# zju-vipa/ProtoPFormer

Hardware: AMD Instinct MI355X
Metric: images/sec train step, deit_small+2000 protos, bs256, 1/2/4/8 MI355X (higher is better)
Workload: dtype bf16; 1 GPU; deit_small_patch16_224, synthetic 224x224, 2000x384 prototypes, 200 classes, k=81, batch 256/GPU (BASELINE.json configs[2]), train step = fwd+CE+PPC+bwd+allreduce+AdamW+EMA, DropPath 0.1; blocks after the token reservation run compacted on the 1+k reserved rows (equal to the masked full-length blocks to bf16 rounding); bf16 backbone: the reserved tokens differ from the fp32 reference's in ~2-3 % o; global_batch=256, parallelism=dp1

## Files before the change

include/ppf_hip.h:

```cpp
#ifndef PPF_HIP_H
#define PPF_HIP_H

#include <stddef.h>
#include <stdint.h>

#ifdef __cplusplus
extern "C" {
#endif

typedef struct ihipStream_t* ppf_stream_t;

#define PPF_ERR_SHAPE (-1)
#define PPF_ERR_ALIGN (-2)
#define PPF_ERR_ARG (-3)

#define PPF_ABI_VERSION 10

const char* ppf_last_error(void);
int ppf_abi_version(void);
int ppf_device_info(int* cu_count, int* clock_mhz, char* name, int name_len);
int ppf_stream_arm(ppf_stream_t stream, int on);
int ppf_stream_wait_stream(ppf_stream_t dst, ppf_stream_t src);
int64_t ppf_stream_mark(ppf_stream_t stream);
int ppf_stream_wait_mark(ppf_stream_t stream, int64_t ticket);

int ppf_gemm_bf16(const void* A, const void* B, void* C, int M, int N, int K, int lda, int ldb, int ldc, int trans_a,
                  int trans_b, int epi, const float* bias, const float* res, int ldres, const float* rowscale,
                  int rows_per_group, const float* colscale, const void* aux_in, void* aux_out, int ldaux, float* colsum,
                  float alpha, void* workspace, size_t workspace_bytes, ppf_stream_t stream);
size_t ppf_gemm_workspace_bytes(int M, int N, int K);

int ppf_gemm_test_force_g224(int force);

int ppf_gemm_probe(int enable);
int ppf_gemm_probe_read(double* ms_total, int64_t* launches, double* flops, double* bytes);

int ppf_path_probe(int enable);
int ppf_path_probe_read(int tag, double* ms_total, int64_t* launches, double* flops, double* bytes);

int ppf_gemm_bf16_batched(const void* A, const void* B, void* C, int M, int N, int K, int lda, int ldb, int ldc, int trans_a,
                          int trans_b, int out_f32, float alpha, int batch_outer, int batch_inner, int64_t sa_o, int64_t sa_i,
                          int64_t sb_o, int64_t sb_i, int64_t sc_o, int64_t sc_i, int kpad, ppf_stream_t stream);

int ppf_layernorm_bwd_f32(const float* dy, const float* x, const int* row_map, const float* w, const float* dres_in, float* dx_out, float* dw, float* db,
                          int rows, int D, float eps, ppf_stream_t stream);
int ppf_ew_bwd_f32(int kind, const float* a, const float* b, float* out, const float* rowscale, int rows_per_group, int M, int N, ppf_stream_t stream);
int ppf_colsum_f32(const float* in, float* out, int M, int N, ppf_stream_t stream);
int ppf_attn_bwd_f32(const float* qkv, const float* dout, const float* policy, float* dqkv, float* scratch, int B, int H, int N, int D, int self_keep,
                     int eps_n, ppf_stream_t stream);
int ppf_th_attn_bwd_f32(const float* qkv, const float* dout, const float* wl, const float* bl, const float* ww, const float* bw, float* dqkv,
                        float* dwl, float* dbl, float* dww, float* dbw, int B, int H, int N, int D, ppf_stream_t stream);
int ppf_class_attn_bwd_f32(const float* q, const float* k, const float* v, const float* policy, const float* dout, float* dq, float* dk, float* dv,
                           int B, int H, int N1, int D, ppf_stream_t stream);

int ppf_rowgemm_supported(int D, int K, int rows_per_tile);
int ppf_rowgemm_bf16(const void* A, const void* B, int M, int D, int K, int lda, int ldb, int rows_per_tile, const float* bias, void* out,
                     ppf_stream_t stream);
int ppf_rowgemm_resid_ln(const void* A, const void* B, int M, int D, int K, int lda, int ldb, int rows_per_tile, const float* bias,
                         const float* res, float* xout, const float* rowscale, int rows_per_group, const float* colscale, void* aux_out,
                         const float* ln_w, const float* ln_b, void* ln_out, float* ln_mean, float* ln_rstd, float eps, ppf_stream_t stream);
int ppf_rowgemm_lnbwd(const void* A, const void* B, int M, int D, int K, int lda, int ldb, int rows_per_tile, const float* x, const float* mean,
                      const float* rstd, const float* w, const float* dres_in, float* dx_out, void* cast_out, const float* rowscale,
                      int rows_per_group, const float* colscale, const void* branch, float* partial, size_t partial_bytes, ppf_stream_t stream);
int ppf_rowgemm_colsum(const float* partial, int tiles, int D, int nparts, float* dw, float* db, float* dg, ppf_stream_t stream);
int ppf_transpose_bf16_batched(const void* src, void* dst, const void* desc_i64, int n, int total_tiles, ppf_stream_t stream);

int ppf_layernorm_fwd(const float* x, const int* row_map, const float* w, const float* b, void* y, float* mean, float* rstd,
                      int rows, int D, float eps, ppf_stream_t stream);
int ppf_layernorm_bwd(const void* dy, const float* x, const int* row_map, const float* w, const float* mean, const float* rstd,
                      const float* dres_in, float* dx_out, float* dw, float* db, void* cast_out, const float* rowscale,
                      int rows_per_group, const float* colscale, float* dbias_next, const void* branch, float* dcolscale,
                      int rows, int D, float* partial, size_t partial_bytes, ppf_stream_t stream);
int ppf_layernorm_bwd_blocks(int rows);
int ppf_layernorm_bwd_reduce(const float* partial, int rows, int D, float* dw, float* db, float* dbias_next, float* dcolscale,
                             ppf_stream_t stream);

int ppf_attn_fwd(const void* qkv, void* out, const float* policy, float* rowmax, float* zinv, int B, int H, int N, int D,
                 int self_keep, int eps_n, ppf_stream_t stream);
int ppf_attn_fwd_hm_supported(int H, int N, int D);
int ppf_attn_fwd_hm(const void* qkv, void* out, const float* policy, float* rowmax, float* zinv, float* headmean, int NP, int B, int H, int N,
                    int D, int self_keep, int eps_n, ppf_stream_t stream);
int ppf_attn_headmean(const void* qkv, const float* policy, const float* rowmax, const float* zinv, float* headmean, int NP,
                      int B, int H, int N, int D, int self_keep, int eps_n, ppf_stream_t stream);
int ppf_attn_bwd(const void* qkv, const void* out, const void* dout, void* dqkv, const float* policy, const float* rowmax,
                 const float* zinv, float* delta, int B, int H, int N, int D, int self_keep, int eps_n, ppf_stream_t stream);

int ppf_th_scores(const void* qkv, const float* wl, const float* bl, float* sp, int B, int H, int N, int D, int NP, ppf_stream_t stream);
int ppf_th_dwl(const void* qkv, const float* ds_prime, float* dwl, int B, int H, int N, int D, int NP, ppf_stream_t stream);
int ppf_th_softmax_mix(float* sp, void* a16, float* hm, const float* ww, const float* bw, int B, int H, int N, int NP, int NPK,
                       ppf_stream_t stream);
int ppf_th_softmax_bwd(const float* prob, float* da, void* ds16, const float* ww, const float* wl, float* dww, float* dbw, float* dbl,
                       int B, int H, int N, int NP, int NPK, ppf_stream_t stream);
int ppf_th_fused_supported(int H, int N, int D);
int ppf_th_fwd(const void* qkv, const float* wl, const float* bl, const float* ww, const float* bw, void* a16, float* hm, float* rowmax,
               float* zinv, void* out, int B, int H, int N, int D, int NP, int NPK, ppf_stream_t stream);
size_t ppf_th_bwd_partial_floats(int B, int H, int N);
int ppf_th_bwd(const void* qkv, const void* dout, const float* wl, const float* bl, const float* ww, const float* rowmax, const float* zinv,
               void* ds16, float* partial, int B, int H, int N, int D, int NPK, ppf_stream_t stream);
int ppf_th_param_reduce(const float* partial, int B, int H, int N, float* dww, float* dbw, float* dbl, float* dwl, ppf_stream_t stream);
int ppf_th_grads_supported(int H, int N, int D);
int ppf_th_grads(const void* qkv, const void* dout, const void* ds16, const void* a16, void* dqkv, int B, int H, int N, int D, int NPK,
                 ppf_stream_t stream);
int ppf_class_attn_fwd(const void* q, const void* k, const void* v, const float* policy, float* attn, float* zinv, float* rowmean,
                       void* out, int B, int H, int N1, int D, ppf_stream_t stream);
int ppf_class_attn_bwd(const void* q, const void* k, const void* v, const float* attn, const float* zinv, const void* dout, void* dq,
                       void* dk, void* dv, int B, int H, int N1, int D, ppf_stream_t stream);
int ppf_merge3_cast(const float* a, const float* b, const float* cq, void* out, int rows, int D, int N1, ppf_stream_t stream);

int ppf_rollout_threshold(const float* hm_layer, int B, int N, int NP, int kdrop, void* thr_out_u32, ppf_stream_t stream);
int ppf_rollout(const float* hm, int64_t layer_stride, int L, int B, int N, int NP, const float* init_rows, int n_init, int lead,
                int kdrop, int kdrop_init, float identity, int k, const void* thr_u32, float* cls_attn, int* idx, float* policy,
                ppf_stream_t stream);
int ppf_topk_sorted(const float* scores, int B, int n, int k, int* idx, ppf_stream_t stream);

int ppf_proto_fwd(const float* tok, int64_t stride_b, int t0, int T, const float* protos, int B, int P, int Dp, int act_kind,
                  float eps, float* act_max, int* argmax, float* dist_full, float* act_full, void* workspace, size_t workspace_bytes,
                  ppf_stream_t stream);
size_t ppf_proto_fwd_workspace(int P, int Dp);
int ppf_proto_bwd(const float* tok, int64_t stride_b, int t0, int T, const float* protos, int B, int P, int Dp, int act_kind,
                  float eps, const float* dist_full, int map_is_act, const float* g_full, const float* g_max, const int* argmax, float* dtok,
                  int64_t dstride_b, float* dprotos, void* zeroed_workspace, size_t workspace_bytes, ppf_stream_t stream);
size_t ppf_proto_bwd_workspace(int B, int T, int P, int Dp, int want_dtok, int want_dprotos);
int ppf_proto_bwd_rows(const float* tok, int64_t stride_b, int t0, int T, const float* protos, int B, int P, int Dp, int act_kind,
                       float eps, const float* dist_full, int map_is_act, const float* g_rows, const void* label_i64, int ppc, const float* g_max,
                       const int* argmax, float* dtok, int64_t dstride_b, float* dprotos, void* workspace, size_t workspace_bytes,
                       ppf_stream_t stream);
size_t ppf_proto_bwd_single_workspace(int B, int P, int Dp);
int ppf_proto_bwd_single(const float* tok, int64_t stride_b, int t0, const float* protos, int B, int P, int Dp, int act_kind, float eps,
                         const float* dist, const float* g, float* dtok, int64_t dstride_b, float* dprotos, void* workspace,
                         size_t workspace_bytes, ppf_stream_t stream);

int ppf_ppc_loss(const float* act, const int* idx, const void* label_i64, int B, int P, int T, int ppc, int side,
                 float cov_thresh, float mean_thresh, float* partial, float* gcov, float* gmean, float* loss, ppf_stream_t stream);
int ppf_ppc_loss_bwd(const float* gcov, const float* gmean, const float* up_cov, const float* up_mean, const void* label_i64,
                     float* g_full, int B, int P, int T, int ppc, ppf_stream_t stream);
int ppf_cross_entropy(const float* logits, const void* label_i64, float* per_sample, float* dlogits, float* loss, int B, int C,
                      ppf_stream_t stream);
int ppf_soft_cross_entropy(const float* logits, const float* target, const void* label_i64, float smoothing, float* per_sample,
                           float* dlogits, float* loss, int B, int C, ppf_stream_t stream);
int ppf_eval_metrics(const float* logits, const float* logits_global, const float* logits_local, const void* label_i64, double* acc,
                     int B, int C, ppf_stream_t stream);
int ppf_proto_topk_init(float* val, int* img, int* pos, int P, int K, ppf_stream_t stream);
int ppf_proto_topk_merge(const float* act_max, const int* argmax, const int* idx, int k, const float* tok, int64_t stride_b, int t0, int Dp,
                         const void* label_i64, const int* image_id, int ppc, int B, int P, int K, float* val, int* img, int* pos,
                         float* best_feat, ppf_stream_t stream);
int ppf_explain_topk(const float* act_max, const int* argmax, const int* idx, int T, const float* act_full, const float* weight, float scale,
                     int ppc, const float* logits, const int* cls_in, int sign, int B, int P, int C, int M, int K, int G, int* cls_out,
                     float* cls_logit, int* proto, float* contrib, float* act, int* cell, float* evidence, float* maps, ppf_stream_t stream);
int ppf_sgemm(const float* A, const float* Bm, float* C, int M, int N, int K, int64_t sam, int64_t sak, int64_t sbn, int64_t sbk,
              int ldc, float alpha, float beta, float* workspace, int64_t workspace_floats, ppf_stream_t stream);
int64_t ppf_sgemm_pair_workspace(int M, int N0, int K0, int N1, int K1);
int ppf_sgemm_pair(const float* A0, const float* B0, float* out0, int N0, int K0, int64_t sam0, int64_t sak0, int64_t sbn0, int64_t sbk0,
                   int ldo0, float alpha0, const float* A1, const float* B1, float* out1, int N1, int K1, int64_t sam1, int64_t sak1,
                   int64_t sbn1, int64_t sbk1, int ldo1, float alpha1, float* sum, int ldsum, float c0, float c1, int M, float* workspace,
                   int64_t workspace_floats, ppf_stream_t stream);
int ppf_axpby(const float* x, const float* y, float* out, float a, float b, int64_t n, ppf_stream_t stream);
int ppf_axpbypcz(const float* x, const float* y, const float* z, float* out, float a, float b, float c, int64_t n, ppf_stream_t stream);

int ppf_act_upsample(const float* grids, float* out, int M, int g, int S, ppf_stream_t stream);
int ppf_act_peak(const float* grids, int M, int g, int S, float* peak_val, int* peak_yx, const int* parts, int maps_per_img, int n_parts,
                 int half_size, void* table_u8, ppf_stream_t stream);
int ppf_act_part_table(const int* peak_yx, int M, int S, const int* parts, int maps_per_img, int n_parts, int half_size, void* table_u8,
                       ppf_stream_t stream);
int ppf_act_order_stats(const float* grids, int M, int g, int S, int k_lo, int k_hi, float* stats, ppf_stream_t stream);
int ppf_act_box(const float* grids, const double* thr, int M, int g, int S, int* box, ppf_stream_t stream);
int ppf_add_gauss_noise(const float* x, float* out, int B, int64_t n_per_img, const void* image_id_i64, float sigma, uint64_t seed,
                        ppf_stream_t stream);
int ppf_part_meter_update(const void* table_u8, const void* table_noisy_u8, const int* parts, const void* label_i64, int B, int ppc, int n_parts,
                          int C, int* hits, int* visible, int* stable, int* images, int* bad, ppf_stream_t stream);

int ppf_cast_f32_bf16(const float* in, void* out, int64_t n, ppf_stream_t stream);
int ppf_cast_bf16_f32(const void* in, float* out, int64_t n, ppf_stream_t stream);
int ppf_im2col_patch(const float* img, void* cols, int B, int C, int H, int W, int patch, ppf_stream_t stream);
int ppf_assemble_tokens(const float* tok, const float* cls, const float* pos, float* x, int B, int Np, int D, int lead,
                        ppf_stream_t stream);
int ppf_assemble_tokens_bwd(const float* dx, void* dtok, float* dpos, float* dcls, int B, int Np, int D, int lead,
                            ppf_stream_t stream);
int ppf_sigmoid_bwd_blocks(int rows);
int ppf_sigmoid_bwd(const float* df, const float* f, void* dz, float* dbias, int rows, int cols, float* partial, size_t partial_bytes,
                    ppf_stream_t stream);
int ppf_adamw_step(float* p, const float* g, float* m, float* v, float* ema, void* p16, int64_t n, int nseg,
                   const int64_t* seg_bounds, const float* seg_lr, const float* seg_wd, float beta1, float beta2, float eps,
                   int step, float ema_decay, float grad_scale, ppf_stream_t stream);
int ppf_adamw_step_dev(float* p, const float* g, float* m, float* v, float* ema, void* p16, int64_t n, int nseg,
                       const int64_t* seg_bounds, const float* hyper, float beta1, float beta2, float eps, float ema_decay,
                       ppf_stream_t stream);
int ppf_adamw_step_guarded(float* p, const float* g, float* m, float* v, float* ema, void* p16, int64_t n, int nseg,
                           const int64_t* seg_bounds, const float* hyper, float beta1, float beta2, float eps, float ema_decay,
                           const float* loss, int* nonfinite_flag, ppf_stream_t stream);
int ppf_hyper_set(float* hyper, const float* host_vals, int n, ppf_stream_t stream);
int ppf_clip_grad_blocks(void);
int ppf_clip_grad_scale(const float* g, int64_t n, float max_norm, float pre_scale, float* partial, float* hyper, float* norm_out,
                        ppf_stream_t stream);
int ppf_droppath_scales(float* out, const float* keep, int nslot, int B, uint64_t seed, void* state_u64, ppf_stream_t stream);
int ppf_reserved_rows_map(const int* idx, int* rows, int B, int k, int N, ppf_stream_t stream);
int ppf_gather_rows(const void* src, const int* rows, void* dst, int nrows, int row_bytes, ppf_stream_t stream);
int ppf_scatter_rows(const void* src, const int* rows, void* dst, int nrows_src, int nrows_dst, int row_bytes, ppf_stream_t stream);
int ppf_memset_zero(void* ptr, size_t bytes, ppf_stream_t stream);
int ppf_copy_2d(void* dst, int64_t dst_pitch, const void* src, int64_t src_pitch, int64_t width, int64_t rows, ppf_stream_t stream);
int ppf_image_finish_u8(const void* in_u8_hwc, float* out_nchw, int B, int H, int W, const float* mean3, const float* std3,
                        const int* rects, uint64_t seed, const void* state_u64, ppf_stream_t stream);
#define PPF_MIX_KIND 0
#define PPF_MIX_YL 1
#define PPF_MIX_YH 2
#define PPF_MIX_XL 3
#define PPF_MIX_XH 4
#define PPF_MIX_WSELF 5
#define PPF_MIX_WOTHER 6
#define PPF_MIX_WORDS 8
int ppf_mixup_apply(float* x, const int* table_host, int* table_dev, int B, int Cc, int H, int W, ppf_stream_t stream);
int ppf_mixup_target(const void* label_i64, const float* lam, int lam_stride, float off_value, float on_value, float* target, int B,
                     int C, ppf_stream_t stream);
int ppf_scale_by_scalar(const float* x, const float* scalar_dev, float* out, int64_t n, ppf_stream_t stream);

int ppf_im2col_patch_f32(const float* img, float* cols, int B, int C, int H, int W, int patch, ppf_stream_t stream);
int ppf_layernorm_fwd_f32(const float* x, const int* row_map, const float* w, const float* b, float* y, int rows, int D, float eps,
                          ppf_stream_t stream);
int ppf_epilogue_f32(float* C, const float* bias, int kind, const float* res, const float* rowscale, int rows_per_group,
                     const float* colscale, int M, int N, ppf_stream_t stream);
int ppf_attn_fwd_f32(const float* qkv, float* out, const float* policy, float* headmean, int NP, int B, int H, int N, int D,
                     int self_keep, int eps_n, ppf_stream_t stream);
int ppf_th_attn_fwd_f32(const float* qkv, const float* wl, const float* bl, const float* ww, const float* bw, float* out,
                        float* headmean, int NP, int B, int H, int N, int D, ppf_stream_t stream);
int ppf_class_attn_fwd_f32(const float* q, const float* k, const float* v, const float* policy, float* attn_mean, float* out, int B,
                           int H, int N1, int D, ppf_stream_t stream);

#ifdef __cplusplus
}
#endif
#endif
```

protopformer_amd/backbone.py:

```python
import functools
import os

import torch
import torch.nn as nn

from . import _lib, ops
from .ops import EPI_ATOMIC, EPI_BF16, EPI_DGELU, EPI_F32, EPI_GELU, EPI_RESID, EPI_SIGMOID_F32

LN_EPS = 1e-6
_KEEP_CACHE = {}
_ROW_BWD_MAX_ELEMS = 12_000_000


def _row_bwd(M, D):
    return M * D <= _ROW_BWD_MAX_ELEMS


def droppath_scales(rates, B, device, training):
    slots = [r if training else 0.0 for r in rates]
    active = [i for i, r in enumerate(slots) if r > 0.0]
    if not active:
        return None, [-1] * len(slots)
    key = (tuple(slots), str(device))
    st = _KEEP_CACHE.get(key)
# ... 164 lines not shown
    for j in reversed(range(1, len(convs))):
        c, x_in = convs[j], acts[j - 1]
        ops.linear_wgrad_f32(d, x_in, gv(c.weight), gv(c.bias))
        d = ops.ew_bwd_f32(5, ops.linear_dgrad_f32(d, c.weight), x_in)
    ops.colsum_f32(d, gv(convs[0].bias))
    return ops.cast_bf16(d)


class WgradLane:

    def __init__(self, device):
        self.enabled = os.environ.get("PPF_WGRAD_STREAM", "1") != "0"
        self.streams = [torch.cuda.Stream(device=device)] if self.enabled else []
        self.raws = [st.cuda_stream for st in self.streams]
        self.last_read = {}
        self.tracked = set()
        self.held = []
        self.pending = []

    def track(self, t):
        self.tracked.add(t.data_ptr())
        return t

    def submit(self, fn, reads, tag=None, defer=False):
        if not self.enabled:
            fn()
            return
        self.pending.append((fn, reads, tag))
        self.held.extend(reads)
        if not defer:
            self.flush()

    def flush(self, tag=None):
        if not self.pending:
            return
        raw = self.raws[0]
        try:
            _lib.call("ppf_stream_wait_stream", raw, _lib.stream_ptr())
            for fn, reads, tg in self.pending:
                _lib.push_stream(raw)
                try:
                    fn()
                    ptrs = [t.data_ptr() for t in reads if t.data_ptr() in self.tracked]
                    if ptrs:
                        ticket = _lib.stream_mark(raw)
                        for q in ptrs:
                            self.last_read[q] = ticket
                finally:
                    _lib.pop_stream()
        finally:
            self.pending.clear()

    def before_overwrite(self, t):
        if t.data_ptr() not in self.tracked:
            raise RuntimeError("WgradLane.before_overwrite: buffer was not registered with track()")
        q = t.data_ptr()
        if any(r.data_ptr() == q for _, reads, _t in self.pending for r in reads):
            self.flush()
        ticket = self.last_read.pop(q, None)
        if ticket is not None:
            _lib.call("ppf_stream_wait_mark", _lib.stream_ptr(), ticket)

    def join(self):
        if self.enabled:
            self.flush()
            for raw in self.raws:
                _lib.call("ppf_stream_wait_stream", _lib.stream_ptr(), raw)
        self.last_read.clear()
        self.tracked.clear()
        self.held.clear()


def wgrad_lane(store):
    lane = getattr(store, "_wgrad_lane", None)
    if lane is None:
        lane = store._wgrad_lane = WgradLane(store.device)
    return lane


_ROLL_TAIL = 1
_ROLL_BATCH = 3


def _wgrad(store, dy16, x16, weight, bias=None, defer=False):
    gw = store.grad_view(weight)
    gb = store.grad_view(bias) if bias is not None else None
    wgrad_lane(store).submit(lambda: ops.gemm(dy16, x16, trans_a=True, trans_b=True, epi=EPI_ATOMIC, out=gw.reshape(weight.shape[0], -1),
                                              colsum=gb), (dy16, x16), defer=defer and min(weight.shape[0], weight.shape[1]) <= 256)


_DGRAD_ROW = 3


def _dgrad(store, dy16, weight, rows, which):
    wt = store.w16t(weight)
    if wt is not None and (_DGRAD_ROW & which) and ops.rowgemm_ok(wt.shape[0], wt.shape[1], rows):
        return ops.rowgemm_bf16(dy16, wt, rows)
    if wt is not None:
        return ops.gemm(dy16, wt, epi=EPI_BF16)
    return ops.gemm(dy16, store.w16(weight), trans_b=True, epi=EPI_BF16)


def head_bwd(ppnet, store, saved, df):
    head = saved["head"]
    conv = addon_convs(ppnet)[0]
    dz = addon_bwd(ppnet, store, head, saved["f"].reshape(-1, saved["f"].shape[-1]), df)
    _wgrad(store, dz, head["nf"], conv.weight)
    return ops.gemm(dz, store.w16(conv.weight).reshape(conv.out_channels, -1), trans_b=True, epi=EPI_BF16)


def chunk_ready(gs, lane, chunk):
    lane.flush()
    _lib.run_live(lambda: gs.chunk_ready(chunk, also=lane.streams))


def dyb_ring(lane, D):
    nring = 4 if D > 256 else 64
    ring = {}

    def next_dyb(cur):
        if nring >= 64:
            return torch.empty_like(cur)
        bufs = ring.setdefault(tuple(cur.shape), [cur])
        if not any(b.data_ptr() == cur.data_ptr() for b in bufs):
            bufs.append(cur)
        if len(bufs) < nring:
            nxt = lane.track(torch.empty_like(cur))
            bufs.append(nxt)
        else:
            i = next(j for j, b in enumerate(bufs) if b.data_ptr() == cur.data_ptr())
            nxt = bufs[(i + 1) % len(bufs)]
        lane.before_overwrite(nxt)
        return nxt

    return next_dyb


def branch_out(store, dyb, rowscale, rows_per_group, gamma=None, raw=None):
    kw = dict(cast_out=dyb, rowscale=rowscale, rows_per_group=rows_per_group)
    if gamma is not None:
        kw.update(colscale=gamma, branch=raw, dcolscale=store.grad_view(gamma))
    return kw


def mlp_bwd(store, blk, L, dyb, bias_done):
    fc1, fc2 = blk.mlp.fc1, blk.mlp.fc2
    _wgrad(store, dyb, L["g"], fc2.weight, None if bias_done else fc2.bias, defer=True)
    w2t = store.w16t(fc2.weight)
    if w2t is not None:
        dh = ops.gemm(dyb, w2t, epi=EPI_DGELU, aux_in=L["h"])
    else:
        dh = ops.gemm(dyb, store.w16(fc2.weight), trans_b=True, epi=EPI_DGELU, aux_in=L["h"])
    _wgrad(store, dh, L["n2"], fc1.weight, fc1.bias)
    return dh


def row_tile_bwd(store, blk, D, rpt):
    covered = (all(store.w16t(w) is not None for w in (blk.mlp.fc1.weight, blk.attn.qkv.weight, blk.attn.proj.weight))
               and ops.rowgemm_ok(D, blk.mlp.fc1.out_features, rpt) and ops.rowgemm_ok(D, 3 * D, rpt) and ops.rowgemm_ok(D, D, rpt))
    return rpt if covered else None


def block_bwd(blk, store, L, dx, dyb, bias_done, below, *, next_dyb, attn_bwd, lnb, dgrad, row_tile):
    lane = wgrad_lane(store)
    gv = store.grad_view
    Nl = L["N"]
    fc1, qkv, proj = blk.mlp.fc1, blk.attn.qkv, blk.attn.proj
    fused = row_tile is not None

    def norm_bwd(dy, weight, dn, x, mean, rstd, norm, out, bias_next=None):
        nw = norm.weight
        if fused:
            ops.rowgemm_lnbwd(dy, store.w16t(weight), x, mean, rstd, nw, gv(nw), gv(norm.bias), row_tile, dres_in=dx, dx_out=dx,
                              lane=lane, defer_reduce=True, **out)
        else:
            lnb(dn, x, nw, mean, rstd, gv(nw), gv(norm.bias), dres_in=dx, dx_out=dx, dbias_next=gv(bias_next) if out else None, **out)

    dh = mlp_bwd(store, blk, L, dyb, bias_done)
    dyb = next_dyb(dyb)
    dn2 = None if fused else dgrad(dh, fc1.weight, Nl, 1)
    norm_bwd(dh, fc1.weight, dn2, L["x1"], L["mean2"], L["rstd2"], blk.norm2, branch_out(store, dyb, L["s1"], Nl, getattr(blk, "gamma_1", None), L["raw1"]),
             proj.bias)
    bias_done = not fused
    _wgrad(store, dyb, L["ao"], proj.weight, None if bias_done else proj.bias, defer=True)
    dao = ops.rowgemm_bf16(dyb, store.w16t(proj.weight), row_tile) if fused else dgrad(dyb, proj.weight, Nl, 4)
    dqkv = attn_bwd(blk, L, dao)
    _wgrad(store, dqkv, L["n1"], qkv.weight, qkv.bias)
    dn1 = None if fused else dgrad(dqkv, qkv.weight, Nl, 2)
    if below is None:
        norm_bwd(dqkv, qkv.weight, dn1, L["x"], L["mean1"], L["rstd1"], blk.norm1, {})
        return None, bias_done
    prev, Lp = below
    dyb = next_dyb(dyb)
    norm_bwd(dqkv, qkv.weight, dn1, L["x"], L["mean1"], L["rstd1"], blk.norm1,
             branch_out(store, dyb, Lp["s2"], Nl, getattr(prev, "gamma_2", None), Lp["raw2"]), prev.mlp.fc2.bias)
    return dyb, not fused


def embed_bwd(ppnet, store, saved, dx, lead):
    feats = ppnet.features
    pe = feats.patch_embed
    Np, D = pe.num_patches, dx.shape[1]
    gv = store.grad_view
    dtok = ops.assemble_tokens_bwd(dx, gv(feats.pos_embed).reshape(Np + lead, D), gv(feats.cls_token).reshape(D) if lead else None,
                                   dx.shape[0] // (Np + lead), Np, D, lead)
    _wgrad(store, dtok, saved["cols"], pe.proj.weight, pe.proj.bias)
    lane = wgrad_lane(store)
    gs = getattr(ppnet, "_grad_sync", None)
    if gs is not None:
        chunk_ready(gs, lane, gs.head_chunk)
    lane.join()


def deit_backward(ppnet, store, saved, df):
    feats = ppnet.features
    layers, head = saved["layers"], saved["head"]
    x_last = saved["x_last"]
    B, N, D = x_last.shape
    M = B * N
    dev = x_last.device
    lane = wgrad_lane(store)
    lnb = functools.partial(ops.layernorm_bwd, lane=lane, defer_reduce=True)
    dnf = head_bwd(ppnet, store, saved, df)
    alloc = ops.zeros if head["row_map"] is not None else (lambda shape, dtype, device: torch.empty(shape, dtype=dtype, device=device))
    dx = alloc((M, D), torch.float32, dev)
    dyb = lane.track(alloc((M, D), torch.bfloat16, dev))
    last = feats.blocks[-1]
    lnb(dnf, x_last.reshape(M, D), feats.norm.weight, head["meanf"], head["rstdf"], store.grad_view(feats.norm.weight),
        store.grad_view(feats.norm.bias), dx_out=dx, row_map=head["row_map"], cast_out=dyb, rowscale=layers[-1]["s2"],
        rows_per_group=N, dbias_next=store.grad_view(last.mlp.fc2.bias))
    gs = getattr(ppnet, "_grad_sync", None)
    if gs is not None:
        chunk_ready(gs, lane, gs.tail_chunk)
    bwd = functools.partial(block_bwd, next_dyb=dyb_ring(lane, D), lnb=lnb, dgrad=functools.partial(_dgrad, store),
                            attn_bwd=lambda blk, L, dao: ops.attn_bwd(L["qkv"], L["ao"], dao, L["rowmax"], L["zinv"], B, feats.num_heads, L["N"], D,
                                                                      policy=L["policy"], self_keep=True, eps_n=L["eps_n"]))
    bias_done = True
    for i in range(len(layers) - 1, -1, -1):
        L = layers[i]
        Nl = L["N"]
        row_tile = row_tile_bwd(store, feats.blocks[i], D, ops.rowgemm_tile_rows(B * Nl, Nl, backward=True)) if _row_bwd(B * Nl, D) else None
        dyb, bias_done = bwd(feats.blocks[i], store, L, dx, dyb, bias_done, (feats.blocks[i - 1], layers[i - 1]) if i > 0 else None,
                             row_tile=row_tile)
        if i > 0 and L["rows"] is not None:
            Mf = B * layers[i - 1]["N"]
            dx = ops.scatter_rows(dx, L["rows"], Mf)
            dyb = lane.track(ops.scatter_rows(dyb, L["rows"], Mf))
        if gs is not None and i in gs.block_chunk:
            chunk_ready(gs, lane, gs.block_chunk[i])
    if layers and layers[0]["rows"] is not None:
        dx = ops.scatter_rows(dx, layers[0]["rows"], B * (feats.patch_embed.num_patches + 1))
    embed_bwd(ppnet, store, saved, dx, 1)


class TokensFn(torch.autograd.Function):

    @staticmethod
    def forward(ctx, img, ppnet, dp, *params):
        store = ppnet.flat_store()
        store.refresh_bf16()
        feats = ppnet.features
        need_bwd = any(ctx.needs_input_grad)
        if need_bwd and "t16_params" in ppnet._arch_fns:
            if store._t16 is None:
                store.register_transposed(ppnet._arch_fns["t16_params"](feats))
            if store._t16 is not None and not store._t16["fresh"] and feats.embed_dim <= 256:
                wgrad_lane(store).submit(store.refresh_t16, (store.bf16, store._t16["buf"]), defer=True)
            else:
                store.refresh_t16()
        saved = {} if need_bwd else None
        (layer, k), = ppnet.reserve_layer_nums
        fwd = ppnet._arch_fns
        x = fwd["embed"](feats, store, img, saved)
        x_out, cls_attn, idx, layers = fwd["blocks"](feats, store, x, layer, k, dp, save=need_bwd)
        f, head = head_tokens_fwd(ppnet, store, x_out, idx)
        if need_bwd:
            saved.update(layers=layers, head=head, x_last=x_out, f=f)
            ctx.saved = saved
            ctx.ppnet = ppnet
        ctx.mark_non_differentiable(cls_attn, idx)
        return f, cls_attn, idx

    @staticmethod
    def backward(ctx, df, _dcls, _didx):
        ppnet, saved = ctx.ppnet, ctx.saved
        store = ppnet.flat_store()
        store.attach_all_grads()
        ppnet._arch_fns["backward"](ppnet, store, saved, df.contiguous().reshape(-1, df.shape[-1]))
        ctx.saved = None
        return (None, None, None) + (None,) * (len(ctx.needs_input_grad) - 3)


def t16_params(feats):
    return [w for blk in feats.blocks for w in (blk.mlp.fc1.weight, blk.attn.qkv.weight, blk.attn.proj.weight, blk.mlp.fc2.weight)]


DEIT_FNS = dict(embed=functools.partial(embed_tokens, lead=1), blocks=deit_blocks_fwd, backward=deit_backward, t16_params=t16_params)
```

protopformer_amd/csrc/elementwise.hip:

```cpp
#include "ppf_common.h"
#include "ppf_hip.h"

namespace {

__global__ __launch_bounds__(256) void cast_kernel(const float* __restrict__ in, bf16_t* __restrict__ out, int64_t n8) {
    for (int64_t i = (int64_t)blockIdx.x * 256 + threadIdx.x; i < n8; i += (int64_t)gridDim.x * 256) {
        const float4 a = reinterpret_cast<const float4*>(in)[2 * i], b = reinterpret_cast<const float4*>(in)[2 * i + 1];
        reinterpret_cast<uint4*>(out)[i] = make_uint4(pack_bf16x2(a.x, a.y), pack_bf16x2(a.z, a.w), pack_bf16x2(b.x, b.y), pack_bf16x2(b.z, b.w));
    }
}

__global__ __launch_bounds__(256) void widen_kernel(const bf16_t* __restrict__ in, float* __restrict__ out, int64_t n8) {
    for (int64_t i = (int64_t)blockIdx.x * 256 + threadIdx.x; i < n8; i += (int64_t)gridDim.x * 256) {
        const uint4 u = reinterpret_cast<const uint4*>(in)[i];
        const float2 a = unpack_bf16x2(u.x), b = unpack_bf16x2(u.y), c = unpack_bf16x2(u.z), d = unpack_bf16x2(u.w);
        reinterpret_cast<float4*>(out)[2 * i] = make_float4(a.x, a.y, b.x, b.y);
        reinterpret_cast<float4*>(out)[2 * i + 1] = make_float4(c.x, c.y, d.x, d.y);
    }
}

__global__ __launch_bounds__(256) void im2col_kernel(const float* __restrict__ img, bf16_t* __restrict__ cols, int B, int C,
                                                     int H, int W, int p, int64_t total8) {
    const int gh = H / p, gw = W / p, pp8 = p / 8, kdim = C * p * p;
    for (int64_t i = (int64_t)blockIdx.x * 256 + threadIdx.x; i < total8; i += (int64_t)gridDim.x * 256) {
// ... 123 lines not shown
            dz[o] = h;
            acc += bf16_to_f32(h);
        }
        if (partial) partial[(size_t)blockIdx.x * cols + c] = acc;
        else if (dbias) unsafeAtomicAdd(dbias + c, acc);
    }
}
__global__ __launch_bounds__(1024) void sigmoid_bias_reduce_kernel(const float* __restrict__ partial, float* __restrict__ dbias, int nblk, int cols) {
    __shared__ float red[16][64];
    const int cl = threadIdx.x & 63, g = threadIdx.x >> 6, c = blockIdx.x * 64 + cl;
    float acc = 0.f;
    if (c < cols) {
#pragma unroll 8
        for (int b = g; b < nblk; b += 16) acc += partial[(size_t)b * cols + c];
    }
    red[g][cl] = acc;
    __syncthreads();
    if (g == 0 && c < cols) {
        float t = 0.f;
#pragma unroll
        for (int i = 0; i < 16; ++i) t += red[i][cl];
        dbias[c] += t;
    }
}

__global__ __launch_bounds__(256) void sumsq_partial_kernel(const float* __restrict__ g, int64_t n4, float* __restrict__ partial) {
    float acc = 0.f;
    for (int64_t i = (int64_t)blockIdx.x * 256 + threadIdx.x; i < n4; i += (int64_t)gridDim.x * 256) {
        const float4 v = reinterpret_cast<const float4*>(g)[i];
        acc += v.x * v.x + v.y * v.y + v.z * v.z + v.w * v.w;
    }
    __shared__ float red[4];
    acc = wave_sum(acc);
    if ((threadIdx.x & 63) == 0) red[threadIdx.x >> 6] = acc;
    __syncthreads();
    if (threadIdx.x == 0) partial[blockIdx.x] = (red[0] + red[1]) + (red[2] + red[3]);
}
__global__ __launch_bounds__(256) void clip_finish_kernel(const float* __restrict__ partial, int nblk, float max_norm, float pre_scale,
                                                          float* __restrict__ hyper, float* __restrict__ norm_out) {
    __shared__ float red[256];
    float acc = 0.f;
    for (int i = threadIdx.x; i < nblk; i += 256) acc += partial[i];
    red[threadIdx.x] = acc;
    __syncthreads();
    for (int s = 128; s > 0; s >>= 1) {
        if (threadIdx.x < s) red[threadIdx.x] += red[threadIdx.x + s];
        __syncthreads();
    }
    if (threadIdx.x == 0) {
        const float nrm = pre_scale * sqrtf(red[0]);
        hyper[19] = fminf(1.0f, max_norm / (nrm + 1e-6f));
        if (norm_out) *norm_out = nrm;
    }
}

__global__ __launch_bounds__(256) void droppath_kernel(float* __restrict__ out, const float* __restrict__ keep, int nslot, int B,
                                                       uint64_t seed, unsigned long long* __restrict__ state) {
    const unsigned long long step = state[0];
    const int total = nslot * B;
    for (int i4 = threadIdx.x; i4 * 4 < total; i4 += 256) {
        const uint4 r = philox4x32_10(make_uint4((uint32_t)i4, 0u, (uint32_t)step, (uint32_t)(step >> 32)),
                                      make_uint2((uint32_t)seed, (uint32_t)(seed >> 32)));
        const uint32_t rv[4] = {r.x, r.y, r.z, r.w};
#pragma unroll
        for (int j = 0; j < 4; ++j) {
            const int i = i4 * 4 + j;
            if (i < total) {
                const float kp = keep[i / B];
                const float u = (float)(rv[j] >> 8) * (1.0f / 16777216.0f);
                out[i] = floorf(kp + u) / kp;
            }
        }
    }
    __syncthreads();
    if (threadIdx.x == 0) state[0] = step + 1;
}

__global__ __launch_bounds__(256) void rows_map_kernel(const int* __restrict__ idx, int* __restrict__ rows, int B, int k, int N) {
    const int i = blockIdx.x * 256 + threadIdx.x;
    if (i >= B * (k + 1)) return;
    const int b = i / (k + 1), j = i % (k + 1);
    rows[i] = b * N + (j == 0 ? 0 : 1 + idx[b * k + j - 1]);
}
__global__ __launch_bounds__(256) void move_rows_kernel(const uint4* __restrict__ src, const int* __restrict__ rows, uint4* __restrict__ dst,
                                                        int nrows, int vec, int scatter) {
    const int64_t total = (int64_t)nrows * vec;
    for (int64_t i = (int64_t)blockIdx.x * 256 + threadIdx.x; i < total; i += (int64_t)gridDim.x * 256) {
        const int r = (int)(i / vec), c = (int)(i % vec);
        const int64_t o = (int64_t)rows[r] * vec + c;
        if (scatter) dst[o] = src[i]; else dst[i] = src[o];
    }
}
__global__ __launch_bounds__(256) void scale_by_kernel(const float* __restrict__ x, const float* __restrict__ scalar, float* __restrict__ out, int64_t n) {
    const float s = *scalar;
    for (int64_t i = (int64_t)blockIdx.x * 256 + threadIdx.x; i < n; i += (int64_t)gridDim.x * 256) out[i] = x[i] * s;
}

struct FinishParams { const unsigned char* in; float* out; const int* rects; int B, H, W; float mean[3], inv_std[3]; uint64_t seed; const unsigned long long* state; };
__global__ __launch_bounds__(256) void image_finish_kernel(const FinishParams p) {
    const int64_t hw = (int64_t)p.H * p.W, total4 = (int64_t)p.B * hw / 4;
    const unsigned long long step = p.state ? p.state[0] : 0ull;
    for (int64_t i = (int64_t)blockIdx.x * 256 + threadIdx.x; i < total4; i += (int64_t)gridDim.x * 256) {
        const int b = (int)((i * 4) / hw);
        const int64_t pix = i * 4 - (int64_t)b * hw;
        const int y = (int)(pix / p.W), x = (int)(pix % p.W);
        const unsigned char* src = p.in + ((int64_t)b * hw + pix) * 3;
        const uint32_t w0 = reinterpret_cast<const uint32_t*>(src)[0], w1 = reinterpret_cast<const uint32_t*>(src)[1], w2 = reinterpret_cast<const uint32_t*>(src)[2];
        const unsigned char px[12] = {(unsigned char)w0, (unsigned char)(w0 >> 8), (unsigned char)(w0 >> 16), (unsigned char)(w0 >> 24),
                                      (unsigned char)w1, (unsigned char)(w1 >> 8), (unsigned char)(w1 >> 16), (unsigned char)(w1 >> 24),
                                      (unsigned char)w2, (unsigned char)(w2 >> 8), (unsigned char)(w2 >> 16), (unsigned char)(w2 >> 24)};
        int ry = 0, rx = 0, rh = 0, rw = 0;
        if (p.rects) { ry = p.rects[4 * b]; rx = p.rects[4 * b + 1]; rh = p.rects[4 * b + 2]; rw = p.rects[4 * b + 3]; }
        const bool row_in = rh > 0 && y >= ry && y < ry + rh;
#pragma unroll
        for (int c = 0; c < 3; ++c) {
            float v[4];
#pragma unroll
            for (int j = 0; j < 4; ++j) v[j] = ((float)px[3 * j + c] * (1.0f / 255.0f) - p.mean[c]) * p.inv_std[c];
            if (row_in && x + 3 >= rx && x < rx + rw) {
                const uint4 r = philox4x32_10(make_uint4((uint32_t)(i & 0xffffffff), (uint32_t)(i >> 32) * 3u + c, (uint32_t)step, (uint32_t)(step >> 32)),
                                              make_uint2((uint32_t)p.seed, (uint32_t)(p.seed >> 32)));
                const float u0 = ((float)(r.x >> 8) + 0.5f) * (1.0f / 16777216.0f), u1 = (float)(r.y >> 8) * (1.0f / 16777216.0f);
                const float u2 = ((float)(r.z >> 8) + 0.5f) * (1.0f / 16777216.0f), u3 = (float)(r.w >> 8) * (1.0f / 16777216.0f);
                const float m0 = sqrtf(-2.0f * __logf(u0)), m1 = sqrtf(-2.0f * __logf(u2));
                const float n[4] = {m0 * __cosf(6.283185307f * u1), m0 * __sinf(6.283185307f * u1), m1 * __cosf(6.283185307f * u3), m1 * __sinf(6.283185307f * u3)};
#pragma unroll
                for (int j = 0; j < 4; ++j)
                    if (x + j >= rx && x + j < rx + rw) v[j] = n[j];
            }
            *reinterpret_cast<float4*>(p.out + ((int64_t)b * 3 + c) * hw + pix) = make_float4(v[0], v[1], v[2], v[3]);
        }
    }
}

struct HyperVals { float v[20]; int n; };
__global__ void hyper_set_kernel(float* __restrict__ hyper, const HyperVals h) {
    if ((int)threadIdx.x < h.n) hyper[threadIdx.x] = h.v[threadIdx.x];
}

__global__ __launch_bounds__(256) void copy_2d_kernel(const uint4* __restrict__ src, uint4* __restrict__ dst, int rows, int w16, long long sp16, long long dp16) {
    const long long total = (long long)rows * w16;
    for (long long i = (long long)blockIdx.x * 256 + threadIdx.x; i < total; i += (long long)gridDim.x * 256) {
        const long long r = i / w16, c = i - r * w16;
        dst[r * dp16 + c] = src[r * sp16 + c];
    }
}

inline int grid_for(int64_t work, int per_block = 256) {
    int64_t g = (work + per_block - 1) / per_block;
    return (int)(g < 1 ? 1 : (g > 2048 ? 2048 : g));
}

__global__ __launch_bounds__(256) void transpose_bf16_kernel(const bf16_t* __restrict__ src, bf16_t* __restrict__ dst, const long long* __restrict__ desc, int n) {
    __shared__ bf16_t tile[64][66];
    int b = blockIdx.x, i = 0;
    for (; i < n; ++i) {
        const int tiles = (int)((desc[4 * i + 2] + 63) / 64) * (int)((desc[4 * i + 3] + 63) / 64);
        if (b < tiles) break;
        b -= tiles;
    }
    if (i == n) return;
    const bf16_t* s = src + desc[4 * i];
    bf16_t* d = dst + desc[4 * i + 1];
    const int rows = (int)desc[4 * i + 2], cols = (int)desc[4 * i + 3];
    const int tc = (cols + 63) / 64, r0 = (b / tc) * 64, c0 = (b % tc) * 64;
    const int tx = threadIdx.x & 63, ty = threadIdx.x >> 6;
// ... 68 lines not shown
}

int ppf_adamw_step(float* p, const float* g, float* m, float* v, float* ema, void* p16, int64_t n, int nseg, const int64_t* seg_bounds,
                   const float* seg_lr, const float* seg_wd, float beta1, float beta2, float eps, int step, float ema_decay,
                   float grad_scale, hipStream_t stream) {
    PPF_CHECK_ARG(n > 0 && (n % 4) == 0 && nseg >= 1 && nseg <= MAX_SEGS && step >= 1, PPF_ERR_ARG, "ppf_adamw_step: bad arguments");
    AdamParams a;
    a.p = p; a.g = g; a.m = m; a.v = v; a.ema = ema; a.p16 = (bf16_t*)p16; a.n = n; a.nseg = nseg;
    for (int s = 0; s < nseg; ++s) {
        PPF_CHECK_ARG(seg_bounds[s] % 4 == 0 && seg_bounds[s + 1] >= seg_bounds[s], PPF_ERR_ALIGN, "ppf_adamw_step: segment bounds must be multiples of 4");
        a.seg[s].begin = seg_bounds[s]; a.seg[s].end = seg_bounds[s + 1]; a.seg[s].lr = seg_lr[s]; a.seg[s].wd = seg_wd[s];
    }
    a.beta1 = beta1; a.beta2 = beta2; a.eps = eps;
    a.bc1 = 1.0f - powf(beta1, (float)step);
    a.bc2_sqrt = sqrtf(1.0f - powf(beta2, (float)step));
    a.ema_decay = ema_decay; a.grad_scale = grad_scale; a.hyper = nullptr;
    a.guard = nullptr; a.nonfinite = nullptr;
    hipLaunchKernelGGL(adamw_kernel, dim3(grid_for(n / 4)), dim3(256), 0, stream, a);
    PPF_LAUNCH_CHECK();
    return 0;
}

int ppf_adamw_step_guarded(float* p, const float* g, float* m, float* v, float* ema, void* p16, int64_t n, int nseg,
                           const int64_t* seg_bounds, const float* hyper, float beta1, float beta2, float eps, float ema_decay,
                           const float* loss, int* nonfinite_flag, hipStream_t stream) {
    PPF_CHECK_ARG(n > 0 && (n % 4) == 0 && nseg >= 1 && nseg <= MAX_SEGS && hyper, PPF_ERR_ARG, "ppf_adamw_step_dev: bad arguments");
    PPF_CHECK_ARG((loss == nullptr) == (nonfinite_flag == nullptr), PPF_ERR_ARG, "ppf_adamw_step_guarded: loss and flag go together");
    AdamParams a;
    a.p = p; a.g = g; a.m = m; a.v = v; a.ema = ema; a.p16 = (bf16_t*)p16; a.n = n; a.nseg = nseg;
    for (int s = 0; s < MAX_SEGS; ++s) { a.seg[s].begin = a.seg[s].end = 0; a.seg[s].lr = a.seg[s].wd = 0.f; }
    for (int s = 0; s < nseg; ++s) {
        PPF_CHECK_ARG(seg_bounds[s] % 4 == 0 && seg_bounds[s + 1] >= seg_bounds[s], PPF_ERR_ALIGN, "ppf_adamw_step_dev: segment bounds must be multiples of 4");
        a.seg[s].begin = seg_bounds[s]; a.seg[s].end = seg_bounds[s + 1];
    }
    a.beta1 = beta1; a.beta2 = beta2; a.eps = eps; a.bc1 = a.bc2_sqrt = 1.f; a.ema_decay = ema_decay; a.grad_scale = 1.f; a.hyper = hyper;
    a.guard = loss; a.nonfinite = nonfinite_flag;
    hipLaunchKernelGGL(adamw_kernel, dim3(grid_for(n / 4)), dim3(256), 0, stream, a);
    PPF_LAUNCH_CHECK();
    return 0;
}

int ppf_adamw_step_dev(float* p, const float* g, float* m, float* v, float* ema, void* p16, int64_t n, int nseg,
                       const int64_t* seg_bounds, const float* hyper, float beta1, float beta2, float eps, float ema_decay,
                       hipStream_t stream) {
    return ppf_adamw_step_guarded(p, g, m, v, ema, p16, n, nseg, seg_bounds, hyper, beta1, beta2, eps, ema_decay, nullptr, nullptr, stream);
}

int ppf_hyper_set(float* hyper, const float* host_vals, int n, hipStream_t stream) {
    PPF_CHECK_ARG(hyper && host_vals && n >= 1 && n <= 20, PPF_ERR_ARG, "ppf_hyper_set: bad arguments");
    HyperVals h;
    for (int i = 0; i < 20; ++i) h.v[i] = i < n ? host_vals[i] : 0.f;
    h.n = n;
    hipLaunchKernelGGL(hyper_set_kernel, dim3(1), dim3(64), 0, stream, hyper, h);
    PPF_LAUNCH_CHECK();
    return 0;
}

int ppf_clip_grad_blocks(void) { return 512; }

int ppf_clip_grad_scale(const float* g, int64_t n, float max_norm, float pre_scale, float* partial, float* hyper, float* norm_out,
                        hipStream_t stream) {
    PPF_CHECK_ARG(n > 0 && (n % 4) == 0 && max_norm > 0.f && partial && hyper, PPF_ERR_ARG, "ppf_clip_grad_scale: bad arguments");
    const int nblk = ppf_clip_grad_blocks();
    hipLaunchKernelGGL(sumsq_partial_kernel, dim3(nblk), dim3(256), 0, stream, g, n / 4, partial);
    hipLaunchKernelGGL(clip_finish_kernel, dim3(1), dim3(256), 0, stream, partial, nblk, max_norm, pre_scale, hyper, norm_out);
    PPF_LAUNCH_CHECK();
    return 0;
}

int ppf_droppath_scales(float* out, const float* keep, int nslot, int B, uint64_t seed, void* state_u64, hipStream_t stream) {
    PPF_CHECK_ARG(nslot > 0 && B > 0 && out && keep && state_u64, PPF_ERR_ARG, "ppf_droppath_scales: bad arguments");
    hipLaunchKernelGGL(droppath_kernel, dim3(1), dim3(256), 0, stream, out, keep, nslot, B, seed, (unsigned long long*)state_u64);
    PPF_LAUNCH_CHECK();
    return 0;
}

int ppf_reserved_rows_map(const int* idx, int* rows, int B, int k, int N, hipStream_t stream) {
    PPF_CHECK_ARG(B > 0 && k > 0 && N > k, PPF_ERR_SHAPE, "ppf_reserved_rows_map: bad shape B=%d k=%d N=%d", B, k, N);
    hipLaunchKernelGGL(rows_map_kernel, dim3((B * (k + 1) + 255) / 256), dim3(256), 0, stream, idx, rows, B, k, N);
    PPF_LAUNCH_CHECK();
    return 0;
}

int ppf_gather_rows(const void* src, const int* rows, void* dst, int nrows, int row_bytes, hipStream_t stream) {
    PPF_CHECK_ARG(nrows > 0 && row_bytes > 0 && row_bytes % 16 == 0, PPF_ERR_ALIGN, "ppf_gather_rows: row_bytes=%d must be a positive multiple of 16", row_bytes);
    hipLaunchKernelGGL(move_rows_kernel, dim3(grid_for((int64_t)nrows * (row_bytes / 16))), dim3(256), 0, stream, (const uint4*)src, rows, (uint4*)dst,
                       nrows, row_bytes / 16, 0);
    PPF_LAUNCH_CHECK();
    return 0;
}

int ppf_scatter_rows(const void* src, const int* rows, void* dst, int nrows_src, int nrows_dst, int row_bytes, hipStream_t stream) {
    PPF_CHECK_ARG(nrows_src > 0 && nrows_dst >= nrows_src && row_bytes > 0 && row_bytes % 16 == 0, PPF_ERR_ALIGN, "ppf_scatter_rows: bad arguments");
    hipError_t e = ppf_memset_async(dst, 0, (size_t)nrows_dst * row_bytes, stream);
    if (e != hipSuccess) { ppf_set_error("ppf_scatter_rows: memset failed: %s", hipGetErrorString(e)); return (int)e; }
    hipLaunchKernelGGL(move_rows_kernel, dim3(grid_for((int64_t)nrows_src * (row_bytes / 16))), dim3(256), 0, stream, (const uint4*)src, rows, (uint4*)dst,
                       nrows_src, row_bytes / 16, 1);
    PPF_LAUNCH_CHECK();
    return 0;
}

int ppf_image_finish_u8(const void* in_u8_hwc, float* out_nchw, int B, int H, int W, const float* mean3, const float* std3, const int* rects,
                        uint64_t seed, const void* state_u64, hipStream_t stream) {
    PPF_CHECK_ARG(B > 0 && H > 0 && W > 0 && W % 4 == 0 && in_u8_hwc && out_nchw && mean3 && std3, PPF_ERR_ARG, "ppf_image_finish_u8: bad arguments (W %% 4 == 0)");
    PPF_CHECK_ARG((((uintptr_t)in_u8_hwc) & 3) == 0 && (((uintptr_t)out_nchw) & 15) == 0, PPF_ERR_ALIGN, "ppf_image_finish_u8: alignment");
    FinishParams p;
    p.in = (const unsigned char*)in_u8_hwc; p.out = out_nchw; p.rects = rects; p.B = B; p.H = H; p.W = W; p.seed = seed;
    p.state = (const unsigned long long*)state_u64;
    for (int c = 0; c < 3; ++c) { p.mean[c] = mean3[c]; p.inv_std[c] = 1.0f / std3[c]; }
    hipLaunchKernelGGL(image_finish_kernel, dim3(grid_for((int64_t)B * H * W / 4)), dim3(256), 0, stream, p);
    PPF_LAUNCH_CHECK();
    return 0;
}

int ppf_memset_zero(void* ptr, size_t bytes, hipStream_t stream) {
    if (bytes == 0) return 0;
    hipError_t e = ppf_memset_async(ptr, 0, bytes, stream);
    if (e != hipSuccess) { ppf_set_error("ppf_memset_zero: %s", hipGetErrorString(e)); return (int)e; }
    return 0;
}

int ppf_scale_by_scalar(const float* x, const float* scalar_dev, float* out, int64_t n, hipStream_t stream) {
    PPF_CHECK_ARG(n > 0 && x && scalar_dev && out, PPF_ERR_ARG, "ppf_scale_by_scalar: bad arguments");
    hipLaunchKernelGGL(scale_by_kernel, dim3(grid_for(n)), dim3(256), 0, stream, x, scalar_dev, out, n);
    PPF_LAUNCH_CHECK();
    return 0;
}

int ppf_transpose_bf16_batched(const void* src, void* dst, const void* desc_i64, int n, int total_tiles, hipStream_t stream) {
    PPF_CHECK_ARG(src && dst && desc_i64 && n > 0 && total_tiles > 0, PPF_ERR_ARG, "ppf_transpose_bf16_batched: bad arguments");
    hipLaunchKernelGGL(transpose_bf16_kernel, dim3(total_tiles), dim3(256), 0, stream, (const bf16_t*)src, (bf16_t*)dst, (const long long*)desc_i64, n);
    PPF_LAUNCH_CHECK();
    return 0;
}

int ppf_copy_2d(void* dst, int64_t dst_pitch, const void* src, int64_t src_pitch, int64_t width, int64_t rows, hipStream_t stream) {
    PPF_CHECK_ARG(dst && src && width > 0 && rows > 0 && dst_pitch >= width && src_pitch >= width, PPF_ERR_ARG, "ppf_copy_2d: bad arguments");
    if ((((uintptr_t)dst | (uintptr_t)src | (uint64_t)dst_pitch | (uint64_t)src_pitch | (uint64_t)width) & 15) == 0 && rows * (width / 16) < (int64_t)1 << 31) {
        const int w16 = (int)(width / 16);
        hipLaunchKernelGGL(copy_2d_kernel, dim3(grid_for(rows * w16)), dim3(256), 0, stream, (const uint4*)src, (uint4*)dst, (int)rows, w16,
                           (long long)(src_pitch / 16), (long long)(dst_pitch / 16));
        PPF_LAUNCH_CHECK();
        return 0;
    }
    hipError_t e = ppf_memcpy2d_async(dst, (size_t)dst_pitch, src, (size_t)src_pitch, (size_t)width, (size_t)rows, hipMemcpyDeviceToDevice, stream);
    if (e != hipSuccess) { ppf_set_error("ppf_copy_2d: %s", hipGetErrorString(e)); return (int)e; }
    return 0;
}

}
```

protopformer_amd/csrc/gemm_bf16.hip:

```cpp
#include "ppf_common.h"
#include "ppf_hip.h"
#include "gemm_common.h"
#include <cstdlib>
#include <type_traits>

namespace {
using namespace ppfg;

constexpr int BM = 128, BN = 128, BK = 64, NTHREADS = 256;
constexpr int TILE_BYTES = BM * BK * 2;
constexpr int STAGE_LD = 68;
constexpr int STAGE_BYTES = 4 * 32 * STAGE_LD * 4;


__device__ __forceinline__ int lds_off_mode0(int r, int c16) { return lds_row_off(r, c16); }
template <int ROWS>
__device__ __forceinline__ int lds_off_mode1(int kc, int col) {
    return kc * (ROWS * 2) + ((((col >> 5) ^ (kc & 3))) << 6) + ((col & 31) << 1);
}

typedef uint32_t u32x4 __attribute__((ext_vector_type(4)));

template <bool T, int ROWS, int NTHR = NTHREADS>
struct TileIO {
    static constexpr int NLD = ROWS * 8 / NTHR;
    static constexpr int RPP = NTHR / 8;
    static constexpr int CPR = ROWS / 8;
    static constexpr int KPP = NTHR / CPR;
    static __device__ __forceinline__ unsigned gload(u32x4 (&reg)[NLD], const bf16_t* __restrict__ X, int ld, int R, int row0,
                                                     int k0, int kend, int tid, int kpad) {
        unsigned mask = 0;
        if constexpr (!T) {
            const int c16 = tid & 7, rb = tid >> 3;
            const bool kok = kpad ? (k0 + c16 * 8) < kend : (k0 + c16 * 8 + 8) <= kend;
            const int kk = kok ? k0 + c16 * 8 : 0;
#pragma unroll
            for (int i = 0; i < NLD; ++i) {
                const int r = row0 + rb + RPP * i;
                const bf16_t* src = X + (size_t)min(r, R - 1) * ld + kk;
                reg[i] = *reinterpret_cast<const u32x4*>(src);
                mask |= (kok && r < R) ? (1u << i) : 0u;
            }
        } else {
            const int c16 = tid % CPR, kb = tid / CPR;
            const int col = row0 + c16 * 8;
            const bool cok = kpad ? col < R : (col + 8) <= R;
            const int cc = cok ? col : 0;
#pragma unroll
            for (int i = 0; i < NLD; ++i) {
                const int kc = k0 + kb + KPP * i;
                const bf16_t* src = X + (size_t)min(kc, kend - 1) * ld + cc;
                reg[i] = *reinterpret_cast<const u32x4*>(src);
                mask |= (cok && kc < kend) ? (1u << i) : 0u;
            }
        }
        return mask;
    }
    static __device__ __forceinline__ void sstore(const u32x4 (&reg)[NLD], unsigned mask, unsigned char* tile, int tid) {
        const u32x4 zero = {0u, 0u, 0u, 0u};
        if constexpr (!T) {
            const int c16 = tid & 7, rb = tid >> 3;
#pragma unroll
            for (int i = 0; i < NLD; ++i)
                *reinterpret_cast<u32x4*>(tile + lds_off_mode0(rb + RPP * i, c16)) = ((mask >> i) & 1u) ? reg[i] : zero;
        } else {
            const int c16 = tid % CPR, kb = tid / CPR;
#pragma unroll
            for (int i = 0; i < NLD; ++i)
                *reinterpret_cast<u32x4*>(tile + lds_off_mode1<ROWS>(kb + KPP * i, c16 * 8)) = ((mask >> i) & 1u) ? reg[i] : zero;
        }
    }
    static __device__ __forceinline__ bf16x8 frag(const unsigned char* tile, int rbase, int ks, int lane) {
        if constexpr (!T) {
            return *reinterpret_cast<const bf16x8*>(tile + lds_off_mode0(rbase + (lane & 31), ks * 2 + (lane >> 5)));
        } else {
            typedef __attribute__((address_space(3))) bf16x4 lds_bf16x4;
            const int s = lane & 15, g16 = (lane >> 4) & 1, h = lane >> 5;
            const int col = rbase + 16 * g16 + 4 * (s & 3);
            const int kc = ks * 16 + 8 * h + (s >> 2);
            bf16x4 lo = __builtin_amdgcn_ds_read_tr16_b64_v4bf16((lds_bf16x4*)(tile + lds_off_mode1<ROWS>(kc, col)));
            bf16x4 hi = __builtin_amdgcn_ds_read_tr16_b64_v4bf16((lds_bf16x4*)(tile + lds_off_mode1<ROWS>(kc + 4, col)));
            return __builtin_shufflevector(lo, hi, 0, 1, 2, 3, 4, 5, 6, 7);
        }
    }
};


template <int EPI>
__device__ __forceinline__ void epilogue_rows(const GemmParams& p, const float* stage, int mbase, int nbase, int lane) {
    if (EpiWide<EPI>::value && ((p.ldc | p.ldaux) & 7) == 0) {
        const int col = (lane & 7) * 8;
        const int n = nbase + col;
        if (n + 8 <= p.N) {
            const EpiCols8 cc = epi_load_cols8<EPI>(p, n, true);
            EpiRow8 rr[4];
#pragma unroll
            for (int pass = 0; pass < 4; ++pass) {
                const int m = mbase + pass * 8 + (lane >> 3);
                rr[pass] = epi_load_row8<EPI>(p, m, n, m < p.M);
            }
#pragma unroll
            for (int pass = 0; pass < 4; ++pass) {
                const int r = pass * 8 + (lane >> 3);
                const int m = mbase + r;
                const float4 a = *reinterpret_cast<const float4*>(stage + r * STAGE_LD + col);
                const float4 b = *reinterpret_cast<const float4*>(stage + r * STAGE_LD + col + 4);
                if (m < p.M) epi_store8<EPI>(p, m, n, a, b, cc, rr[pass]);
            }
        } else if (n < p.N) {
            const EpiCols cc = epi_load_cols<EPI>(p, n, true);
#pragma unroll
            for (int pass = 0; pass < 4; ++pass) {
                const int r = pass * 8 + (lane >> 3);
                const int m = mbase + r;
                if (m < p.M) {
                    const EpiRow rr = epi_load_row<EPI>(p, m, n, true);
                    const float4 v = *reinterpret_cast<const float4*>(stage + r * STAGE_LD + col);
                    epi_store<EPI>(p, m, n, v.x, v.y, v.z, v.w, cc, rr);
                }
            }
        }
    } else {
        const int col = (lane & 15) * 4;
        const int n = nbase + col;
        const EpiCols cc = epi_load_cols<EPI>(p, n, n < p.N);
        EpiRow rr[8];
#pragma unroll
        for (int pass = 0; pass < 8; ++pass) {
            const int m = mbase + pass * 4 + (lane >> 4);
            rr[pass] = epi_load_row<EPI>(p, m, n, m < p.M && n < p.N);
        }
#pragma unroll
        for (int pass = 0; pass < 8; ++pass) {
            const int r = pass * 4 + (lane >> 4);
            const int m = mbase + r;
            const float4 v = *reinterpret_cast<const float4*>(stage + r * STAGE_LD + col);
            if (m < p.M && n < p.N) epi_store<EPI>(p, m, n, v.x, v.y, v.z, v.w, cc, rr[pass]);
        }
    }
}

struct KSlice { int kbeg, kend; };
__device__ __forceinline__ KSlice k_slice(int K, int nsplit, int zslice) {
    const int kchunk = (((K + nsplit - 1) / nsplit) + BK - 1) / BK * BK;
    const int kbeg = zslice * kchunk;
    return {kbeg, min(K, kbeg + kchunk)};
}

template <int EPI, int MT>
__device__ __forceinline__ void strip_epilogue(const GemmParams& p, const f32x16 (&acc)[2][MT], int mi, unsigned char* smem, int wave, int lane,
                                               int mbase, int nbase) {
    const int h = lane >> 5;
    float* stage = reinterpret_cast<float*>(smem) + wave * (32 * STAGE_LD);
#pragma unroll
    for (int ni = 0; ni < 2; ++ni)
#pragma unroll
        for (int g = 0; g < 4; ++g)
            *reinterpret_cast<float4*>(stage + (lane & 31) * STAGE_LD + 32 * ni + 8 * g + 4 * h) =
                make_float4(acc[ni][mi][4 * g], acc[ni][mi][4 * g + 1], acc[ni][mi][4 * g + 2], acc[ni][mi][4 * g + 3]);
    __builtin_amdgcn_wave_barrier();
    epilogue_rows<EPI>(p, stage, mbase, nbase, lane);
    __builtin_amdgcn_wave_barrier();
}

__device__ __forceinline__ void store_partial_colsum(const GemmParams& p, int m, float v) {
    p.ws[p.zslice * ((size_t)p.M * p.N + (size_t)p.cs_parts * p.M) + (size_t)p.M * p.N + m] = v;
}

template <bool TA, bool TB, int EPI, bool COLSUM>
__global__ __launch_bounds__(NTHREADS, 3) void gemm_kernel(const GemmParams p_) {
    constexpr int PD = 1, MT = 2;
    extern __shared__ __attribute__((aligned(16))) unsigned char smem[];
    constexpr int TBM = 64 * MT;
    constexpr int A_BYTES = TBM * BK * 2;
    using IOA = TileIO<TA, TBM>;
    using IOB = TileIO<TB, BN>;
    const int tid = threadIdx.x, lane = tid & 63, wave = tid >> 6;
    const int wm = (wave & 1) * (32 * MT), wn = (wave >> 1) * 64;

    const int tiles_n = (p_.N + BN - 1) / BN;
    const int tiles = tiles_n * ((p_.M + TBM - 1) / TBM);
    const int vid_all = xcd_remap(blockIdx.x, gridDim.x);
    const int zslice = vid_all / tiles, vid = vid_all - zslice * tiles;
    const int m0 = (vid / tiles_n) * TBM, n0 = (vid % tiles_n) * BN;
    GemmParams p = p_;
    p.zslice = zslice;
    if (gridDim.y > 1) {
        const int bo = blockIdx.y / p.batch_inner, bi = blockIdx.y % p.batch_inner;
        p.A += bo * p.sa_o + bi * p.sa_i;
        p.B += bo * p.sb_o + bi * p.sb_i;
        const long long co = bo * p.sc_o + bi * p.sc_i;
        p.C = (EPI == EPI_BF16) ? (void*)(reinterpret_cast<bf16_t*>(p.C) + co) : (void*)(reinterpret_cast<float*>(p.C) + co);
    }

    const auto [kbeg, kend] = k_slice(p.K, p.nsplit, zslice);
    if (kbeg >= kend) return;
    const int nk = (kend - kbeg + BK - 1) / BK;

    u32x4 ra[PD][IOA::NLD], rb[PD][IOB::NLD];
    unsigned ma[PD], mb[PD];
    f32x16 acc[2][MT];
#pragma unroll
    for (int i = 0; i < 2; ++i)
#pragma unroll
        for (int j = 0; j < MT; ++j)
#pragma unroll
            for (int r = 0; r < 16; ++r) acc[i][j][r] = 0.f;
    f32x16 accs[MT];
    if constexpr (COLSUM) {
#pragma unroll
        for (int j = 0; j < MT; ++j)
#pragma unroll
            for (int r = 0; r < 16; ++r) accs[j][r] = 0.f;
    }
    const bool do_colsum = COLSUM && p.colsum != nullptr && n0 == 0 && wn == 0;
    unsigned char* tA = smem;
    unsigned char* tB = smem + A_BYTES;

#pragma unroll
    for (int st = 0; st < PD; ++st) {
        const int k0 = min(kbeg + st * BK, kbeg + (nk - 1) * BK);
        ma[st] = IOA::gload(ra[st], p.A, p.lda, p.M, m0, k0, kend, tid, p.kpad);
        mb[st] = IOB::gload(rb[st], p.B, p.ldb, p.N, n0, k0, kend, tid, p.kpad);
    }
    IOA::sstore(ra[0], ma[0], tA, tid);
    IOB::sstore(rb[0], mb[0], tB, tid);
    __syncthreads();

    for (int kt0 = 0; kt0 < nk; kt0 += PD) {
#pragma unroll
        for (int u = 0; u < PD; ++u) {
            const int kt = kt0 + u;
            if (kt >= nk) break;
            {
                const int k0 = kbeg + min(kt + PD, nk - 1) * BK;
                ma[u] = IOA::gload(ra[u], p.A, p.lda, p.M, m0, k0, kend, tid, p.kpad);
                mb[u] = IOB::gload(rb[u], p.B, p.ldb, p.N, n0, k0, kend, tid, p.kpad);
            }
#pragma unroll
            for (int ks = 0; ks < BK / 16; ++ks) {
                bf16x8 fa[MT], fb[2];
#pragma unroll
                for (int i = 0; i < MT; ++i) fa[i] = IOA::frag(tA, wm + 32 * i, ks, lane);
#pragma unroll
                for (int i = 0; i < 2; ++i) fb[i] = IOB::frag(tB, wn + 32 * i, ks, lane);
#pragma unroll
                for (int ni = 0; ni < 2; ++ni)
#pragma unroll
                    for (int mi = 0; mi < MT; ++mi)
                        acc[ni][mi] = __builtin_amdgcn_mfma_f32_32x32x16_bf16(fb[ni], fa[mi], acc[ni][mi], 0, 0, 0);
                if constexpr (COLSUM) {
                    if (do_colsum) {
                        bf16x8 ones;
#pragma unroll
                        for (int e = 0; e < 8; ++e) ones[e] = (__bf16)1.0f;
#pragma unroll
                        for (int mi = 0; mi < MT; ++mi)
                            accs[mi] = __builtin_amdgcn_mfma_f32_32x32x16_bf16(ones, fa[mi], accs[mi], 0, 0, 0);
                    }
                }
            }
            __syncthreads();
            if (kt + 1 < nk) {
                IOA::sstore(ra[(u + 1) % PD], ma[(u + 1) % PD], tA, tid);
                IOB::sstore(rb[(u + 1) % PD], mb[(u + 1) % PD], tB, tid);
            }
            __syncthreads();
        }
    }

#pragma unroll
    for (int mi = 0; mi < MT; ++mi) {
        strip_epilogue<EPI>(p, acc, mi, smem, wave, lane, m0 + wm + 32 * mi, n0 + wn);
        if constexpr (COLSUM) {
            const int m = m0 + wm + 32 * mi + (lane & 31);
            if (do_colsum && (lane >> 5) == 0 && m < p.M) {
                if constexpr (EPI == EPI_PARTIAL) store_partial_colsum(p, m, accs[mi][0]);
                else unsafeAtomicAdd(p.colsum + m, accs[mi][0]);
            }
        }
    }
}

template <int WMW, int WNW, bool COLSUM>
__global__ __launch_bounds__(64 * WMW * WNW, 1) void wgrad8_kernel(const GemmParams p_) {
    extern __shared__ __attribute__((aligned(16))) unsigned char smem[];
    constexpr int NTHR = 64 * WMW * WNW, TBM = 64 * WMW, TBN = 64 * WNW;
    using IOA = TileIO<true, TBM, NTHR>;
    using IOB = TileIO<true, TBN, NTHR>;
    const int tid = threadIdx.x, lane = tid & 63;
    const int wave = __builtin_amdgcn_readfirstlane(tid >> 6);
    const int wm = (wave % WMW) * 64, wn = (wave / WMW) * 64;
    const int tiles_n = (p_.N + TBN - 1) / TBN;
    const int tiles = tiles_n * ((p_.M + TBM - 1) / TBM);
    const int vid_all = xcd_remap(blockIdx.x, gridDim.x);
    const int zslice = vid_all / tiles, vid = vid_all - zslice * tiles;
    const int m0 = (vid / tiles_n) * TBM, n0 = (vid % tiles_n) * TBN;
    GemmParams p = p_;
    p.zslice = zslice;
    const auto [kbeg, kend] = k_slice(p.K, p.nsplit, zslice);
    if (kbeg >= kend) return;
    const int nk = (kend - kbeg + BK - 1) / BK;

    u32x4 ra[IOA::NLD], rb[IOB::NLD];
    unsigned ma, mb;
    f32x16 acc[2][2];
#pragma unroll
    for (int i = 0; i < 2; ++i)
#pragma unroll
        for (int j = 0; j < 2; ++j)
#pragma unroll
            for (int r = 0; r < 16; ++r) acc[i][j][r] = 0.f;
    f32x16 accs[2];
    if constexpr (COLSUM) {
#pragma unroll
        for (int j = 0; j < 2; ++j)
#pragma unroll
            for (int r = 0; r < 16; ++r) accs[j][r] = 0.f;
    }
    const bool do_colsum = COLSUM && p.colsum != nullptr && n0 == 0 && wn == 0;
    unsigned char* tA = smem;
    unsigned char* tB = smem + TBM * BK * 2;
    ma = IOA::gload(ra, p.A, p.lda, p.M, m0, kbeg, kend, tid, 0);
    mb = IOB::gload(rb, p.B, p.ldb, p.N, n0, kbeg, kend, tid, 0);
    IOA::sstore(ra, ma, tA, tid);
    IOB::sstore(rb, mb, tB, tid);
    __syncthreads();
    for (int kt = 0; kt < nk; ++kt) {
        {
            const int k0 = kbeg + min(kt + 1, nk - 1) * BK;
            ma = IOA::gload(ra, p.A, p.lda, p.M, m0, k0, kend, tid, 0);
            mb = IOB::gload(rb, p.B, p.ldb, p.N, n0, k0, kend, tid, 0);
        }
#pragma unroll
        for (int ks = 0; ks < BK / 16; ++ks) {
            bf16x8 fa[2], fb[2];
#pragma unroll
            for (int i = 0; i < 2; ++i) fa[i] = IOA::frag(tA, wm + 32 * i, ks, lane);
#pragma unroll
            for (int i = 0; i < 2; ++i) fb[i] = IOB::frag(tB, wn + 32 * i, ks, lane);
#pragma unroll
            for (int ni = 0; ni < 2; ++ni)
#pragma unroll
                for (int mi = 0; mi < 2; ++mi) acc[ni][mi] = __builtin_amdgcn_mfma_f32_32x32x16_bf16(fb[ni], fa[mi], acc[ni][mi], 0, 0, 0);
            if constexpr (COLSUM) {
                if (do_colsum) {
                    bf16x8 ones;
#pragma unroll
                    for (int e = 0; e < 8; ++e) ones[e] = (__bf16)1.0f;
#pragma unroll
                    for (int mi = 0; mi < 2; ++mi) accs[mi] = __builtin_amdgcn_mfma_f32_32x32x16_bf16(ones, fa[mi], accs[mi], 0, 0, 0);
                }
            }
        }
        __syncthreads();
        if (kt + 1 < nk) {
            IOA::sstore(ra, ma, tA, tid);
            IOB::sstore(rb, mb, tB, tid);
        }
        __syncthreads();
    }
#pragma unroll
    for (int mi = 0; mi < 2; ++mi) {
        strip_epilogue<EPI_PARTIAL>(p, acc, mi, smem, wave, lane, m0 + wm + 32 * mi, n0 + wn);
        if constexpr (COLSUM) {
            const int m = m0 + wm + 32 * mi + (lane & 31);
            if (do_colsum && (lane >> 5) == 0 && m < p.M) store_partial_colsum(p, m, accs[mi][0]);
        }
    }
}

template <int WMW, int WNW>
int launch_wgrad8(const GemmParams& p, int splitk, hipStream_t stream) {
    constexpr int NTHR = 64 * WMW * WNW, TBM = 64 * WMW, TBN = 64 * WNW;
    constexpr int opnd = (TBM + TBN) * BK * 2, strips = (NTHR / 64) * 32 * STAGE_LD * 4;
    constexpr int lds = opnd > strips ? opnd : strips;
    const int tiles = ((p.M + TBM - 1) / TBM) * ((p.N + TBN - 1) / TBN);
    return ppf_launch<wgrad8_kernel<WMW, WNW, true>>(dim3(tiles * splitk), dim3(NTHR), lds, stream, "wgrad8", p);
}

typedef __attribute__((address_space(3))) void g4_lds_t;
typedef const __attribute__((address_space(1))) void g4_gbl_t;

template <int NLA>
struct DirectLds {
    unsigned offA[NLA], offB[4];
    const unsigned char *gA, *gB;
    __device__ __forceinline__ DirectLds(const GemmParams& p, int m0, int n0, int tid)
        : gA(reinterpret_cast<const unsigned char*>(p.A)), gB(reinterpret_cast<const unsigned char*>(p.B)) {
        const int rb = tid >> 3, ch = (tid & 7) ^ lds_swz(rb);
#pragma unroll
        for (int i = 0; i < NLA; ++i) offA[i] = ((unsigned)min(m0 + rb + 32 * i, p.M - 1) * (unsigned)p.lda + ch * 8) * 2u;
#pragma unroll
        for (int i = 0; i < 4; ++i) offB[i] = ((unsigned)min(n0 + rb + 32 * i, p.N - 1) * (unsigned)p.ldb + ch * 8) * 2u;
    }
    __device__ __forceinline__ void load(int kt, unsigned char* tA, unsigned char* tB, int wave) const {
        const unsigned char* ka = gA + (size_t)kt * (BK * 2);
        const unsigned char* kb = gB + (size_t)kt * (BK * 2);
#pragma unroll
        for (int i = 0; i < NLA; ++i)
            __builtin_amdgcn_global_load_lds((g4_gbl_t*)(ka + offA[i]), (g4_lds_t*)(tA + i * 4096 + wave * 1024), 16, 0, 0);
#pragma unroll
        for (int i = 0; i < 4; ++i)
            __builtin_amdgcn_global_load_lds((g4_gbl_t*)(kb + offB[i]), (g4_lds_t*)(tB + i * 4096 + wave * 1024), 16, 0, 0);
        asm volatile("s_waitcnt vmcnt(0)" ::: "memory");
        __syncthreads();
    }
};

template <int EPI>
__global__ __launch_bounds__(NTHREADS, 4) void gemm128g_kernel(const GemmParams p) {
    extern __shared__ __attribute__((aligned(16))) unsigned char smem[];
    using IO = TileIO<false, 128>;
    const int tid = threadIdx.x, lane = tid & 63;
    const int wave = __builtin_amdgcn_readfirstlane(tid >> 6);
    const int wm = (wave & 1) * 64, wn = (wave >> 1) * 64;
    const int tiles_n = (p.N + BN - 1) / BN;
    const int vid = xcd_remap(blockIdx.x, gridDim.x);
    const int m0 = (vid / tiles_n) * BM, n0 = (vid % tiles_n) * BN;
    unsigned char* tA = smem;
    unsigned char* tB = smem + TILE_BYTES;
    const DirectLds<BM / 32> dl(p, m0, n0, tid);
    f32x16 acc[2][2];
#pragma unroll
    for (int i = 0; i < 2; ++i)
#pragma unroll
        for (int j = 0; j < 2; ++j)
#pragma unroll
            for (int r = 0; r < 16; ++r) acc[i][j][r] = 0.f;

    const int nk = p.K / BK;
    for (int kt = 0; kt < nk; ++kt) {
        if (kt > 0) __syncthreads();
        dl.load(kt, tA, tB, wave);
#pragma unroll
        for (int ks = 0; ks < BK / 16; ++ks) {
            bf16x8 fa[2], fb[2];
#pragma unroll
            for (int i = 0; i < 2; ++i) fa[i] = IO::frag(tA, wm + 32 * i, ks, lane);
#pragma unroll
            for (int i = 0; i < 2; ++i) fb[i] = IO::frag(tB, wn + 32 * i, ks, lane);
#pragma unroll
            for (int ni = 0; ni < 2; ++ni)
#pragma unroll
                for (int mi = 0; mi < 2; ++mi)
                    acc[ni][mi] = __builtin_amdgcn_mfma_f32_32x32x16_bf16(fb[ni], fa[mi], acc[ni][mi], 0, 0, 0);
        }
    }
    __syncthreads();
#pragma unroll
    for (int mi = 0; mi < 2; ++mi) strip_epilogue<EPI>(p, acc, mi, smem, wave, lane, m0 + wm + 32 * mi, n0 + wn);
}

template <int EPI>
int launch_g4(const GemmParams& p, hipStream_t stream) {
    constexpr int lds = 2 * TILE_BYTES > STAGE_BYTES ? 2 * TILE_BYTES : STAGE_BYTES;
    const int tiles = ((p.M + BM - 1) / BM) * ((p.N + BN - 1) / BN);
    return ppf_launch<gemm128g_kernel<EPI>>(dim3(tiles), dim3(NTHREADS), lds, stream, "gemm128g", p);
}

constexpr int G224_ROWS = 224, G224_MT = 7, G224_LD = 36;
// ... 3 lines not shown
    const int tid = threadIdx.x, lane = tid & 63;
    const int wave = __builtin_amdgcn_readfirstlane(tid >> 6);
    const int wn = wave * 32;
    const int tiles_n = (p.N + BN - 1) / BN;
    const int vid = xcd_remap(blockIdx.x, gridDim.x);
    const int m0 = (vid / tiles_n) * G224_ROWS, n0 = (vid % tiles_n) * BN;
    unsigned char* tA = smem;
    unsigned char* tB = smem + G224_ROWS * BK * 2;
    const DirectLds<G224_MT> dl(p, m0, n0, tid);
    f32x16 acc[G224_MT];
#pragma unroll
    for (int j = 0; j < G224_MT; ++j)
#pragma unroll
        for (int r = 0; r < 16; ++r) acc[j][r] = 0.f;
    const int nk = p.K / BK;
    for (int kt = 0; kt < nk; ++kt) {
        if (kt > 0) __syncthreads();
        dl.load(kt, tA, tB, wave);
#pragma unroll
        for (int ks = 0; ks < BK / 16; ++ks) {
            const bf16x8 fb = IO::frag(tB, wn, ks, lane);
#pragma unroll
            for (int mi = 0; mi < G224_MT; ++mi)
                acc[mi] = __builtin_amdgcn_mfma_f32_32x32x16_bf16(fb, IO::frag(tA, 32 * mi, ks, lane), acc[mi], 0, 0, 0);
        }
    }
    __syncthreads();
    const int h = lane >> 5;
    float* stage = reinterpret_cast<float*>(smem) + wave * (32 * G224_LD);
    bf16_t* C = reinterpret_cast<bf16_t*>(p.C);
#pragma unroll
    for (int mi = 0; mi < G224_MT; ++mi) {
#pragma unroll
        for (int g = 0; g < 4; ++g)
            *reinterpret_cast<float4*>(stage + (lane & 31) * G224_LD + 8 * g + 4 * h) =
                make_float4(acc[mi][4 * g], acc[mi][4 * g + 1], acc[mi][4 * g + 2], acc[mi][4 * g + 3]);
        __builtin_amdgcn_fence(__ATOMIC_RELEASE, "wavefront");
        __builtin_amdgcn_wave_barrier();
#pragma unroll
        for (int pass = 0; pass < 2; ++pass) {
            const int r = pass * 16 + (lane >> 2), col = (lane & 3) * 8;
            const int m = m0 + 32 * mi + r, n = n0 + wn + col;
            const float4 a = *reinterpret_cast<const float4*>(stage + r * G224_LD + col);
            const float4 b = *reinterpret_cast<const float4*>(stage + r * G224_LD + col + 4);
            if (m < p.M && n < p.N)
                *reinterpret_cast<uint4*>(C + (size_t)m * p.ldc + n) = make_uint4(pack_bf16x2(a.x * p.alpha, a.y * p.alpha), pack_bf16x2(a.z * p.alpha, a.w * p.alpha),
                                                                                 pack_bf16x2(b.x * p.alpha, b.y * p.alpha), pack_bf16x2(b.z * p.alpha, b.w * p.alpha));
        }
        __builtin_amdgcn_fence(__ATOMIC_RELEASE, "wavefront");
        __builtin_amdgcn_wave_barrier();
    }
}

bool g4_eligible(const GemmParams& p);
int g_force_g224 = 0;
bool g224_eligible(const GemmParams& p, int epi) {
    if (epi != EPI_BF16 || p.bias != nullptr || p.kpad || p.K % BK != 0 || p.N % 8 != 0 || (p.ldc & 7) != 0) return false;
    if ((long long)p.M * p.lda >= (1ll << 30) || (long long)p.N * p.ldb >= (1ll << 30)) return false;
    if (g_force_g224) return true;
    if (p.K < 768) return false;
    const int cus = ppf_cu_count();
    const long long tn = (p.N + BN - 1) / BN;
    const long long t128 = (long long)((p.M + BM - 1) / BM) * tn, t224 = (long long)((p.M + G224_ROWS - 1) / G224_ROWS) * tn;
    const int per128 = g4_eligible(p) ? 4 : 3;
    auto cost = [](long long tiles, long long slots, int rows, int per) {
        const long long full = tiles / slots, rest = tiles - full * slots;
        double c = (double)full * rows * per;
        if (rest) c += rows * per * (4 * rest >= slots ? 1.0 : 0.5);
        return c;
    };
    return t128 >= (long long)per128 * cus && cost(t224, 3ll * cus, G224_ROWS, 3) < 0.97 * cost(t128, (long long)per128 * cus, BM, per128);
}
int launch_g224(const GemmParams& p, hipStream_t stream) {
    constexpr int lds = G224_ROWS * BK * 2 + TILE_BYTES;
    const int tiles = ((p.M + G224_ROWS - 1) / G224_ROWS) * ((p.N + BN - 1) / BN);
    return ppf_launch<gemm224g_kernel>(dim3(tiles), dim3(NTHREADS), lds, stream, "gemm224g", p);
}

bool g4_eligible(const GemmParams& p) {
    return p.K % BK == 0 && p.K <= 512 && p.N >= 512 && !p.kpad && (long long)p.M * p.lda < (1ll << 30) &&
           (long long)p.N * p.ldb < (1ll << 30) && (long long)((p.M + BM - 1) / BM) * ((p.N + BN - 1) / BN) >= 512;
}

template <bool TA, bool TB, int EPI, bool COLSUM>
int launch(const GemmParams& p, int splitk, hipStream_t stream, int nbatch = 1) {
    const int tiles = ((p.M + BM - 1) / BM) * ((p.N + BN - 1) / BN);
    constexpr int lds = 2 * TILE_BYTES > STAGE_BYTES ? 2 * TILE_BYTES : STAGE_BYTES;
    GemmParams q = p;
    q.nsplit = splitk;
    return ppf_launch<gemm_kernel<TA, TB, EPI, COLSUM>>(dim3(tiles * splitk, nbatch, 1), dim3(NTHREADS), lds, stream, "gemm", q);
}

__global__ __launch_bounds__(256) void splitk_reduce_kernel(const float* __restrict__ ws, float* __restrict__ C, float* __restrict__ colsum,
                                                            int M, int N, int ldc, int nsplit, int cs_parts) {
    const size_t mn = (size_t)M * N, slice = mn + (colsum ? (size_t)cs_parts * M : 0);
    const size_t total4 = mn / 4;
    const size_t i = (size_t)blockIdx.x * 256 + threadIdx.x;
    if (i < total4) {
        const float* p = ws + i * 4;
        float4 acc = make_float4(0.f, 0.f, 0.f, 0.f);
        for (int z0 = 0; z0 < nsplit; z0 += 16) {
            float4 v[16];
#pragma unroll
            for (int u = 0; u < 16; ++u) {
                const int z = min(z0 + u, nsplit - 1);
                v[u] = *reinterpret_cast<const float4*>(p + (size_t)z * slice);
            }
#pragma unroll
            for (int u = 0; u < 16; ++u)
                if (z0 + u < nsplit) { acc.x += v[u].x; acc.y += v[u].y; acc.z += v[u].z; acc.w += v[u].w; }
        }
        const size_t e = i * 4, m = e / N, n = e - m * N;
        float4* dst = reinterpret_cast<float4*>(C + m * ldc + n);
        const float4 c = *dst;
        *dst = make_float4(c.x + acc.x, c.y + acc.y, c.z + acc.z, c.w + acc.w);
    } else if (colsum && i < total4 + (size_t)M) {
        const size_t m = i - total4;
        float a = 0.f;
        for (int z = 0; z < nsplit; ++z)
            for (int q = 0; q < cs_parts; ++q) a += ws[(size_t)z * slice + mn + (size_t)q * M + m];
        colsum[m] += a;
    }
}

PpfEventPool g_probe;
bool g_probe_on = false;

constexpr size_t PPF_GEMM_COUNTER_BYTES = 16384;

int pick_splitk(int M, int N, int K) {
    const int tiles = ((M + BM - 1) / BM) * ((N + BN - 1) / BN);
    const int target = min(M, N) <= 256 ? 216 : 432;
    int s = target / tiles;
    const int maxs = (K + 4 * BK - 1) / (4 * BK);
    if (s > maxs) s = maxs;
    if (s < 1) s = 1;
    const int kchunk = (((K + s - 1) / s) + BK - 1) / BK * BK;
    return (K + kchunk - 1) / kchunk;
}

template <int... EPIS, class F>
bool dispatch_epi(int epi, int& rc, F&& f) {
    return ((epi == EPIS && (rc = f(std::integral_constant<int, EPIS>()), true)) || ...);
}

}

extern "C" {

int ppf_gemm_test_force_g224(int force) { g_force_g224 = force != 0; return 0; }

size_t ppf_gemm_workspace_bytes(int M, int N, int K) {
    return PPF_GEMM_COUNTER_BYTES + (size_t)pick_splitk(M, N, K) * ((size_t)M * N + M) * sizeof(float);
}

int ppf_gemm_bf16(const void* A, const void* B, void* C, int M, int N, int K, int lda, int ldb, int ldc, int trans_a,
                  int trans_b, int epi, const float* bias, const float* res, int ldres, const float* rowscale,
                  int rows_per_group, const float* colscale, const void* aux_in, void* aux_out, int ldaux, float* colsum,
                  float alpha, void* workspace, size_t workspace_bytes, hipStream_t stream) {
    PPF_CHECK_ARG(M > 0 && N > 0 && K > 0, PPF_ERR_SHAPE, "ppf_gemm_bf16: bad shape M=%d N=%d K=%d", M, N, K);
    PPF_CHECK_ARG((lda % 8) == 0 && (ldb % 8) == 0 && (ldc % 4) == 0 && (N % 4) == 0, PPF_ERR_ALIGN,
                  "ppf_gemm_bf16: lda/ldb must be multiples of 8, ldc and N of 4 (lda=%d ldb=%d ldc=%d N=%d)", lda, ldb, ldc, N);
    PPF_CHECK_ARG(trans_a ? (M % 8 == 0) : (K % 8 == 0), PPF_ERR_ALIGN, "ppf_gemm_bf16: A inner extent must be a multiple of 8");
    PPF_CHECK_ARG(trans_b ? (N % 8 == 0) : (K % 8 == 0), PPF_ERR_ALIGN, "ppf_gemm_bf16: B inner extent must be a multiple of 8");
    PPF_CHECK_ARG((((uintptr_t)A | (uintptr_t)B | (uintptr_t)C) & 15) == 0, PPF_ERR_ALIGN, "ppf_gemm_bf16: pointers must be 16-byte aligned");
    PPF_CHECK_ARG(!(trans_a && !trans_b), PPF_ERR_ARG, "ppf_gemm_bf16: (trans_a=1, trans_b=0) is not instantiated");
    PPF_CHECK_ARG((((uintptr_t)aux_in | (uintptr_t)aux_out | (uintptr_t)res) & 15) == 0 && (ldaux % 4) == 0 && (ldres % 4) == 0, PPF_ERR_ALIGN,
                  "ppf_gemm_bf16: aux / residual pointers must be 16-byte aligned, ldaux and ldres multiples of 4 (the epilogues use 8/16-byte accesses)");
    GemmParams p;
    p.A = (const bf16_t*)A; p.B = (const bf16_t*)B; p.C = C; p.M = M; p.N = N; p.K = K; p.lda = lda; p.ldb = ldb; p.ldc = ldc;
    p.bias = bias; p.res = res; p.ldres = ldres; p.rowscale = rowscale; p.rows_per_group = rows_per_group > 0 ? rows_per_group : 1;
    p.colscale = colscale; p.aux_in = (const bf16_t*)aux_in; p.aux_out = (bf16_t*)aux_out; p.ldaux = ldaux; p.colsum = colsum; p.alpha = alpha; p.ws = nullptr;
    p.batch_inner = 1; p.sa_o = p.sa_i = p.sb_o = p.sb_i = p.sc_o = p.sc_i = 0; p.kpad = 0; p.cs_parts = 1; p.nsplit = 1;
    if (epi == EPI_RESID) PPF_CHECK_ARG(res != nullptr, PPF_ERR_ARG, "ppf_gemm_bf16: epi=4 needs a residual");
    if (epi == EPI_GELU) PPF_CHECK_ARG(aux_out != nullptr, PPF_ERR_ARG, "ppf_gemm_bf16: epi=2 needs aux_out");
    if (epi == EPI_DGELU) PPF_CHECK_ARG(aux_in != nullptr, PPF_ERR_ARG, "ppf_gemm_bf16: epi=5 needs aux_in");
    int rc;
    if (!trans_a && !trans_b) {
        if (g224_eligible(p, epi)) return launch_g224(p, stream);
        const auto g4 = [&](auto e) { return launch_g4<decltype(e)::value>(p, stream); };
        const auto nt = [&](auto e) { return launch<false, false, decltype(e)::value, false>(p, 1, stream); };
        if (g4_eligible(p) && dispatch_epi<EPI_BF16, EPI_GELU, EPI_RESID, EPI_DGELU>(epi, rc, g4)) return rc;
        if (dispatch_epi<EPI_BF16, EPI_F32, EPI_GELU, EPI_SIGMOID_F32, EPI_RESID, EPI_DGELU>(epi, rc, nt)) return rc;
    } else if (!trans_a && trans_b) {
        const auto nn = [&](auto e) { return launch<false, true, decltype(e)::value, false>(p, 1, stream); };
        if (dispatch_epi<EPI_BF16, EPI_F32, EPI_DGELU>(epi, rc, nn)) return rc;
    } else if (epi == EPI_ATOMIC) {
        const int ns = pick_splitk(M, N, K);
        const size_t need = PPF_GEMM_COUNTER_BYTES + (size_t)ns * ((size_t)M * N + M) * sizeof(float);
        if (workspace == nullptr || workspace_bytes < need || ns == 1) return launch<true, true, EPI_ATOMIC, true>(p, ns, stream);
        p.ws = (float*)((unsigned char*)workspace + PPF_GEMM_COUNTER_BYTES);
        p.cs_parts = 1;
        p.nsplit = ns;
        hipEvent_t e1 = nullptr;
        if (g_probe_on) {
            const auto ev = g_probe.acquire();
            (void)hipEventRecord(ev.first, stream);
            e1 = ev.second;
        }
        const bool wide = (M < N ? M : N) >= 320;
        if (wide && M >= 512 && M >= N && (M % 256 == 0 || M >= 1024)) rc = launch_wgrad8<4, 2>(p, ns, stream);
        else if (wide && N >= 512 && (N % 256 == 0 || N >= 1024)) rc = launch_wgrad8<2, 4>(p, ns, stream);
        else rc = launch<true, true, EPI_PARTIAL, true>(p, ns, stream);
        if (rc) return rc;
        if (e1) {
            (void)hipEventRecord(e1, stream);
            g_probe.flops += 2.0 * M * N * (double)K;
            g_probe.bytes += 2.0 * ((double)M * K + (double)N * K) + 4.0 * M * N;
        }
        const size_t work = (size_t)M * N / 4 + (colsum ? M : 0);
        const int grid = (int)((work + 255) / 256);
        hipLaunchKernelGGL(splitk_reduce_kernel, dim3(grid), dim3(256), 0, stream, p.ws, (float*)C, colsum, M, N, ldc, ns, p.cs_parts);
        PPF_LAUNCH_CHECK();
        return 0;
    } else if (epi == EPI_F32) {
        return launch<true, true, EPI_F32, false>(p, 1, stream);
    }
    ppf_set_error("ppf_gemm_bf16: combination trans_a=%d trans_b=%d epi=%d not instantiated", trans_a, trans_b, epi);
    return PPF_ERR_ARG;
}

int ppf_gemm_probe(int enable) {
    if (enable == 1) g_probe.reset();
    if (enable == 2) g_probe.destroy();
    g_probe_on = enable == 1;
    return 0;
}
int ppf_gemm_probe_read(double* ms_total, int64_t* launches, double* flops, double* bytes) {
    return g_probe.sum_ms("ppf_gemm_probe_read", ms_total, launches, flops, bytes);
}

int ppf_gemm_bf16_batched(const void* A, const void* B, void* C, int M, int N, int K, int lda, int ldb, int ldc, int trans_a, int trans_b,
                          int out_f32, float alpha, int batch_outer, int batch_inner, int64_t sa_o, int64_t sa_i, int64_t sb_o, int64_t sb_i,
                          int64_t sc_o, int64_t sc_i, int kpad, hipStream_t stream) {
    PPF_CHECK_ARG(M > 0 && N > 0 && K > 0 && batch_outer > 0 && batch_inner > 0, PPF_ERR_SHAPE, "ppf_gemm_bf16_batched: bad shape");
    PPF_CHECK_ARG((lda % 8) == 0 && (ldb % 8) == 0 && (ldc % 4) == 0 && (N % 4) == 0, PPF_ERR_ALIGN, "ppf_gemm_bf16_batched: ld alignment");
    PPF_CHECK_ARG(kpad || (trans_a ? (M % 8 == 0) : (K % 8 == 0)), PPF_ERR_ALIGN, "ppf_gemm_bf16_batched: A inner extent must be a multiple of 8");
    PPF_CHECK_ARG(kpad || (trans_b ? (N % 8 == 0) : (K % 8 == 0)), PPF_ERR_ALIGN, "ppf_gemm_bf16_batched: B inner extent must be a multiple of 8");
    PPF_CHECK_ARG(((sa_o | sa_i | sb_o | sb_i) % 8) == 0 && ((sc_o | sc_i) % 4) == 0, PPF_ERR_ALIGN, "ppf_gemm_bf16_batched: batch strides alignment");
    PPF_CHECK_ARG(out_f32 || (ldc % 8) != 0 || ((sc_o | sc_i) % 8) == 0, PPF_ERR_ALIGN,
                  "ppf_gemm_bf16_batched: bf16 output with ldc %% 8 == 0 needs batch strides of C that are multiples of 8 elements (sc_o=%lld sc_i=%lld)",
                  (long long)sc_o, (long long)sc_i);
    PPF_CHECK_ARG((((uintptr_t)A | (uintptr_t)B | (uintptr_t)C) & 15) == 0, PPF_ERR_ALIGN, "ppf_gemm_bf16_batched: pointers must be 16-byte aligned");
    GemmParams p;
    p.A = (const bf16_t*)A; p.B = (const bf16_t*)B; p.C = C; p.M = M; p.N = N; p.K = K; p.lda = lda; p.ldb = ldb; p.ldc = ldc;
    p.bias = nullptr; p.res = nullptr; p.ldres = 0; p.rowscale = nullptr; p.rows_per_group = 1; p.colscale = nullptr; p.aux_in = nullptr;
    p.aux_out = nullptr; p.ldaux = 0; p.colsum = nullptr; p.ws = nullptr; p.alpha = alpha;
    p.batch_inner = batch_inner; p.sa_o = sa_o; p.sa_i = sa_i; p.sb_o = sb_o; p.sb_i = sb_i; p.sc_o = sc_o; p.sc_i = sc_i; p.kpad = kpad;
    const int nb = batch_outer * batch_inner;
    const auto go = [&](auto ta, auto tb) {
        int rc = PPF_ERR_ARG;
        dispatch_epi<EPI_BF16, EPI_F32>(out_f32 ? EPI_F32 : EPI_BF16, rc, [&](auto e) {
            return launch<decltype(ta)::value, decltype(tb)::value, decltype(e)::value, false>(p, 1, stream, nb);
        });
        return rc;
    };
    if (!trans_a && !trans_b) return go(std::false_type(), std::false_type());
    if (!trans_a && trans_b) return go(std::false_type(), std::true_type());
    if (trans_a && trans_b) return go(std::true_type(), std::true_type());
    ppf_set_error("ppf_gemm_bf16_batched: (trans_a=1, trans_b=0) is not instantiated");
    return PPF_ERR_ARG;
}

}
```

protopformer_amd/csrc/gemm_common.h:

```cpp
#pragma once
#include "ppf_common.h"

namespace ppfg {

enum Epi { EPI_BF16 = 0, EPI_F32 = 1, EPI_GELU = 2, EPI_SIGMOID_F32 = 3, EPI_RESID = 4, EPI_DGELU = 5, EPI_ATOMIC = 6, EPI_PARTIAL = 7 };

struct GemmParams {
    const bf16_t* A; const bf16_t* B; void* C;
    int M, N, K, lda, ldb, ldc;
    const float* bias;
    const float* res;
    int ldres;
    const float* rowscale;
    int rows_per_group;
    const float* colscale;
    const bf16_t* aux_in;
    bf16_t* aux_out;
    int ldaux;
    float* colsum;
    float* ws;
    float alpha;
    int batch_inner;
    long long sa_o, sa_i, sb_o, sb_i, sc_o, sc_i;
    int zslice;
    int nsplit;
    int cs_parts;
    int kpad;
};

constexpr float GELU8_ZERO = 26.0f, GELU8_STEP = 1.0f / 196.0f, GELU8_INV = 196.0f;
__device__ __forceinline__ uint32_t gelu8_pack4(float a, float b, float c, float d) {
    uint32_t r = 0;
    r = __builtin_amdgcn_cvt_pk_u8_f32(a * GELU8_INV + GELU8_ZERO, 0, r);
    r = __builtin_amdgcn_cvt_pk_u8_f32(b * GELU8_INV + GELU8_ZERO, 1, r);
    r = __builtin_amdgcn_cvt_pk_u8_f32(c * GELU8_INV + GELU8_ZERO, 2, r);
    r = __builtin_amdgcn_cvt_pk_u8_f32(d * GELU8_INV + GELU8_ZERO, 3, r);
    return r;
}
__device__ __forceinline__ void gelu8_unpack4(uint32_t q, float (&d)[4]) {
    d[0] = ((float)(q & 0xffu) - GELU8_ZERO) * GELU8_STEP;
    d[1] = ((float)((q >> 8) & 0xffu) - GELU8_ZERO) * GELU8_STEP;
    d[2] = ((float)((q >> 16) & 0xffu) - GELU8_ZERO) * GELU8_STEP;
    d[3] = ((float)((q >> 24) & 0xffu) - GELU8_ZERO) * GELU8_STEP;
}

struct EpiCols { float4 bias, colscale; };
struct EpiRow { float4 res; uint2 aux; float rowscale; };

template <int EPI>
__device__ __forceinline__ EpiCols epi_load_cols(const GemmParams& p, int n0, bool ok) {
    EpiCols c;
    c.bias = make_float4(0.f, 0.f, 0.f, 0.f);
    c.colscale = make_float4(1.f, 1.f, 1.f, 1.f);
    if constexpr (EPI != EPI_ATOMIC && EPI != EPI_PARTIAL) {
        if (ok && p.bias) c.bias = *reinterpret_cast<const float4*>(p.bias + n0);
        if constexpr (EPI == EPI_RESID) { if (ok && p.colscale) c.colscale = *reinterpret_cast<const float4*>(p.colscale + n0); }
    }
    return c;
}

template <int EPI>
__device__ __forceinline__ EpiRow epi_load_row(const GemmParams& p, int m, int n0, bool ok) {
    EpiRow r;
    r.res = make_float4(0.f, 0.f, 0.f, 0.f); r.aux = make_uint2(0, 0); r.rowscale = 1.0f;
    if constexpr (EPI == EPI_RESID) {
        if (ok) {
            r.res = *reinterpret_cast<const float4*>(p.res + (size_t)m * p.ldres + n0);
            if (p.rowscale) r.rowscale = p.rowscale[m / p.rows_per_group];
        }
    } else if constexpr (EPI == EPI_DGELU) {
        if (ok) {
            const uint32_t t = __builtin_nontemporal_load(reinterpret_cast<const uint32_t*>(reinterpret_cast<const unsigned char*>(p.aux_in) + (size_t)m * p.ldaux + n0));
            r.aux = make_uint2(t, 0);
        }
    }
    return r;
}

template <int EPI>
__device__ __forceinline__ void epi_store(const GemmParams& p, int m, int n0, float v0, float v1, float v2, float v3, const EpiCols& cc, const EpiRow& rr) {
    float v[4] = {v0 * p.alpha, v1 * p.alpha, v2 * p.alpha, v3 * p.alpha};
    if constexpr (EPI == EPI_ATOMIC) {
        float* c = reinterpret_cast<float*>(p.C) + (size_t)m * p.ldc + n0;
#pragma unroll
        for (int i = 0; i < 4; ++i) unsafeAtomicAdd(c + i, v[i]);
        return;
    }
    if constexpr (EPI == EPI_PARTIAL) {
        const size_t slice = (size_t)p.M * p.N + (p.colsum ? (size_t)p.cs_parts * p.M : 0);
        float* dst = p.ws + p.zslice * slice + (size_t)m * p.N + n0;
        *reinterpret_cast<float4*>(dst) = make_float4(v[0], v[1], v[2], v[3]);
        return;
    }
    v[0] += cc.bias.x; v[1] += cc.bias.y; v[2] += cc.bias.z; v[3] += cc.bias.w;
    if constexpr (EPI == EPI_BF16) {
        *reinterpret_cast<uint2*>(reinterpret_cast<bf16_t*>(p.C) + (size_t)m * p.ldc + n0) =
            make_uint2(pack_bf16x2(v[0], v[1]), pack_bf16x2(v[2], v[3]));
    } else if constexpr (EPI == EPI_F32) {
        *reinterpret_cast<float4*>(reinterpret_cast<float*>(p.C) + (size_t)m * p.ldc + n0) = make_float4(v[0], v[1], v[2], v[3]);
    } else if constexpr (EPI == EPI_GELU) {
        ppf_float2 g01, d01, g23, d23;
        gelu_erf_both2(ppf_float2{v[0], v[1]}, g01, d01);
        gelu_erf_both2(ppf_float2{v[2], v[3]}, g23, d23);
        const float g[4] = {g01.x, g01.y, g23.x, g23.y}, d[4] = {d01.x, d01.y, d23.x, d23.y};
        __builtin_nontemporal_store(gelu8_pack4(d[0], d[1], d[2], d[3]), reinterpret_cast<uint32_t*>(reinterpret_cast<unsigned char*>(p.aux_out) + (size_t)m * p.ldaux + n0));
        *reinterpret_cast<uint2*>(reinterpret_cast<bf16_t*>(p.C) + (size_t)m * p.ldc + n0) = make_uint2(pack_bf16x2(g[0], g[1]), pack_bf16x2(g[2], g[3]));
    } else if constexpr (EPI == EPI_SIGMOID_F32) {
#pragma unroll
        for (int i = 0; i < 4; ++i) v[i] = 1.0f / (1.0f + __expf(-v[i]));
        *reinterpret_cast<float4*>(reinterpret_cast<float*>(p.C) + (size_t)m * p.ldc + n0) = make_float4(v[0], v[1], v[2], v[3]);
    } else if constexpr (EPI == EPI_RESID) {
        if (p.aux_out)
            *reinterpret_cast<uint2*>(p.aux_out + (size_t)m * p.ldaux + n0) = make_uint2(pack_bf16x2(v[0], v[1]), pack_bf16x2(v[2], v[3]));
        const float s = rr.rowscale;
        *reinterpret_cast<float4*>(reinterpret_cast<float*>(p.C) + (size_t)m * p.ldc + n0) =
            make_float4(rr.res.x + v[0] * cc.colscale.x * s, rr.res.y + v[1] * cc.colscale.y * s, rr.res.z + v[2] * cc.colscale.z * s,
                        rr.res.w + v[3] * cc.colscale.w * s);
    } else if constexpr (EPI == EPI_DGELU) {
        float hd[4];
        gelu8_unpack4(rr.aux.x, hd);
        *reinterpret_cast<uint2*>(reinterpret_cast<bf16_t*>(p.C) + (size_t)m * p.ldc + n0) =
            make_uint2(pack_bf16x2(v[0] * hd[0], v[1] * hd[1]), pack_bf16x2(v[2] * hd[2], v[3] * hd[3]));
    }
}

template <int EPI> struct EpiWide { static constexpr bool value = (EPI == EPI_BF16 || EPI == EPI_GELU || EPI == EPI_DGELU); };
struct EpiCols8 { float4 bias[2]; };
struct EpiRow8 { uint4 aux; };

template <int EPI>
__device__ __forceinline__ EpiCols8 epi_load_cols8(const GemmParams& p, int n0, bool ok) {
    EpiCols8 c;
    c.bias[0] = c.bias[1] = make_float4(0.f, 0.f, 0.f, 0.f);
    if (ok && p.bias) { c.bias[0] = *reinterpret_cast<const float4*>(p.bias + n0); c.bias[1] = *reinterpret_cast<const float4*>(p.bias + n0 + 4); }
    return c;
}
template <int EPI>
__device__ __forceinline__ EpiRow8 epi_load_row8(const GemmParams& p, int m, int n0, bool ok) {
    EpiRow8 r;
    r.aux = make_uint4(0, 0, 0, 0);
    if constexpr (EPI == EPI_DGELU) {
        if (ok) {
            typedef uint32_t u32x2 __attribute__((ext_vector_type(2)));
            const u32x2 t = __builtin_nontemporal_load(reinterpret_cast<const u32x2*>(reinterpret_cast<const unsigned char*>(p.aux_in) + (size_t)m * p.ldaux + n0));
            r.aux = make_uint4(t.x, t.y, 0, 0);
        }
    }
    return r;
}
template <int EPI>
__device__ __forceinline__ void epi_store8(const GemmParams& p, int m, int n0, const float4& a, const float4& b, const EpiCols8& cc, const EpiRow8& rr) {
    typedef uint32_t u32x4 __attribute__((ext_vector_type(4)));
    float v[8] = {a.x * p.alpha + cc.bias[0].x, a.y * p.alpha + cc.bias[0].y, a.z * p.alpha + cc.bias[0].z, a.w * p.alpha + cc.bias[0].w,
                  b.x * p.alpha + cc.bias[1].x, b.y * p.alpha + cc.bias[1].y, b.z * p.alpha + cc.bias[1].z, b.w * p.alpha + cc.bias[1].w};
    bf16_t* dst = reinterpret_cast<bf16_t*>(p.C) + (size_t)m * p.ldc + n0;
    if constexpr (EPI == EPI_BF16) {
        *reinterpret_cast<uint4*>(dst) = make_uint4(pack_bf16x2(v[0], v[1]), pack_bf16x2(v[2], v[3]), pack_bf16x2(v[4], v[5]), pack_bf16x2(v[6], v[7]));
    } else if constexpr (EPI == EPI_GELU) {
        ppf_float2 g[4], d[4];
#pragma unroll
        for (int i = 0; i < 4; ++i) gelu_erf_both2(ppf_float2{v[2 * i], v[2 * i + 1]}, g[i], d[i]);
        typedef uint32_t u32x2 __attribute__((ext_vector_type(2)));
        const u32x2 dv = {gelu8_pack4(d[0].x, d[0].y, d[1].x, d[1].y), gelu8_pack4(d[2].x, d[2].y, d[3].x, d[3].y)};
        __builtin_nontemporal_store(dv, reinterpret_cast<u32x2*>(reinterpret_cast<unsigned char*>(p.aux_out) + (size_t)m * p.ldaux + n0));
        *reinterpret_cast<uint4*>(dst) = make_uint4(pack_bf16x2(g[0].x, g[0].y), pack_bf16x2(g[1].x, g[1].y), pack_bf16x2(g[2].x, g[2].y), pack_bf16x2(g[3].x, g[3].y));
    } else if constexpr (EPI == EPI_DGELU) {
        float ha[4], hb[4];
        gelu8_unpack4(rr.aux.x, ha);
        gelu8_unpack4(rr.aux.y, hb);
        *reinterpret_cast<uint4*>(dst) = make_uint4(pack_bf16x2(v[0] * ha[0], v[1] * ha[1]), pack_bf16x2(v[2] * ha[2], v[3] * ha[3]),
                                                    pack_bf16x2(v[4] * hb[0], v[5] * hb[1]), pack_bf16x2(v[6] * hb[2], v[7] * hb[3]));
    }
}


}
```

protopformer_amd/csrc/layernorm.hip:

```cpp
#include "ppf_common.h"
#include "ppf_hip.h"
#include <cstdlib>
#include <type_traits>

namespace {

constexpr int WAVES = 4;
constexpr int MAXJ = 8;

template <int NJ>
__global__ __launch_bounds__(256) void ln_fwd_kernel(const float* __restrict__ x, const int* __restrict__ row_map,
                                                     const float* __restrict__ w, const float* __restrict__ b,
                                                     bf16_t* __restrict__ y, float* __restrict__ mean_out,
                                                     float* __restrict__ rstd_out, int rows, int D, float eps) {
    const int lane = threadIdx.x & 63, wave = threadIdx.x >> 6;
    float2 wv[NJ], bv[NJ];
#pragma unroll
    for (int j = 0; j < NJ; ++j) {
        const int c = 2 * lane + 128 * j;
        wv[j] = c < D ? *reinterpret_cast<const float2*>(w + c) : make_float2(0.f, 0.f);
        bv[j] = c < D ? *reinterpret_cast<const float2*>(b + c) : make_float2(0.f, 0.f);
    }
    const float invD = 1.0f / (float)D;
    for (int r = blockIdx.x * WAVES + wave; r < rows; r += gridDim.x * WAVES) {
        const size_t src = row_map ? (size_t)row_map[r] : (size_t)r;
        const float* xr = x + src * D;
        float2 v[NJ];
        float s = 0.f;
#pragma unroll
        for (int j = 0; j < NJ; ++j) {
            const int c = 2 * lane + 128 * j;
            v[j] = c < D ? *reinterpret_cast<const float2*>(xr + c) : make_float2(0.f, 0.f);
            s += v[j].x + v[j].y;
        }
        const float mu = wave_sum(s) * invD;
        float q = 0.f;
#pragma unroll
        for (int j = 0; j < NJ; ++j) {
            const int c = 2 * lane + 128 * j;
            if (c < D) { const float a = v[j].x - mu, bb = v[j].y - mu; q += a * a + bb * bb; }
        }
        const float rs = rsqrtf(wave_sum(q) * invD + eps);
        bf16_t* yr = y + (size_t)r * D;
#pragma unroll
        for (int j = 0; j < NJ; ++j) {
            const int c = 2 * lane + 128 * j;
            if (c < D)
                *reinterpret_cast<uint32_t*>(yr + c) =
                    pack_bf16x2((v[j].x - mu) * rs * wv[j].x + bv[j].x, (v[j].y - mu) * rs * wv[j].y + bv[j].y);
        }
        if (lane == 0) { mean_out[r] = mu; rstd_out[r] = rs; }
    }
}

struct LnBwdParams {
    const bf16_t* dy; const float* x; const int* row_map; const float* w; const float* mean; const float* rstd;
    const float* dres_in; float* dx_out; float* dw; float* db;
    bf16_t* cast_out; const float* rowscale; int rows_per_group; const float* colscale; float* dbias_next;
    const bf16_t* branch; float* dcolscale;
    int rows, D;
    float* partial;
};

template <int NJ>
__global__ __launch_bounds__(256) void ln_bwd_kernel(const LnBwdParams p) {
    __shared__ float red[WAVES][NJ * 2 * 64];
    const int lane = threadIdx.x & 63, wave = threadIdx.x >> 6;
    const int D = p.D;
    float2 wv[NJ], cs[NJ];
    float2 adw[NJ], adb[NJ], anb[NJ], acs[NJ];
#pragma unroll
    for (int j = 0; j < NJ; ++j) {
        const int c = 2 * lane + 128 * j;
        wv[j] = (p.dy && c < D) ? *reinterpret_cast<const float2*>(p.w + c) : make_float2(0.f, 0.f);
        cs[j] = (p.colscale && c < D) ? *reinterpret_cast<const float2*>(p.colscale + c) : make_float2(1.f, 1.f);
        adw[j] = adb[j] = anb[j] = acs[j] = make_float2(0.f, 0.f);
    }
    const float invD = 1.0f / (float)D;
    for (int r = blockIdx.x * WAVES + wave; r < p.rows; r += gridDim.x * WAVES) {
        const size_t src = p.row_map ? (size_t)p.row_map[r] : (size_t)r;
        float2 dx[NJ];
#pragma unroll
        for (int j = 0; j < NJ; ++j) {
            const int c = 2 * lane + 128 * j;
            dx[j] = (p.dres_in && c < D) ? *reinterpret_cast<const float2*>(p.dres_in + src * D + c) : make_float2(0.f, 0.f);
        }
        if (p.dy) {
            const float mu = p.mean[r], rs = p.rstd[r];
            float2 xh[NJ], g[NJ];
            float s1 = 0.f, s2 = 0.f;
#pragma unroll
            for (int j = 0; j < NJ; ++j) {
                const int c = 2 * lane + 128 * j;
                if (c < D) {
                    const float2 xv = *reinterpret_cast<const float2*>(p.x + src * D + c);
                    const float2 dyv = unpack_bf16x2(*reinterpret_cast<const uint32_t*>(p.dy + (size_t)r * D + c));
                    xh[j] = make_float2((xv.x - mu) * rs, (xv.y - mu) * rs);
                    g[j] = make_float2(dyv.x * wv[j].x, dyv.y * wv[j].y);
                    s1 += g[j].x + g[j].y;
                    s2 += g[j].x * xh[j].x + g[j].y * xh[j].y;
                    adw[j].x += dyv.x * xh[j].x; adw[j].y += dyv.y * xh[j].y;
                    adb[j].x += dyv.x; adb[j].y += dyv.y;
                } else {
                    xh[j] = g[j] = make_float2(0.f, 0.f);
                }
            }
            const float c1 = wave_sum(s1) * invD, c2 = wave_sum(s2) * invD;
#pragma unroll
            for (int j = 0; j < NJ; ++j) {
                dx[j].x += rs * (g[j].x - c1 - xh[j].x * c2);
                dx[j].y += rs * (g[j].y - c1 - xh[j].y * c2);
            }
        }
        const float rsc = p.rowscale ? p.rowscale[src / p.rows_per_group] : 1.0f;
#pragma unroll
        for (int j = 0; j < NJ; ++j) {
            const int c = 2 * lane + 128 * j;
            if (c < D) {
                if (p.dx_out) *reinterpret_cast<float2*>(p.dx_out + src * D + c) = dx[j];
                if (p.cast_out) {
                    const float sx = dx[j].x * rsc, sy = dx[j].y * rsc;
                    if (p.branch) {
                        const float2 br = unpack_bf16x2(*reinterpret_cast<const uint32_t*>(p.branch + src * D + c));
                        acs[j].x += sx * br.x; acs[j].y += sy * br.y;
                    }
                    const uint32_t pk = pack_bf16x2(sx * cs[j].x, sy * cs[j].y);
                    *reinterpret_cast<uint32_t*>(p.cast_out + src * D + c) = pk;
                    const float2 rt = unpack_bf16x2(pk);
                    anb[j].x += rt.x; anb[j].y += rt.y;
                }
            }
        }
    }
    auto flush = [&](float2 (&a)[NJ], float* dst, int which) {
        if (!dst) return;
        float* part = p.partial ? p.partial + ((size_t)blockIdx.x * 4 + which) * D : nullptr;
        __syncthreads();
#pragma unroll
        for (int j = 0; j < NJ; ++j) { red[wave][(j * 64 + lane) * 2] = a[j].x; red[wave][(j * 64 + lane) * 2 + 1] = a[j].y; }
        __syncthreads();
        for (int i = threadIdx.x; i < NJ * 128; i += 256) {
            const int j = i >> 7, rem = i & 127, l = rem >> 1, e = rem & 1;
            const int c = 2 * l + 128 * j + e;
            if (c < D) {
                float s = 0.f;
#pragma unroll
                for (int wv_ = 0; wv_ < WAVES; ++wv_) s += red[wv_][i];
                if (part) part[c] = s; else unsafeAtomicAdd(dst + c, s);
            }
        }
    };
    if (p.dy) { flush(adw, p.dw, 0); flush(adb, p.db, 1); }
    if (p.cast_out) { flush(anb, p.dbias_next, 2); if (p.branch) flush(acs, p.dcolscale, 3); }
}

template <int V, int NJ, bool LS>
__global__ __launch_bounds__(256) void ln_bwd2_kernel(const LnBwdParams p) {
    __shared__ float red[WAVES][NJ * V * 32];
    const int lane = threadIdx.x & 63, wave = threadIdx.x >> 6, l32 = lane & 31, half = lane >> 5;
    const int D = p.D;
    float wv[NJ][V], cs[NJ][V], adw[NJ][V], adb[NJ][V], anb[NJ][V], acs[NJ][V];
#pragma unroll
    for (int j = 0; j < NJ; ++j)
#pragma unroll
        for (int e = 0; e < V; ++e) {
            const int c = V * l32 + 32 * V * j + e;
            wv[j][e] = p.dy ? p.w[c] : 0.f;
            cs[j][e] = (LS && p.colscale) ? p.colscale[c] : 1.f;
            adw[j][e] = adb[j][e] = anb[j][e] = acs[j][e] = 0.f;
        }
    const float invD = 1.0f / (float)D;
    for (int r0 = (blockIdx.x * WAVES + wave) * 2; r0 < p.rows; r0 += gridDim.x * WAVES * 2) {
        const int r = r0 + half;
        const bool ok = r < p.rows;
        const size_t src = ok ? (p.row_map ? (size_t)p.row_map[r] : (size_t)r) : 0;
        float dx[NJ][V];
#pragma unroll
        for (int j = 0; j < NJ; ++j) {
            const int c = V * l32 + 32 * V * j;
            if (p.dres_in && ok) {
                if constexpr (V == 4) { const float4 t = *reinterpret_cast<const float4*>(p.dres_in + src * D + c); dx[j][0] = t.x; dx[j][1] = t.y; dx[j][2] = t.z; dx[j][3] = t.w; }
                else { const float2 t = *reinterpret_cast<const float2*>(p.dres_in + src * D + c); dx[j][0] = t.x; dx[j][1] = t.y; }
            } else {
#pragma unroll
                for (int e = 0; e < V; ++e) dx[j][e] = 0.f;
            }
        }
        if (p.dy) {
            const float mu = ok ? p.mean[r] : 0.f, rs = ok ? p.rstd[r] : 0.f;
            float xh[NJ][V], g[NJ][V];
            float s1 = 0.f, s2 = 0.f;
#pragma unroll
            for (int j = 0; j < NJ; ++j) {
                const int c = V * l32 + 32 * V * j;
                float xv[V], dyv[V];
                if (ok) {
                    if constexpr (V == 4) {
                        const float4 t = *reinterpret_cast<const float4*>(p.x + src * D + c); xv[0] = t.x; xv[1] = t.y; xv[2] = t.z; xv[3] = t.w;
                        const uint2 u = *reinterpret_cast<const uint2*>(p.dy + (size_t)r * D + c);
                        const float2 a = unpack_bf16x2(u.x), b = unpack_bf16x2(u.y); dyv[0] = a.x; dyv[1] = a.y; dyv[2] = b.x; dyv[3] = b.y;
                    } else {
                        const float2 t = *reinterpret_cast<const float2*>(p.x + src * D + c); xv[0] = t.x; xv[1] = t.y;
                        const float2 a = unpack_bf16x2(*reinterpret_cast<const uint32_t*>(p.dy + (size_t)r * D + c)); dyv[0] = a.x; dyv[1] = a.y;
                    }
                } else {
#pragma unroll
                    for (int e = 0; e < V; ++e) { xv[e] = 0.f; dyv[e] = 0.f; }
                }
#pragma unroll
                for (int e = 0; e < V; ++e) {
                    xh[j][e] = (xv[e] - mu) * rs;
                    g[j][e] = dyv[e] * wv[j][e];
                    s1 += g[j][e];
                    s2 += g[j][e] * xh[j][e];
                    adw[j][e] += dyv[e] * xh[j][e];
                    adb[j][e] += dyv[e];
                }
            }
#pragma unroll
            for (int o = 16; o > 0; o >>= 1) { s1 += __shfl_xor(s1, o, 64); s2 += __shfl_xor(s2, o, 64); }
            const float c1 = s1 * invD, c2 = s2 * invD;
#pragma unroll
            for (int j = 0; j < NJ; ++j)
#pragma unroll
                for (int e = 0; e < V; ++e) dx[j][e] += rs * (g[j][e] - c1 - xh[j][e] * c2);
        }
        if (!ok) continue;
        const float rsc = p.rowscale ? p.rowscale[src / p.rows_per_group] : 1.0f;
#pragma unroll
        for (int j = 0; j < NJ; ++j) {
            const int c = V * l32 + 32 * V * j;
            if (p.dx_out) {
                if constexpr (V == 4) *reinterpret_cast<float4*>(p.dx_out + src * D + c) = make_float4(dx[j][0], dx[j][1], dx[j][2], dx[j][3]);
                else *reinterpret_cast<float2*>(p.dx_out + src * D + c) = make_float2(dx[j][0], dx[j][1]);
            }
            if (p.cast_out) {
                float sx[V];
#pragma unroll
                for (int e = 0; e < V; ++e) sx[e] = dx[j][e] * rsc;
                if (LS && p.branch) {
                    float br[V];
                    if constexpr (V == 4) {
                        const uint2 u = *reinterpret_cast<const uint2*>(p.branch + src * D + c);
                        const float2 a = unpack_bf16x2(u.x), b = unpack_bf16x2(u.y); br[0] = a.x; br[1] = a.y; br[2] = b.x; br[3] = b.y;
                    } else {
                        const float2 a = unpack_bf16x2(*reinterpret_cast<const uint32_t*>(p.branch + src * D + c)); br[0] = a.x; br[1] = a.y;
                    }
#pragma unroll
                    for (int e = 0; e < V; ++e) acs[j][e] += sx[e] * br[e];
                }
                uint32_t pk[V / 2];
#pragma unroll
                for (int e = 0; e < V; e += 2) {
                    pk[e / 2] = LS ? pack_bf16x2(sx[e] * cs[j][e], sx[e + 1] * cs[j][e + 1]) : pack_bf16x2(sx[e], sx[e + 1]);
                    const float2 rt = unpack_bf16x2(pk[e / 2]);
                    anb[j][e] += rt.x; anb[j][e + 1] += rt.y;
                }
                if constexpr (V == 4) *reinterpret_cast<uint2*>(p.cast_out + src * D + c) = make_uint2(pk[0], pk[1]);
                else *reinterpret_cast<uint32_t*>(p.cast_out + src * D + c) = pk[0];
            }
        }
    }
    auto flush = [&](float (&a)[NJ][V], float* dst, int which) {
        if (!dst) return;
        float* part = p.partial ? p.partial + ((size_t)blockIdx.x * 4 + which) * D : nullptr;
        __syncthreads();
#pragma unroll
        for (int j = 0; j < NJ; ++j)
#pragma unroll
            for (int e = 0; e < V; ++e) {
                const float v = a[j][e] + __shfl_xor(a[j][e], 32, 64);
                if (half == 0) red[wave][(j * 32 + l32) * V + e] = v;
            }
        __syncthreads();
        for (int i = threadIdx.x; i < NJ * V * 32; i += 256) {
            float s = 0.f;
#pragma unroll
            for (int w_ = 0; w_ < WAVES; ++w_) s += red[w_][i];
            const int j = i / (32 * V), rem = i % (32 * V);
            if (part) part[32 * V * j + rem] = s;
            else unsafeAtomicAdd(dst + 32 * V * j + rem, s);
        }
    };
    if (p.dy) { flush(adw, p.dw, 0); flush(adb, p.db, 1); }
    if (p.cast_out) { flush(anb, p.dbias_next, 2); if (LS && p.branch) flush(acs, p.dcolscale, 3); }
}

constexpr int LN_RS = 16;
__global__ __launch_bounds__(1024) void ln_colsum_reduce_kernel(const float* __restrict__ partial, int nblocks, int D, float* d0, float* d1,
                                                                  float* d2, float* d3) {
    __shared__ float red[16][64];
    const int which = blockIdx.y;
    float* dst = which == 0 ? d0 : which == 1 ? d1 : which == 2 ? d2 : d3;
    if (!dst) return;
    const int cl = threadIdx.x & 63, g = threadIdx.x >> 6, c = blockIdx.x * 64 + cl;
    float s = 0.f;
    if (c < D) {
#pragma unroll 8
        for (int b = g; b < nblocks; b += 16) s += partial[((size_t)b * 4 + which) * D + c];
    }
    red[g][cl] = s;
    __syncthreads();
    if (g == 0 && c < D) {
        float t = 0.f;
#pragma unroll
        for (int i = 0; i < 16; ++i) t += red[i][cl];
        dst[c] += t;
    }
}

int ln_bwd_grid(int rows) {
    constexpr int cap = 1024;
    const int g = (rows + WAVES * 8 - 1) / (WAVES * 8);
    return g < cap ? g : cap;
}

template <typename F>
int dispatch_nj(int D, F&& f) {
    const int nj = (D + 127) / 128;
    switch (nj) {
        case 1: return f(std::integral_constant<int, 1>());
        case 2: return f(std::integral_constant<int, 2>());
        case 3: return f(std::integral_constant<int, 3>());
        case 4: return f(std::integral_constant<int, 4>());
        case 6: return f(std::integral_constant<int, 6>());
        case 8: return f(std::integral_constant<int, 8>());
        default: break;
    }
    ppf_set_error("layernorm: unsupported width D=%d (need D even, ceil(D/128) in {1,2,3,4,6,8})", D);
    return PPF_ERR_SHAPE;
}

}

extern "C" {

int ppf_layernorm_fwd(const float* x, const int* row_map, const float* w, const float* b, void* y, float* mean, float* rstd,
                      int rows, int D, float eps, hipStream_t stream) {
    PPF_CHECK_ARG(rows > 0 && D > 0 && (D % 2) == 0 && D <= 128 * MAXJ, PPF_ERR_SHAPE, "ppf_layernorm_fwd: bad shape rows=%d D=%d", rows, D);
    const int grid = min((rows + WAVES - 1) / WAVES, 256 * 16);
    return dispatch_nj(D, [&](auto nj) {
        hipLaunchKernelGGL((ln_fwd_kernel<decltype(nj)::value>), dim3(grid), dim3(256), 0, stream, x, row_map, w, b, (bf16_t*)y, mean, rstd, rows, D, eps);
        PPF_LAUNCH_CHECK();
        return 0;
    });
}

int ppf_layernorm_bwd(const void* dy, const float* x, const int* row_map, const float* w, const float* mean, const float* rstd,
                      const float* dres_in, float* dx_out, float* dw, float* db, void* cast_out, const float* rowscale,
                      int rows_per_group, const float* colscale, float* dbias_next, const void* branch, float* dcolscale,
                      int rows, int D, float* partial, size_t partial_bytes, hipStream_t stream) {
    PPF_CHECK_ARG(rows > 0 && D > 0 && (D % 2) == 0 && D <= 128 * MAXJ, PPF_ERR_SHAPE, "ppf_layernorm_bwd: bad shape rows=%d D=%d", rows, D);
    PPF_CHECK_ARG(dy != nullptr || dres_in != nullptr, PPF_ERR_ARG, "ppf_layernorm_bwd: need dy or dres_in");
    LnBwdParams p;
    p.dy = (const bf16_t*)dy; p.x = x; p.row_map = row_map; p.w = w; p.mean = mean; p.rstd = rstd; p.dres_in = dres_in; p.dx_out = dx_out;
    p.dw = dw; p.db = db; p.cast_out = (bf16_t*)cast_out; p.rowscale = rowscale; p.rows_per_group = rows_per_group > 0 ? rows_per_group : 1;
    p.colscale = colscale; p.dbias_next = dbias_next; p.branch = (const bf16_t*)branch; p.dcolscale = dcolscale; p.rows = rows; p.D = D;
    const int grid = ln_bwd_grid(rows);
    PPF_CHECK_ARG(partial == nullptr || partial_bytes >= (size_t)(grid + LN_RS) * 4 * D * sizeof(float), PPF_ERR_ARG,
                  "ppf_layernorm_bwd: partial-sum workspace needs ppf_layernorm_bwd_blocks(rows)*4*D*4 = %zu bytes", (size_t)(grid + LN_RS) * 4 * D * sizeof(float));
    p.partial = partial;
    const bool ls = colscale != nullptr || branch != nullptr || dcolscale != nullptr;
#define PPF_LN2(V, NJ) { if (ls) hipLaunchKernelGGL((ln_bwd2_kernel<V, NJ, true>), dim3(grid), dim3(256), 0, stream, p); \
                         else hipLaunchKernelGGL((ln_bwd2_kernel<V, NJ, false>), dim3(grid), dim3(256), 0, stream, p); \
                         PPF_LAUNCH_CHECK(); return 0; }
    if (D % 128 == 0 && D <= 512) { switch (D / 128) { case 1: PPF_LN2(4, 1) case 2: PPF_LN2(4, 2) case 3: PPF_LN2(4, 3) case 4: PPF_LN2(4, 4) } }
    if (D % 64 == 0 && D <= 512) { switch (D / 64) { case 1: PPF_LN2(2, 1) case 3: PPF_LN2(2, 3) case 5: PPF_LN2(2, 5) case 7: PPF_LN2(2, 7) } }
#undef PPF_LN2
    return dispatch_nj(D, [&](auto nj) {
        hipLaunchKernelGGL((ln_bwd_kernel<decltype(nj)::value>), dim3(grid), dim3(256), 0, stream, p);
        PPF_LAUNCH_CHECK();
        return 0;
    });
}

int ppf_layernorm_bwd_blocks(int rows) { return ln_bwd_grid(rows) + LN_RS; }

int ppf_layernorm_bwd_reduce(const float* partial, int rows, int D, float* dw, float* db, float* dbias_next, float* dcolscale, hipStream_t stream) {
    PPF_CHECK_ARG(partial && rows > 0 && D > 0, PPF_ERR_ARG, "ppf_layernorm_bwd_reduce: bad arguments");
    const int nb = ln_bwd_grid(rows);
    hipLaunchKernelGGL(ln_colsum_reduce_kernel, dim3((D + 63) / 64, 4), dim3(1024), 0, stream, partial, nb, D, dw, db, dbias_next, dcolscale);
    PPF_LAUNCH_CHECK();
    return 0;
}

}
```

protopformer_amd/ops.py:

```python
import os

import torch

from . import _lib

EPI_BF16, EPI_F32, EPI_GELU, EPI_SIGMOID_F32, EPI_RESID, EPI_DGELU, EPI_ATOMIC = range(7)


DOMINANT_NAME = ("weight-gradient bf16 MFMA GEMM, split over the contraction, ordered partial tiles: wgrad8_kernel<4,2> / <2,4> (256x128 / 128x256 tiles) "
                 "and gemm_kernel<TA=1,TB=1,EPI_PARTIAL,COLSUM> (128x128)")


_WORKSPACE = {}
_GEMM_WS = {}
_RETIRED_WS = []


def _workspace(device, nbytes, pool=_WORKSPACE):
    key = (device, _lib.stream_ptr())
    buf = pool.get(key)
    if buf is None or buf.numel() < nbytes:
        if buf is not None:
            _RETIRED_WS.append(buf)
        buf = torch.empty(max(nbytes, 64 << 20), dtype=torch.uint8, device=device)
        pool[key] = buf
    return buf


def _chk(t, dtype=None):
    assert t.is_cuda and t.is_contiguous(), "kernel operands must be contiguous CUDA tensors"
    if dtype is not None:
        assert t.dtype == dtype, f"expected {dtype}, got {t.dtype}"
    return t


def gemm(a, b, *, trans_a=False, trans_b=False, epi=EPI_BF16, out=None, bias=None, res=None, rowscale=None,
         rows_per_group=1, colscale=None, aux_in=None, aux_out=None, colsum=None, alpha=1.0, lda=None, ldb=None, workspace=True):
    _chk(a, torch.bfloat16), _chk(b, torch.bfloat16)
    lda = a.shape[1] if lda is None else lda
    ldb = b.shape[1] if ldb is None else ldb
    M, K = (a.shape[1], a.numel() // lda) if trans_a else (a.numel() // lda, a.shape[1])
    N, Kb = (b.shape[1], b.numel() // ldb) if trans_b else (b.numel() // ldb, b.shape[1])
    assert K == Kb, f"contraction mismatch {K} vs {Kb}"
    if out is None:
        odt = torch.float32 if epi in (EPI_F32, EPI_SIGMOID_F32, EPI_RESID, EPI_ATOMIC) else torch.bfloat16
        out = torch.empty((M, N), dtype=odt, device=a.device)
        if epi == EPI_ATOMIC:
            zero_(out)
    ldaux = 0
    for t in (aux_in, aux_out):
        if t is not None:
            _chk(t, torch.uint8 if epi in (EPI_GELU, EPI_DGELU) else torch.bfloat16)
            ldaux = t.shape[-1]
    ws = None
    if epi == EPI_ATOMIC and workspace:
        ws = _workspace(a.device, _lib.lib().ppf_gemm_workspace_bytes(M, N, K), _GEMM_WS)
    _lib.call("ppf_gemm_bf16", a, b, out, M, N, K, lda, ldb, out.shape[-1], int(trans_a), int(trans_b), epi,
              bias, res, res.shape[-1] if res is not None else 0, rowscale, rows_per_group, colscale, aux_in, aux_out, ldaux,
              colsum, float(alpha), ws, ws.numel() if ws is not None else 0)
    return out


def rowgemm_ok(D, K, rows_per_tile):
    return bool(_lib.lib().ppf_rowgemm_supported(int(D), int(K), int(rows_per_tile)))


_CU_COUNT = {}


def rowgemm_tile_rows(M, rows_per_sample, device=None, backward=False):
    dev = torch.cuda.current_device() if device is None else device
    cus = _CU_COUNT.get(dev)
    if cus is None:
        cus = _CU_COUNT[dev] = torch.cuda.get_device_properties(dev).multi_processor_count
    tiles = (M + rows_per_sample - 1) // rows_per_sample
    if 3 * tiles > 2 * cus or rows_per_sample <= 16:
        return rows_per_sample
    half = (rows_per_sample + 1) // 2
    if backward:
        target = max(1, int(0.62 * cus))
        return max(half, min(rows_per_sample, (M + target - 1) // target))
    return half


def rowgemm_bf16(a, b, rows_per_tile, bias=None):
    _chk(a, torch.bfloat16), _chk(b, torch.bfloat16)
    M, K = a.shape
    D = b.shape[0]
    out = torch.empty((M, D), dtype=torch.bfloat16, device=a.device)
    _lib.call("ppf_rowgemm_bf16", a, b, M, D, K, K, b.shape[1], rows_per_tile, bias, out)
    return out


def rowgemm_resid_ln(a, b, res, rows_per_tile, bias=None, rowscale=None, rows_per_group=1, ln_w=None, ln_b=None, eps=1e-6, colscale=None, aux_out=None):
    _chk(a, torch.bfloat16), _chk(b, torch.bfloat16), _chk(res, torch.float32)
    M, K = a.shape
    D = b.shape[0]
    xout = torch.empty((M, D), dtype=torch.float32, device=a.device)
    n = mean = rstd = None
    if ln_w is not None:
        n = torch.empty((M, D), dtype=torch.bfloat16, device=a.device)
        mean = torch.empty(M, dtype=torch.float32, device=a.device)
        rstd = torch.empty(M, dtype=torch.float32, device=a.device)
    _lib.call("ppf_rowgemm_resid_ln", a, b, M, D, K, K, b.shape[1], rows_per_tile, bias, res, xout, rowscale, rows_per_group, colscale, aux_out,
              ln_w, ln_b, n, mean, rstd, float(eps))
    return xout, n, mean, rstd


def rowgemm_lnbwd(a, b, x, mean, rstd, w, dw, db, rows_per_tile, dres_in=None, dx_out=None, cast_out=None, rowscale=None, rows_per_group=1,
                  lane=None, defer_reduce=False, colscale=None, branch=None, dcolscale=None):
    _chk(a, torch.bfloat16), _chk(b, torch.bfloat16), _chk(x, torch.float32)
    M, K = a.shape
    D = b.shape[0]
    tiles = (M + rows_per_tile - 1) // rows_per_tile
    nparts = 3 if colscale is not None else 2
    part = torch.empty(tiles * nparts * D, dtype=torch.float32, device=a.device)
    if dx_out is None:
        dx_out = torch.empty((M, D), dtype=torch.float32, device=a.device)
    _lib.call("ppf_rowgemm_lnbwd", a, b, M, D, K, K, b.shape[1], rows_per_tile, x, mean, rstd, w, dres_in, dx_out, cast_out, rowscale, rows_per_group,
              colscale, branch, part, part.numel() * 4)
    red = lambda: _lib.call("ppf_rowgemm_colsum", part, tiles, D, nparts, dw, db, dcolscale)
    if lane is not None:
        lane.submit(red, (part,), defer=defer_reduce)
    else:
        red()
    return dx_out


def transpose_bf16_batched(src, dst, desc, n, total_tiles):
    _lib.call("ppf_transpose_bf16_batched", src, dst, desc, n, total_tiles)


def layernorm_fwd(x, w, b, eps=1e-6, row_map=None):
    _chk(x, torch.float32)
    D = x.shape[-1]
    rows = row_map.numel() if row_map is not None else x.numel() // D
    y = torch.empty((rows, D), dtype=torch.bfloat16, device=x.device)
    mean = torch.empty(rows, dtype=torch.float32, device=x.device)
    rstd = torch.empty(rows, dtype=torch.float32, device=x.device)
    _lib.call("ppf_layernorm_fwd", x, row_map, w, b, y, mean, rstd, rows, D, float(eps))
    return y, mean, rstd


def layernorm_bwd(dy, x, w, mean, rstd, dw, db, *, dres_in=None, dx_out=None, row_map=None, cast_out=None, rowscale=None,
                  rows_per_group=1, colscale=None, dbias_next=None, branch=None, dcolscale=None, lane=None, defer_reduce=False):
    D = x.shape[-1] if x is not None else dres_in.shape[-1]
    if dy is not None:
        rows = dy.numel() // D
    else:
        rows = dres_in.numel() // D
    sums = (dw if dy is not None else None, db if dy is not None else None, dbias_next if cast_out is not None else None,
            dcolscale if (cast_out is not None and branch is not None) else None)
    part = None
    if any(t is not None for t in sums):
        dev = (dy if dy is not None else dres_in).device
        part = torch.empty(_lib.lib().ppf_layernorm_bwd_blocks(rows) * 4 * D, dtype=torch.float32, device=dev)
    _lib.call("ppf_layernorm_bwd", dy, x, row_map, w, mean, rstd, dres_in, dx_out, dw, db, cast_out, rowscale, rows_per_group,
              colscale, dbias_next, branch, dcolscale, rows, D, part, part.numel() * 4 if part is not None else 0)
    if part is not None:
        red = lambda: _lib.call("ppf_layernorm_bwd_reduce", part, rows, D, *sums)
        if lane is not None:
            lane.submit(red, (part,), defer=defer_reduce, tag="LNRED")
        else:
            red()


def cast_bf16(src, dst=None):
    _chk(src, torch.float32)
    n = src.numel()
    assert n % 8 == 0
    if dst is None:
        dst = torch.empty(src.shape, dtype=torch.bfloat16, device=src.device)
    _lib.call("ppf_cast_f32_bf16", src, dst, n)
    return dst


def im2col_patch(img, patch):
    _chk(img, torch.float32)
    B, C, H, W = img.shape
    cols = torch.empty((B * (H // patch) * (W // patch), C * patch * patch), dtype=torch.bfloat16, device=img.device)
    _lib.call("ppf_im2col_patch", img, cols, B, C, H, W, patch)
    return cols


def assemble_tokens(tok, cls, pos, B, Np, D, lead):
    x = torch.empty((B, Np + lead, D), dtype=torch.float32, device=tok.device)
    _lib.call("ppf_assemble_tokens", tok, cls, pos, x, B, Np, D, lead)
    return x


def assemble_tokens_bwd(dx, dpos, dcls, B, Np, D, lead):
    dtok = torch.empty((B * Np, D), dtype=torch.bfloat16, device=dx.device)
    _lib.call("ppf_assemble_tokens_bwd", dx, dtok, dpos, dcls, B, Np, D, lead)
    return dtok


def attn_fwd_hm_ok(H, N, D):
    return bool(_lib.lib().ppf_attn_fwd_hm_supported(H, N, D))


def attn_fwd(qkv, B, H, N, D, policy=None, self_keep=True, eps_n=0, headmean=None):
    _chk(qkv, torch.bfloat16)
    out = torch.empty((B * N, D), dtype=torch.bfloat16, device=qkv.device)
    rowmax = torch.empty((B, H, N), dtype=torch.float32, device=qkv.device)
    zinv = torch.empty((B, H, N), dtype=torch.float32, device=qkv.device)
    if headmean is not None:
        NP = (N + 3) // 4 * 4
        _lib.call("ppf_attn_fwd_hm", qkv, out, policy, rowmax, zinv, headmean, NP, B, H, N, D, int(self_keep), int(eps_n))
    else:
        _lib.call("ppf_attn_fwd", qkv, out, policy, rowmax, zinv, B, H, N, D, int(self_keep), int(eps_n))
    return out, rowmax, zinv


def attn_headmean(qkv, rowmax, zinv, B, H, N, D, policy=None, self_keep=True, out=None, eps_n=0):
    NP = (N + 3) // 4 * 4
    if out is None:
        out = torch.empty((B, N, NP), dtype=torch.float32, device=qkv.device)
    _lib.call("ppf_attn_headmean", qkv, policy, rowmax, zinv, out, NP, B, H, N, D, int(self_keep), int(eps_n))
    return out


def attn_bwd(qkv, out, dout, rowmax, zinv, B, H, N, D, policy=None, self_keep=True, eps_n=0):
    dqkv = torch.empty_like(qkv)
    delta = torch.empty((B, H, N), dtype=torch.float32, device=qkv.device)
    _lib.call("ppf_attn_bwd", qkv, out, dout, dqkv, policy, rowmax, zinv, delta, B, H, N, D, int(self_keep), int(eps_n))
    return dqkv


def rollout_threshold(hm_layer, thr_out, N, discard_ratio=0.9):
    B, _, NP = hm_layer.shape
    _lib.call("ppf_rollout_threshold", hm_layer, B, N, NP, int(N * N * discard_ratio), thr_out)


def rollout_outputs(B, N, k, lead, device):
    Nk = N - lead
    return (torch.empty((B, Nk), dtype=torch.float32, device=device), torch.empty((B, k), dtype=torch.int32, device=device),
            torch.empty((B, Nk + 1), dtype=torch.float32, device=device))


def rollout(hm, L, B, N, k, lead=1, init_rows=None, discard_ratio=0.9, identity=0.2, thr=None, out=None):
    _chk(hm, torch.float32)
# ... 336 lines not shown
              a1, b1, out1, N1, K1, sa1[0], sa1[1], sb1[0], sb1[1], out1.shape[-1] if out1 is not None else 0, float(alpha1),
              total, total.shape[-1] if total is not None else 0, float(c0), float(c1), M, ws, ws.numel() // 4)


def axpbypcz(x, y, z, a, b, c):
    out = torch.empty_like(x)
    _lib.call("ppf_axpbypcz", x, y, z, out, float(a), float(b), float(c), x.numel())
    return out


_CONST = {}


def const_scalar(device, value):
    key = (device, float(value))
    t = _CONST.get(key)
    if t is None:
        t = _CONST[key] = torch.full((), float(value), dtype=torch.float32, device=device)
    return t


def is_const_one(t):
    c = _CONST.get((t.device, 1.0))
    return c is not None and t.data_ptr() == c.data_ptr()


def axpby(x, y, a, b, out=None):
    if out is None:
        out = torch.empty_like(x)
    _lib.call("ppf_axpby", x, y, out, float(a), float(b), x.numel())
    return out


def topk_sorted(scores, k):
    _chk(scores, torch.float32)
    B, n = scores.shape
    idx = torch.empty((B, k), dtype=torch.int32, device=scores.device)
    _lib.call("ppf_topk_sorted", scores, B, n, k, idx)
    return idx


def sigmoid_bwd(df, f, dbias):
    rows, cols = f.shape
    dz = torch.empty((rows, cols), dtype=torch.bfloat16, device=f.device)
    part = torch.empty(_lib.lib().ppf_sigmoid_bwd_blocks(rows) * cols, dtype=torch.float32, device=f.device) if dbias is not None else None
    _lib.call("ppf_sigmoid_bwd", df, f, dz, dbias, rows, cols, part, part.numel() * 4 if part is not None else 0)
    return dz


def zeros(shape, dtype, device):
    t = torch.empty(shape, dtype=dtype, device=device)
    _lib.call("ppf_memset_zero", t, t.numel() * t.element_size())
    return t


def zero_(t):
    _lib.call("ppf_memset_zero", t, t.numel() * t.element_size())
    return t


def copy_2d(dst, src):
    assert dst.dim() == 2 and src.dim() == 2 and dst.shape == src.shape and dst.stride(1) == 1 and src.stride(1) == 1 and dst.dtype == src.dtype
    es = dst.element_size()
    _lib.call("ppf_copy_2d", dst, dst.stride(0) * es, src, src.stride(0) * es, dst.shape[1] * es, dst.shape[0])
    return dst


def cat_rows(first, rest):
    B, N, D = rest.shape
    out = torch.empty((B, N + 1, D), dtype=rest.dtype, device=rest.device)
    o2 = out.reshape(B, (N + 1) * D)
    copy_2d(o2[:, :D], first.reshape(B, D))
    copy_2d(o2[:, D:], rest.reshape(B, N * D))
    return out


def reserved_rows_map(idx, N):
    B, k = idx.shape
    rows = torch.empty(B * (k + 1), dtype=torch.int32, device=idx.device)
    _lib.call("ppf_reserved_rows_map", idx, rows, B, k, N)
    return rows


def gather_rows(src, rows):
    _chk(src)
    dst = torch.empty((rows.numel(), src.shape[1]), dtype=src.dtype, device=src.device)
    _lib.call("ppf_gather_rows", src, rows, dst, rows.numel(), src.shape[1] * src.element_size())
    return dst


def scatter_rows(src, rows, nrows_dst):
    _chk(src)
    dst = torch.empty((nrows_dst, src.shape[1]), dtype=src.dtype, device=src.device)
    _lib.call("ppf_scatter_rows", src, rows, dst, src.shape[0], nrows_dst, src.shape[1] * src.element_size())
    return dst


def droppath_draw(out, keep, seed, state):
    nslot, B = out.shape
    _lib.call("ppf_droppath_scales", out, keep, nslot, B, int(seed) & 0xFFFFFFFFFFFFFFFF, state)
    return out


def scale_by_scalar(x, scalar):
    out = torch.empty_like(x)
    _lib.call("ppf_scale_by_scalar", x, scalar, out, x.numel())
    return out


def gemm_batched(a, b, c, M, N, K, lda, ldb, ldc, trans_a, trans_b, out_f32, alpha, bo, bi, sa, sb, sc, kpad=0):
    _lib.call("ppf_gemm_bf16_batched", a, b, c, M, N, K, lda, ldb, ldc, int(trans_a), int(trans_b), int(out_f32), float(alpha), bo, bi,
              sa[0], sa[1], sb[0], sb[1], sc[0], sc[1], int(kpad))


class _Off:

    def __init__(self, t, off):
        self.t, self.off = t, off

    def data_ptr(self):
        return self.t.data_ptr() + self.off * self.t.element_size()


def th_scores(qkv, wl, bl, B, H, N, D):
    NP = (N + 3) // 4 * 4
    sp = torch.empty((B, H, N, NP), dtype=torch.float32, device=qkv.device)
    _lib.call("ppf_th_scores", qkv, wl, bl, sp, B, H, N, D, NP)
    return sp


def th_softmax_mix(sp, ww, bw, hm_out):
    B, H, N, NP = sp.shape
    NPK = (N + 7) // 8 * 8
    a16 = torch.empty((B, H, N, NPK), dtype=torch.bfloat16, device=sp.device)
    _lib.call("ppf_th_softmax_mix", sp, a16, hm_out, ww, bw, B, H, N, NP, NPK)
    return a16


def th_softmax_bwd(prob, da, ww, wl, dww, dbw, dbl):
    B, H, N, NP = prob.shape
    NPK = (N + 7) // 8 * 8
    ds16 = torch.empty((B, H, N, NPK), dtype=torch.bfloat16, device=prob.device)
    _lib.call("ppf_th_softmax_bwd", prob, da, ds16, ww, wl, dww, dbw, dbl, B, H, N, NP, NPK)
    return ds16


def th_dwl(qkv, ds_prime, dwl, B, H, N, D):
    _lib.call("ppf_th_dwl", qkv, ds_prime, dwl, B, H, N, D, ds_prime.shape[-1])


def _th_mode():
    return os.environ.get("PPF_TH_FUSED", "1")


def th_fused_ok(H, N, D):
    return _th_mode() != "0" and bool(_lib.lib().ppf_th_fused_supported(H, N, D))


def th_pv_fused():
    return _th_mode() == "1"


def th_fwd(qkv, wl, bl, ww, bw, hm_out, B, H, N, D, with_out=True):
    NP, NPK = (N + 3) // 4 * 4, (N + 7) // 8 * 8
    a16 = torch.empty((B, H, N, NPK), dtype=torch.bfloat16, device=qkv.device)
    rowmax = torch.empty((B, H, N), dtype=torch.float32, device=qkv.device)
# ... 159 lines not shown
```

Before: 17190 images/sec.

## Skip scattering zero rows at the token-reservation boundary in backward

```diff
diff --git a/include/ppf_hip.h b/include/ppf_hip.h
--- a/include/ppf_hip.h
+++ b/include/ppf_hip.h
@@ -29,6 +29,10 @@
                   int rows_per_group, const float* colscale, const void* aux_in, void* aux_out, int ldaux, float* colsum,
                   float alpha, void* workspace, size_t workspace_bytes, ppf_stream_t stream);
 size_t ppf_gemm_workspace_bytes(int M, int N, int K);
+int ppf_gemm_wgrad_masked(const void* dy, const void* x, const int* inv, void* dW, int M, int N, int K, int lda, int ldb, int ldc, float* colsum,
+                          void* workspace, size_t workspace_bytes, ppf_stream_t stream);
+int ppf_gemm_dgelu_rows(const void* A, const void* B, void* C, int M, int N, int K, int lda, int ldb, int ldc, int trans_b, const void* codes,
+                        const int* rows, int ldaux, ppf_stream_t stream);
 
 int ppf_gemm_test_force_g224(int force);
 
@@ -71,6 +75,10 @@
                       const float* dres_in, float* dx_out, float* dw, float* db, void* cast_out, const float* rowscale,
                       int rows_per_group, const float* colscale, float* dbias_next, const void* branch, float* dcolscale,
                       int rows, int D, float* partial, size_t partial_bytes, ppf_stream_t stream);
+int ppf_layernorm_bwd_masked_supported(int D);
+int ppf_layernorm_bwd_masked(const void* dy, const float* x, const int* inv, const float* w, const float* mean, const float* rstd,
+                             const float* dres_in, float* dx_out, float* dw, float* db, void* cast_out, const float* rowscale,
+                             int rows_per_group, float* dbias_next, int rows, int D, float* partial, size_t partial_bytes, ppf_stream_t stream);
 int ppf_layernorm_bwd_blocks(int rows);
 int ppf_layernorm_bwd_reduce(const float* partial, int rows, int D, float* dw, float* db, float* dbias_next, float* dcolscale,
                              ppf_stream_t stream);
@@ -194,6 +202,7 @@
                         ppf_stream_t stream);
 int ppf_droppath_scales(float* out, const float* keep, int nslot, int B, uint64_t seed, void* state_u64, ppf_stream_t stream);
 int ppf_reserved_rows_map(const int* idx, int* rows, int B, int k, int N, ppf_stream_t stream);
+int ppf_inverse_rows_map(const int* rows, int* inv, int nrows, int nrows_full, ppf_stream_t stream);
 int ppf_gather_rows(const void* src, const int* rows, void* dst, int nrows, int row_bytes, ppf_stream_t stream);
 int ppf_scatter_rows(const void* src, const int* rows, void* dst, int nrows_src, int nrows_dst, int row_bytes, ppf_stream_t stream);
 int ppf_memset_zero(void* ptr, size_t bytes, ppf_stream_t stream);
diff --git a/protopformer_amd/backbone.py b/protopformer_amd/backbone.py
--- a/protopformer_amd/backbone.py
+++ b/protopformer_amd/backbone.py
@@ -270,11 +270,12 @@
 _ROLL_BATCH = 3
 
 
-def _wgrad(store, dy16, x16, weight, bias=None, defer=False):
+def _wgrad(store, dy16, x16, weight, bias=None, defer=False, inv=None):
     gw = store.grad_view(weight)
     gb = store.grad_view(bias) if bias is not None else None
+    reads = (dy16, x16) if inv is None else (dy16, x16, inv)
     wgrad_lane(store).submit(lambda: ops.gemm(dy16, x16, trans_a=True, trans_b=True, epi=EPI_ATOMIC, out=gw.reshape(weight.shape[0], -1),
-                                              colsum=gb), (dy16, x16), defer=defer and min(weight.shape[0], weight.shape[1]) <= 256)
+                                              colsum=gb, inv=inv), reads, defer=defer and min(weight.shape[0], weight.shape[1]) <= 256)
 
 
 _DGRAD_ROW = 3
@@ -331,15 +332,15 @@
     return kw
 
 
-def mlp_bwd(store, blk, L, dyb, bias_done):
+def mlp_bwd(store, blk, L, dyb, bias_done, rows=None, inv=None):
     fc1, fc2 = blk.mlp.fc1, blk.mlp.fc2
-    _wgrad(store, dyb, L["g"], fc2.weight, None if bias_done else fc2.bias, defer=True)
+    _wgrad(store, dyb, L["g"], fc2.weight, None if bias_done else fc2.bias, defer=True, inv=inv)
     w2t = store.w16t(fc2.weight)
     if w2t is not None:
-        dh = ops.gemm(dyb, w2t, epi=EPI_DGELU, aux_in=L["h"])
+        dh = ops.gemm(dyb, w2t, epi=EPI_DGELU, aux_in=L["h"], rows=rows)
     else:
-        dh = ops.gemm(dyb, store.w16(fc2.weight), trans_b=True, epi=EPI_DGELU, aux_in=L["h"])
-    _wgrad(store, dh, L["n2"], fc1.weight, fc1.bias)
+        dh = ops.gemm(dyb, store.w16(fc2.weight), trans_b=True, epi=EPI_DGELU, aux_in=L["h"], rows=rows)
+    _wgrad(store, dh, L["n2"], fc1.weight, fc1.bias, inv=inv)
     return dh
 
 
@@ -349,40 +350,68 @@
     return rpt if covered else None
 
 
-def block_bwd(blk, store, L, dx, dyb, bias_done, below, *, next_dyb, attn_bwd, lnb, dgrad, row_tile):
+def _norm_bwd(store, lane, lnb, row_tile, dx, dy, weight, dn, x, mean, rstd, norm, out, bias_next=None):
+    gv = store.grad_view
+    nw = norm.weight
+    if row_tile is not None:
+        ops.rowgemm_lnbwd(dy, store.w16t(weight), x, mean, rstd, nw, gv(nw), gv(norm.bias), row_tile, dres_in=dx, dx_out=dx,
+                          lane=lane, defer_reduce=True, **out)
+    else:
+        lnb(dn, x, nw, mean, rstd, gv(nw), gv(norm.bias), dres_in=dx, dx_out=dx, dbias_next=gv(bias_next) if out else None, **out)
+
+
+def block_bwd_mlp_proj(blk, store, L, dx, dyb, bias_done, *, next_dyb, lnb, dgrad, row_tile):
     lane = wgrad_lane(store)
-    gv = store.grad_view
     Nl = L["N"]
-    fc1, qkv, proj = blk.mlp.fc1, blk.attn.qkv, blk.attn.proj
+    fc1, proj = blk.mlp.fc1, blk.attn.proj
     fused = row_tile is not None
-
-    def norm_bwd(dy, weight, dn, x, mean, rstd, norm, out, bias_next=None):
-        nw = norm.weight
-        if fused:
-            ops.rowgemm_lnbwd(dy, store.w16t(weight), x, mean, rstd, nw, gv(nw), gv(norm.bias), row_tile, dres_in=dx, dx_out=dx,
-                              lane=lane, defer_reduce=True, **out)
-        else:
-            lnb(dn, x, nw, mean, rstd, gv(nw), gv(norm.bias), dres_in=dx, dx_out=dx, dbias_next=gv(bias_next) if out else None, **out)
-
     dh = mlp_bwd(store, blk, L, dyb, bias_done)
     dyb = next_dyb(dyb)
     dn2 = None if fused else dgrad(dh, fc1.weight, Nl, 1)
-    norm_bwd(dh, fc1.weight, dn2, L["x1"], L["mean2"], L["rstd2"], blk.norm2, branch_out(store, dyb, L["s1"], Nl, getattr(blk, "gamma_1", None), L["raw1"]),
-             proj.bias)
+    _norm_bwd(store, lane, lnb, row_tile, dx, dh, fc1.weight, dn2, L["x1"], L["mean2"], L["rstd2"], blk.norm2,
+              branch_out(store, dyb, L["s1"], Nl, getattr(blk, "gamma_1", None), L["raw1"]), proj.bias)
     bias_done = not fused
     _wgrad(store, dyb, L["ao"], proj.weight, None if bias_done else proj.bias, defer=True)
-    dao = ops.rowgemm_bf16(dyb, store.w16t(proj.weight), row_tile) if fused else dgrad(dyb, proj.weight, Nl, 4)
+    return ops.rowgemm_bf16(dyb, store.w16t(proj.weight), row_tile) if fused else dgrad(dyb, proj.weight, Nl, 4), dyb
+
+
+def block_bwd_mlp_proj_reserved(blk, store, L, dx, dyb, bias_done, rows, rows_per_sample, *, next_dyb, lnb, dgrad):
+    fc1, proj = blk.mlp.fc1, blk.attn.proj
+    Mf = L["x1"].shape[0]
+    inv = ops.inverse_rows_map(rows, Mf)
+    dh = mlp_bwd(store, blk, L, dyb, bias_done, rows, inv)
+    dyb = next_dyb(dyb)
+    dn2 = dgrad(dh, fc1.weight, rows_per_sample, 1)
+    gv = store.grad_view
+    dx_full = torch.empty((Mf, dx.shape[1]), dtype=torch.float32, device=dx.device)
+    lnb(dn2, L["x1"], blk.norm2.weight, L["mean2"], L["rstd2"], gv(blk.norm2.weight), gv(blk.norm2.bias), dres_in=dx, dx_out=dx_full,
+        dbias_next=gv(proj.bias), inv=inv, cast_out=dyb, rowscale=L["s1"], rows_per_group=L["N"])
+    _wgrad(store, dyb, L["ao"], proj.weight, None, defer=True, inv=inv)
+    dao = ops.scatter_rows(dgrad(dyb, proj.weight, rows_per_sample, 4), rows, Mf)
+    return dx_full, dao, dyb
+
+
+def block_bwd_attn(blk, store, L, dx, dao, dyb, below, *, next_dyb, attn_bwd, lnb, dgrad, row_tile):
+    lane = wgrad_lane(store)
+    Nl = L["N"]
+    qkv = blk.attn.qkv
+    fused = row_tile is not None
     dqkv = attn_bwd(blk, L, dao)
     _wgrad(store, dqkv, L["n1"], qkv.weight, qkv.bias)
     dn1 = None if fused else dgrad(dqkv, qkv.weight, Nl, 2)
     if below is None:
-        norm_bwd(dqkv, qkv.weight, dn1, L["x"], L["mean1"], L["rstd1"], blk.norm1, {})
-        return None, bias_done
+        _norm_bwd(store, lane, lnb, row_tile, dx, dqkv, qkv.weight, dn1, L["x"], L["mean1"], L["rstd1"], blk.norm1, {})
+        return None, not fused
     prev, Lp = below
-    dyb = next_dyb(dyb)
-    norm_bwd(dqkv, qkv.weight, dn1, L["x"], L["mean1"], L["rstd1"], blk.norm1,
-             branch_out(store, dyb, Lp["s2"], Nl, getattr(prev, "gamma_2", None), Lp["raw2"]), prev.mlp.fc2.bias)
+    dyb = next_dyb(dyb) if dyb.shape[0] == dx.shape[0] else lane.track(torch.empty(dx.shape, dtype=torch.bfloat16, device=dx.device))
+    _norm_bwd(store, lane, lnb, row_tile, dx, dqkv, qkv.weight, dn1, L["x"], L["mean1"], L["rstd1"], blk.norm1,
+              branch_out(store, dyb, Lp["s2"], Nl, getattr(prev, "gamma_2", None), Lp["raw2"]), prev.mlp.fc2.bias)
     return dyb, not fused
+
+
+def block_bwd(blk, store, L, dx, dyb, bias_done, below, *, next_dyb, attn_bwd, lnb, dgrad, row_tile):
+    dao, dyb = block_bwd_mlp_proj(blk, store, L, dx, dyb, bias_done, next_dyb=next_dyb, lnb=lnb, dgrad=dgrad, row_tile=row_tile)
+    return block_bwd_attn(blk, store, L, dx, dao, dyb, below, next_dyb=next_dyb, attn_bwd=attn_bwd, lnb=lnb, dgrad=dgrad, row_tile=row_tile)
 
 
 def embed_bwd(ppnet, store, saved, dx, lead):
@@ -400,7 +429,7 @@
     lane.join()
 
 
-def deit_backward(ppnet, store, saved, df):
+def deit_backward(ppnet, store, saved, df, dense_reserved_bwd=False):
     feats = ppnet.features
     layers, head = saved["layers"], saved["head"]
     x_last = saved["x_last"]
@@ -420,20 +449,35 @@
     gs = getattr(ppnet, "_grad_sync", None)
     if gs is not None:
         chunk_ready(gs, lane, gs.tail_chunk)
-    bwd = functools.partial(block_bwd, next_dyb=dyb_ring(lane, D), lnb=lnb, dgrad=functools.partial(_dgrad, store),
-                            attn_bwd=lambda blk, L, dao: ops.attn_bwd(L["qkv"], L["ao"], dao, L["rowmax"], L["zinv"], B, feats.num_heads, L["N"], D,
-                                                                      policy=L["policy"], self_keep=True, eps_n=L["eps_n"]))
+    kw = dict(next_dyb=dyb_ring(lane, D), lnb=lnb, dgrad=functools.partial(_dgrad, store))
+    attn_bwd = lambda blk, L, dao: ops.attn_bwd(L["qkv"], L["ao"], dao, L["rowmax"], L["zinv"], B, feats.num_heads, L["N"], D,
+                                                policy=L["policy"], self_keep=True, eps_n=L["eps_n"])
+
+    def tile(blk, Nl):
+        return row_tile_bwd(store, blk, D, ops.rowgemm_tile_rows(B * Nl, Nl, backward=True)) if _row_bwd(B * Nl, D) else None
+
     bias_done = True
+    rows = None
     for i in range(len(layers) - 1, -1, -1):
-        L = layers[i]
+        L, blk = layers[i], feats.blocks[i]
         Nl = L["N"]
-        row_tile = row_tile_bwd(store, feats.blocks[i], D, ops.rowgemm_tile_rows(B * Nl, Nl, backward=True)) if _row_bwd(B * Nl, D) else None
-        dyb, bias_done = bwd(feats.blocks[i], store, L, dx, dyb, bias_done, (feats.blocks[i - 1], layers[i - 1]) if i > 0 else None,
-                             row_tile=row_tile)
+        below = (feats.blocks[i - 1], layers[i - 1]) if i > 0 else None
+        if rows is None:
+            dyb, bias_done = block_bwd(blk, store, L, dx, dyb, bias_done, below, attn_bwd=attn_bwd, row_tile=tile(blk, Nl), **kw)
+        else:
+            dx, dao, dyb = block_bwd_mlp_proj_reserved(blk, store, L, dx, dyb, bias_done, rows, layers[i + 1]["N"], **kw)
+            rows = None
+            dyb, bias_done = block_bwd_attn(blk, store, L, dx, dao, dyb, below, attn_bwd=attn_bwd, row_tile=None, **kw)
         if i > 0 and L["rows"] is not None:
-            Mf = B * layers[i - 1]["N"]
-            dx = ops.scatter_rows(dx, L["rows"], Mf)
-            dyb = lane.track(ops.scatter_rows(dyb, L["rows"], Mf))
+            prev = feats.blocks[i - 1]
+            skip_zero_rows = (not dense_reserved_bwd and getattr(prev, "gamma_1", None) is None and tile(prev, layers[i - 1]["N"]) is None
+                              and ops.layernorm_bwd_masked_ok(D))
+            if not skip_zero_rows:
+                Mf = B * layers[i - 1]["N"]
+                dx = ops.scatter_rows(dx, L["rows"], Mf)
+                dyb = lane.track(ops.scatter_rows(dyb, L["rows"], Mf))
+            else:
+                rows = L["rows"]
         if gs is not None and i in gs.block_chunk:
             chunk_ready(gs, lane, gs.block_chunk[i])
     if layers and layers[0]["rows"] is not None:
diff --git a/protopformer_amd/csrc/elementwise.hip b/protopformer_amd/csrc/elementwise.hip
--- a/protopformer_amd/csrc/elementwise.hip
+++ b/protopformer_amd/csrc/elementwise.hip
@@ -229,6 +229,10 @@
     const int b = i / (k + 1), j = i % (k + 1);
     rows[i] = b * N + (j == 0 ? 0 : 1 + idx[b * k + j - 1]);
 }
+__global__ __launch_bounds__(256) void inverse_rows_kernel(const int* __restrict__ rows, int* __restrict__ inv, int nrows) {
+    const int i = blockIdx.x * 256 + threadIdx.x;
+    if (i < nrows) inv[rows[i]] = i;
+}
 __global__ __launch_bounds__(256) void move_rows_kernel(const uint4* __restrict__ src, const int* __restrict__ rows, uint4* __restrict__ dst,
                                                         int nrows, int vec, int scatter) {
     const int64_t total = (int64_t)nrows * vec;
@@ -463,6 +467,15 @@
     return 0;
 }
 
+int ppf_inverse_rows_map(const int* rows, int* inv, int nrows, int nrows_full, hipStream_t stream) {
+    PPF_CHECK_ARG(rows && inv && nrows > 0 && nrows_full >= nrows, PPF_ERR_ARG, "ppf_inverse_rows_map: bad arguments");
+    hipError_t e = ppf_memset_async(inv, 0xff, (size_t)nrows_full * sizeof(int), stream);
+    if (e != hipSuccess) { ppf_set_error("ppf_inverse_rows_map: memset failed: %s", hipGetErrorString(e)); return (int)e; }
+    hipLaunchKernelGGL(inverse_rows_kernel, dim3((nrows + 255) / 256), dim3(256), 0, stream, rows, inv, nrows);
+    PPF_LAUNCH_CHECK();
+    return 0;
+}
+
 int ppf_gather_rows(const void* src, const int* rows, void* dst, int nrows, int row_bytes, hipStream_t stream) {
     PPF_CHECK_ARG(nrows > 0 && row_bytes > 0 && row_bytes % 16 == 0, PPF_ERR_ALIGN, "ppf_gather_rows: row_bytes=%d must be a positive multiple of 16", row_bytes);
     hipLaunchKernelGGL(move_rows_kernel, dim3(grid_for((int64_t)nrows * (row_bytes / 16))), dim3(256), 0, stream, (const uint4*)src, rows, (uint4*)dst,
diff --git a/protopformer_amd/csrc/gemm_bf16.hip b/protopformer_amd/csrc/gemm_bf16.hip
--- a/protopformer_amd/csrc/gemm_bf16.hip
+++ b/protopformer_amd/csrc/gemm_bf16.hip
@@ -21,14 +21,15 @@
 
 typedef uint32_t u32x4 __attribute__((ext_vector_type(4)));
 
-template <bool T, int ROWS, int NTHR = NTHREADS>
+template <bool T, int ROWS, int NTHR = NTHREADS, int MASK = 0>
 struct TileIO {
+    static_assert(T || MASK == 0, "the row mask applies to the contraction-strided storage mode");
     static constexpr int NLD = ROWS * 8 / NTHR;
     static constexpr int RPP = NTHR / 8;
     static constexpr int CPR = ROWS / 8;
     static constexpr int KPP = NTHR / CPR;
     static __device__ __forceinline__ unsigned gload(u32x4 (&reg)[NLD], const bf16_t* __restrict__ X, int ld, int R, int row0,
-                                                     int k0, int kend, int tid, int kpad) {
+                                                     int k0, int kend, int tid, int kpad, const int* __restrict__ map = nullptr) {
         unsigned mask = 0;
         if constexpr (!T) {
             const int c16 = tid & 7, rb = tid >> 3;
@@ -49,9 +50,16 @@
 #pragma unroll
             for (int i = 0; i < NLD; ++i) {
                 const int kc = k0 + kb + KPP * i;
-                const bf16_t* src = X + (size_t)min(kc, kend - 1) * ld + cc;
+                int kr = min(kc, kend - 1);
+                bool live = true;
+                if constexpr (MASK != 0) {
+                    const int c = map[kr];
+                    live = c >= 0;
+                    kr = live ? (MASK == 1 ? c : kr) : 0;
+                }
+                const bf16_t* src = X + (size_t)kr * ld + cc;
                 reg[i] = *reinterpret_cast<const u32x4*>(src);
-                mask |= (cok && kc < kend) ? (1u << i) : 0u;
+                mask |= (cok && kc < kend && live) ? (1u << i) : 0u;
             }
         }
         return mask;
@@ -167,14 +175,14 @@
     p.ws[p.zslice * ((size_t)p.M * p.N + (size_t)p.cs_parts * p.M) + (size_t)p.M * p.N + m] = v;
 }
 
-template <bool TA, bool TB, int EPI, bool COLSUM>
+template <bool TA, bool TB, int EPI, bool COLSUM, bool MAPB = false>
 __global__ __launch_bounds__(NTHREADS, 3) void gemm_kernel(const GemmParams p_) {
     constexpr int PD = 1, MT = 2;
     extern __shared__ __attribute__((aligned(16))) unsigned char smem[];
     constexpr int TBM = 64 * MT;
     constexpr int A_BYTES = TBM * BK * 2;
-    using IOA = TileIO<TA, TBM>;
-    using IOB = TileIO<TB, BN>;
+    using IOA = TileIO<TA, TBM, NTHREADS, MAPB ? 1 : 0>;
+    using IOB = TileIO<TB, BN, NTHREADS, MAPB ? 2 : 0>;
     const int tid = threadIdx.x, lane = tid & 63, wave = tid >> 6;
     const int wm = (wave & 1) * (32 * MT), wn = (wave >> 1) * 64;
 
@@ -220,8 +228,8 @@
 #pragma unroll
     for (int st = 0; st < PD; ++st) {
         const int k0 = min(kbeg + st * BK, kbeg + (nk - 1) * BK);
-        ma[st] = IOA::gload(ra[st], p.A, p.lda, p.M, m0, k0, kend, tid, p.kpad);
-        mb[st] = IOB::gload(rb[st], p.B, p.ldb, p.N, n0, k0, kend, tid, p.kpad);
+        ma[st] = IOA::gload(ra[st], p.A, p.lda, p.M, m0, k0, kend, tid, p.kpad, p.rowmap);
+        mb[st] = IOB::gload(rb[st], p.B, p.ldb, p.N, n0, k0, kend, tid, p.kpad, p.rowmap);
     }
     IOA::sstore(ra[0], ma[0], tA, tid);
     IOB::sstore(rb[0], mb[0], tB, tid);
@@ -234,8 +242,8 @@
             if (kt >= nk) break;
             {
                 const int k0 = kbeg + min(kt + PD, nk - 1) * BK;
-                ma[u] = IOA::gload(ra[u], p.A, p.lda, p.M, m0, k0, kend, tid, p.kpad);
-                mb[u] = IOB::gload(rb[u], p.B, p.ldb, p.N, n0, k0, kend, tid, p.kpad);
+                ma[u] = IOA::gload(ra[u], p.A, p.lda, p.M, m0, k0, kend, tid, p.kpad, p.rowmap);
+                mb[u] = IOB::gload(rb[u], p.B, p.ldb, p.N, n0, k0, kend, tid, p.kpad, p.rowmap);
             }
 #pragma unroll
             for (int ks = 0; ks < BK / 16; ++ks) {
@@ -282,12 +290,12 @@
     }
 }
 
-template <int WMW, int WNW, bool COLSUM>
+template <int WMW, int WNW, bool COLSUM, bool MAPB = false>
 __global__ __launch_bounds__(64 * WMW * WNW, 1) void wgrad8_kernel(const GemmParams p_) {
     extern __shared__ __attribute__((aligned(16))) unsigned char smem[];
     constexpr int NTHR = 64 * WMW * WNW, TBM = 64 * WMW, TBN = 64 * WNW;
-    using IOA = TileIO<true, TBM, NTHR>;
-    using IOB = TileIO<true, TBN, NTHR>;
+    using IOA = TileIO<true, TBM, NTHR, MAPB ? 1 : 0>;
+    using IOB = TileIO<true, TBN, NTHR, MAPB ? 2 : 0>;
     const int tid = threadIdx.x, lane = tid & 63;
     const int wave = __builtin_amdgcn_readfirstlane(tid >> 6);
     const int wm = (wave % WMW) * 64, wn = (wave / WMW) * 64;
@@ -321,16 +329,16 @@
     const bool do_colsum = COLSUM && p.colsum != nullptr && n0 == 0 && wn == 0;
     unsigned char* tA = smem;
     unsigned char* tB = smem + TBM * BK * 2;
-    ma = IOA::gload(ra, p.A, p.lda, p.M, m0, kbeg, kend, tid, 0);
-    mb = IOB::gload(rb, p.B, p.ldb, p.N, n0, kbeg, kend, tid, 0);
+    ma = IOA::gload(ra, p.A, p.lda, p.M, m0, kbeg, kend, tid, 0, p.rowmap);
+    mb = IOB::gload(rb, p.B, p.ldb, p.N, n0, kbeg, kend, tid, 0, p.rowmap);
     IOA::sstore(ra, ma, tA, tid);
     IOB::sstore(rb, mb, tB, tid);
     __syncthreads();
     for (int kt = 0; kt < nk; ++kt) {
         {
             const int k0 = kbeg + min(kt + 1, nk - 1) * BK;
-            ma = IOA::gload(ra, p.A, p.lda, p.M, m0, k0, kend, tid, 0);
-            mb = IOB::gload(rb, p.B, p.ldb, p.N, n0, k0, kend, tid, 0);
+            ma = IOA::gload(ra, p.A, p.lda, p.M, m0, k0, kend, tid, 0, p.rowmap);
+            mb = IOB::gload(rb, p.B, p.ldb, p.N, n0, k0, kend, tid, 0, p.rowmap);
         }
 #pragma unroll
         for (int ks = 0; ks < BK / 16; ++ks) {
@@ -370,13 +378,13 @@
     }
 }
 
-template <int WMW, int WNW>
+template <int WMW, int WNW, bool MAPB = false>
 int launch_wgrad8(const GemmParams& p, int splitk, hipStream_t stream) {
     constexpr int NTHR = 64 * WMW * WNW, TBM = 64 * WMW, TBN = 64 * WNW;
     constexpr int opnd = (TBM + TBN) * BK * 2, strips = (NTHR / 64) * 32 * STAGE_LD * 4;
     constexpr int lds = opnd > strips ? opnd : strips;
     const int tiles = ((p.M + TBM - 1) / TBM) * ((p.N + TBN - 1) / TBN);
-    return ppf_launch<wgrad8_kernel<WMW, WNW, true>>(dim3(tiles * splitk), dim3(NTHR), lds, stream, "wgrad8", p);
+    return ppf_launch<wgrad8_kernel<WMW, WNW, true, MAPB>>(dim3(tiles * splitk), dim3(NTHR), lds, stream, "wgrad8", p);
 }
 
 typedef __attribute__((address_space(3))) void g4_lds_t;
@@ -546,13 +554,13 @@
            (long long)p.N * p.ldb < (1ll << 30) && (long long)((p.M + BM - 1) / BM) * ((p.N + BN - 1) / BN) >= 512;
 }
 
-template <bool TA, bool TB, int EPI, bool COLSUM>
+template <bool TA, bool TB, int EPI, bool COLSUM, bool MAPB = false>
 int launch(const GemmParams& p, int splitk, hipStream_t stream, int nbatch = 1) {
     const int tiles = ((p.M + BM - 1) / BM) * ((p.N + BN - 1) / BN);
     constexpr int lds = 2 * TILE_BYTES > STAGE_BYTES ? 2 * TILE_BYTES : STAGE_BYTES;
     GemmParams q = p;
     q.nsplit = splitk;
-    return ppf_launch<gemm_kernel<TA, TB, EPI, COLSUM>>(dim3(tiles * splitk, nbatch, 1), dim3(NTHREADS), lds, stream, "gemm", q);
+    return ppf_launch<gemm_kernel<TA, TB, EPI, COLSUM, MAPB>>(dim3(tiles * splitk, nbatch, 1), dim3(NTHREADS), lds, stream, "gemm", q);
 }
 
 __global__ __launch_bounds__(256) void splitk_reduce_kernel(const float* __restrict__ ws, float* __restrict__ C, float* __restrict__ colsum,
@@ -618,10 +626,10 @@
     return PPF_GEMM_COUNTER_BYTES + (size_t)pick_splitk(M, N, K) * ((size_t)M * N + M) * sizeof(float);
 }
 
-int ppf_gemm_bf16(const void* A, const void* B, void* C, int M, int N, int K, int lda, int ldb, int ldc, int trans_a,
-                  int trans_b, int epi, const float* bias, const float* res, int ldres, const float* rowscale,
-                  int rows_per_group, const float* colscale, const void* aux_in, void* aux_out, int ldaux, float* colsum,
-                  float alpha, void* workspace, size_t workspace_bytes, hipStream_t stream) {
+static int gemm_run(const void* A, const void* B, void* C, int M, int N, int K, int lda, int ldb, int ldc, int trans_a,
+                    int trans_b, int epi, const float* bias, const float* res, int ldres, const float* rowscale,
+                    int rows_per_group, const float* colscale, const void* aux_in, void* aux_out, int ldaux, float* colsum,
+                    float alpha, void* workspace, size_t workspace_bytes, const int* rowmap, hipStream_t stream) {
     PPF_CHECK_ARG(M > 0 && N > 0 && K > 0, PPF_ERR_SHAPE, "ppf_gemm_bf16: bad shape M=%d N=%d K=%d", M, N, K);
     PPF_CHECK_ARG((lda % 8) == 0 && (ldb % 8) == 0 && (ldc % 4) == 0 && (N % 4) == 0, PPF_ERR_ALIGN,
                   "ppf_gemm_bf16: lda/ldb must be multiples of 8, ldc and N of 4 (lda=%d ldb=%d ldc=%d N=%d)", lda, ldb, ldc, N);
@@ -636,23 +644,30 @@
     p.bias = bias; p.res = res; p.ldres = ldres; p.rowscale = rowscale; p.rows_per_group = rows_per_group > 0 ? rows_per_group : 1;
     p.colscale = colscale; p.aux_in = (const bf16_t*)aux_in; p.aux_out = (bf16_t*)aux_out; p.ldaux = ldaux; p.colsum = colsum; p.alpha = alpha; p.ws = nullptr;
     p.batch_inner = 1; p.sa_o = p.sa_i = p.sb_o = p.sb_i = p.sc_o = p.sc_i = 0; p.kpad = 0; p.cs_parts = 1; p.nsplit = 1;
+    p.rowmap = rowmap;
+    const bool mapped = rowmap != nullptr;
+    PPF_CHECK_ARG(!mapped || epi == EPI_DGELU || (epi == EPI_ATOMIC && trans_a && trans_b), PPF_ERR_ARG,
+                  "ppf_gemm_bf16: a row map is instantiated for the weight-gradient form and the dGELU epilogue only");
     if (epi == EPI_RESID) PPF_CHECK_ARG(res != nullptr, PPF_ERR_ARG, "ppf_gemm_bf16: epi=4 needs a residual");
     if (epi == EPI_GELU) PPF_CHECK_ARG(aux_out != nullptr, PPF_ERR_ARG, "ppf_gemm_bf16: epi=2 needs aux_out");
     if (epi == EPI_DGELU) PPF_CHECK_ARG(aux_in != nullptr, PPF_ERR_ARG, "ppf_gemm_bf16: epi=5 needs aux_in");
     int rc;
     if (!trans_a && !trans_b) {
+        if (mapped) return g4_eligible(p) ? launch_g4<EPI_DGELU_MAP>(p, stream) : launch<false, false, EPI_DGELU_MAP, false>(p, 1, stream);
         if (g224_eligible(p, epi)) return launch_g224(p, stream);
         const auto g4 = [&](auto e) { return launch_g4<decltype(e)::value>(p, stream); };
         const auto nt = [&](auto e) { return launch<false, false, decltype(e)::value, false>(p, 1, stream); };
         if (g4_eligible(p) && dispatch_epi<EPI_BF16, EPI_GELU, EPI_RESID, EPI_DGELU>(epi, rc, g4)) return rc;
         if (dispatch_epi<EPI_BF16, EPI_F32, EPI_GELU, EPI_SIGMOID_F32, EPI_RESID, EPI_DGELU>(epi, rc, nt)) return rc;
     } else if (!trans_a && trans_b) {
+        if (mapped) return launch<false, true, EPI_DGELU_MAP, false>(p, 1, stream);
         const auto nn = [&](auto e) { return launch<false, true, decltype(e)::value, false>(p, 1, stream); };
         if (dispatch_epi<EPI_BF16, EPI_F32, EPI_DGELU>(epi, rc, nn)) return rc;
     } else if (epi == EPI_ATOMIC) {
         const int ns = pick_splitk(M, N, K);
         const size_t need = PPF_GEMM_COUNTER_BYTES + (size_t)ns * ((size_t)M * N + M) * sizeof(float);
-        if (workspace == nullptr || workspace_bytes < need || ns == 1) return launch<true, true, EPI_ATOMIC, true>(p, ns, stream);
+        if (workspace == nullptr || workspace_bytes < need || ns == 1)
+            return mapped ? launch<true, true, EPI_ATOMIC, true, true>(p, ns, stream) : launch<true, true, EPI_ATOMIC, true>(p, ns, stream);
         p.ws = (float*)((unsigned char*)workspace + PPF_GEMM_COUNTER_BYTES);
         p.cs_parts = 1;
         p.nsplit = ns;
@@ -663,9 +678,9 @@
             e1 = ev.second;
         }
         const bool wide = (M < N ? M : N) >= 320;
-        if (wide && M >= 512 && M >= N && (M % 256 == 0 || M >= 1024)) rc = launch_wgrad8<4, 2>(p, ns, stream);
-        else if (wide && N >= 512 && (N % 256 == 0 || N >= 1024)) rc = launch_wgrad8<2, 4>(p, ns, stream);
-        else rc = launch<true, true, EPI_PARTIAL, true>(p, ns, stream);
+        if (wide && M >= 512 && M >= N && (M % 256 == 0 || M >= 1024)) rc = mapped ? launch_wgrad8<4, 2, true>(p, ns, stream) : launch_wgrad8<4, 2>(p, ns, stream);
+        else if (wide && N >= 512 && (N % 256 == 0 || N >= 1024)) rc = mapped ? launch_wgrad8<2, 4, true>(p, ns, stream) : launch_wgrad8<2, 4>(p, ns, stream);
+        else rc = mapped ? launch<true, true, EPI_PARTIAL, true, true>(p, ns, stream) : launch<true, true, EPI_PARTIAL, true>(p, ns, stream);
         if (rc) return rc;
         if (e1) {
             (void)hipEventRecord(e1, stream);
@@ -682,6 +697,28 @@
     }
     ppf_set_error("ppf_gemm_bf16: combination trans_a=%d trans_b=%d epi=%d not instantiated", trans_a, trans_b, epi);
     return PPF_ERR_ARG;
+}
+
+int ppf_gemm_bf16(const void* A, const void* B, void* C, int M, int N, int K, int lda, int ldb, int ldc, int trans_a,
+                  int trans_b, int epi, const float* bias, const float* res, int ldres, const float* rowscale,
+                  int rows_per_group, const float* colscale, const void* aux_in, void* aux_out, int ldaux, float* colsum,
+                  float alpha, void* workspace, size_t workspace_bytes, hipStream_t stream) {
+    return gemm_run(A, B, C, M, N, K, lda, ldb, ldc, trans_a, trans_b, epi, bias, res, ldres, rowscale, rows_per_group, colscale, aux_in, aux_out,
+                    ldaux, colsum, alpha, workspace, workspace_bytes, nullptr, stream);
+}
+
+int ppf_gemm_wgrad_masked(const void* dy, const void* x, const int* inv, void* dW, int M, int N, int K, int lda, int ldb, int ldc, float* colsum,
+                          void* workspace, size_t workspace_bytes, hipStream_t stream) {
+    PPF_CHECK_ARG(inv != nullptr, PPF_ERR_ARG, "ppf_gemm_wgrad_masked: null row mask");
+    return gemm_run(dy, x, dW, M, N, K, lda, ldb, ldc, 1, 1, EPI_ATOMIC, nullptr, nullptr, 0, nullptr, 1, nullptr, nullptr, nullptr, 0, colsum, 1.0f,
+                    workspace, workspace_bytes, inv, stream);
+}
+
+int ppf_gemm_dgelu_rows(const void* A, const void* B, void* C, int M, int N, int K, int lda, int ldb, int ldc, int trans_b, const void* codes,
+                        const int* rows, int ldaux, hipStream_t stream) {
+    PPF_CHECK_ARG(rows != nullptr, PPF_ERR_ARG, "ppf_gemm_dgelu_rows: null row map");
+    return gemm_run(A, B, C, M, N, K, lda, ldb, ldc, 0, trans_b, EPI_DGELU, nullptr, nullptr, 0, nullptr, 1, nullptr, codes, nullptr, ldaux, nullptr, 1.0f,
+                    nullptr, 0, rows, stream);
 }
 
 int ppf_gemm_probe(int enable) {
@@ -710,6 +747,7 @@
     p.A = (const bf16_t*)A; p.B = (const bf16_t*)B; p.C = C; p.M = M; p.N = N; p.K = K; p.lda = lda; p.ldb = ldb; p.ldc = ldc;
     p.bias = nullptr; p.res = nullptr; p.ldres = 0; p.rowscale = nullptr; p.rows_per_group = 1; p.colscale = nullptr; p.aux_in = nullptr;
     p.aux_out = nullptr; p.ldaux = 0; p.colsum = nullptr; p.ws = nullptr; p.alpha = alpha;
+    p.rowmap = nullptr;
     p.batch_inner = batch_inner; p.sa_o = sa_o; p.sa_i = sa_i; p.sb_o = sb_o; p.sb_i = sb_i; p.sc_o = sc_o; p.sc_i = sc_i; p.kpad = kpad;
     const int nb = batch_outer * batch_inner;
     const auto go = [&](auto ta, auto tb) {
diff --git a/protopformer_amd/csrc/gemm_common.h b/protopformer_amd/csrc/gemm_common.h
--- a/protopformer_amd/csrc/gemm_common.h
+++ b/protopformer_amd/csrc/gemm_common.h
@@ -3,7 +3,8 @@
 
 namespace ppfg {
 
-enum Epi { EPI_BF16 = 0, EPI_F32 = 1, EPI_GELU = 2, EPI_SIGMOID_F32 = 3, EPI_RESID = 4, EPI_DGELU = 5, EPI_ATOMIC = 6, EPI_PARTIAL = 7 };
+enum Epi { EPI_BF16 = 0, EPI_F32 = 1, EPI_GELU = 2, EPI_SIGMOID_F32 = 3, EPI_RESID = 4, EPI_DGELU = 5, EPI_ATOMIC = 6, EPI_PARTIAL = 7,
+           EPI_DGELU_MAP = 8 };
 
 struct GemmParams {
     const bf16_t* A; const bf16_t* B; void* C;
@@ -26,7 +27,10 @@
     int nsplit;
     int cs_parts;
     int kpad;
+    const int* rowmap;
 };
+
+template <int EPI> struct EpiIsDgelu { static constexpr bool value = (EPI == EPI_DGELU || EPI == EPI_DGELU_MAP); };
 
 constexpr float GELU8_ZERO = 26.0f, GELU8_STEP = 1.0f / 196.0f, GELU8_INV = 196.0f;
 __device__ __forceinline__ uint32_t gelu8_pack4(float a, float b, float c, float d) {
@@ -68,9 +72,10 @@
             r.res = *reinterpret_cast<const float4*>(p.res + (size_t)m * p.ldres + n0);
             if (p.rowscale) r.rowscale = p.rowscale[m / p.rows_per_group];
         }
-    } else if constexpr (EPI == EPI_DGELU) {
+    } else if constexpr (EpiIsDgelu<EPI>::value) {
         if (ok) {
-            const uint32_t t = __builtin_nontemporal_load(reinterpret_cast<const uint32_t*>(reinterpret_cast<const unsigned char*>(p.aux_in) + (size_t)m * p.ldaux + n0));
+            const size_t ma = EPI == EPI_DGELU_MAP ? (size_t)p.rowmap[m] : (size_t)m;
+            const uint32_t t = __builtin_nontemporal_load(reinterpret_cast<const uint32_t*>(reinterpret_cast<const unsigned char*>(p.aux_in) + ma * p.ldaux + n0));
             r.aux = make_uint2(t, 0);
         }
     }
@@ -116,7 +121,7 @@
         *reinterpret_cast<float4*>(reinterpret_cast<float*>(p.C) + (size_t)m * p.ldc + n0) =
             make_float4(rr.res.x + v[0] * cc.colscale.x * s, rr.res.y + v[1] * cc.colscale.y * s, rr.res.z + v[2] * cc.colscale.z * s,
                         rr.res.w + v[3] * cc.colscale.w * s);
-    } else if constexpr (EPI == EPI_DGELU) {
+    } else if constexpr (EpiIsDgelu<EPI>::value) {
         float hd[4];
         gelu8_unpack4(rr.aux.x, hd);
         *reinterpret_cast<uint2*>(reinterpret_cast<bf16_t*>(p.C) + (size_t)m * p.ldc + n0) =
@@ -124,7 +129,7 @@
     }
 }
 
-template <int EPI> struct EpiWide { static constexpr bool value = (EPI == EPI_BF16 || EPI == EPI_GELU || EPI == EPI_DGELU); };
+template <int EPI> struct EpiWide { static constexpr bool value = (EPI == EPI_BF16 || EPI == EPI_GELU || EPI == EPI_DGELU || EPI == EPI_DGELU_MAP); };
 struct EpiCols8 { float4 bias[2]; };
 struct EpiRow8 { uint4 aux; };
 
@@ -139,10 +144,11 @@
 __device__ __forceinline__ EpiRow8 epi_load_row8(const GemmParams& p, int m, int n0, bool ok) {
     EpiRow8 r;
     r.aux = make_uint4(0, 0, 0, 0);
-    if constexpr (EPI == EPI_DGELU) {
+    if constexpr (EpiIsDgelu<EPI>::value) {
         if (ok) {
             typedef uint32_t u32x2 __attribute__((ext_vector_type(2)));
-            const u32x2 t = __builtin_nontemporal_load(reinterpret_cast<const u32x2*>(reinterpret_cast<const unsigned char*>(p.aux_in) + (size_t)m * p.ldaux + n0));
+            const size_t ma = EPI == EPI_DGELU_MAP ? (size_t)p.rowmap[m] : (size_t)m;
+            const u32x2 t = __builtin_nontemporal_load(reinterpret_cast<const u32x2*>(reinterpret_cast<const unsigned char*>(p.aux_in) + ma * p.ldaux + n0));
             r.aux = make_uint4(t.x, t.y, 0, 0);
         }
     }
@@ -164,7 +170,7 @@
         const u32x2 dv = {gelu8_pack4(d[0].x, d[0].y, d[1].x, d[1].y), gelu8_pack4(d[2].x, d[2].y, d[3].x, d[3].y)};
         __builtin_nontemporal_store(dv, reinterpret_cast<u32x2*>(reinterpret_cast<unsigned char*>(p.aux_out) + (size_t)m * p.ldaux + n0));
         *reinterpret_cast<uint4*>(dst) = make_uint4(pack_bf16x2(g[0].x, g[0].y), pack_bf16x2(g[1].x, g[1].y), pack_bf16x2(g[2].x, g[2].y), pack_bf16x2(g[3].x, g[3].y));
-    } else if constexpr (EPI == EPI_DGELU) {
+    } else if constexpr (EpiIsDgelu<EPI>::value) {
         float ha[4], hb[4];
         gelu8_unpack4(rr.aux.x, ha);
         gelu8_unpack4(rr.aux.y, hb);
diff --git a/protopformer_amd/csrc/layernorm.hip b/protopformer_amd/csrc/layernorm.hip
--- a/protopformer_amd/csrc/layernorm.hip
+++ b/protopformer_amd/csrc/layernorm.hip
@@ -60,6 +60,7 @@
     const bf16_t* branch; float* dcolscale;
     int rows, D;
     float* partial;
+    const int* inv;
 };
 
 template <int NJ>
@@ -154,7 +155,7 @@
     if (p.cast_out) { flush(anb, p.dbias_next, 2); if (p.branch) flush(acs, p.dcolscale, 3); }
 }
 
-template <int V, int NJ, bool LS>
+template <int V, int NJ, bool LS, bool IM = false>
 __global__ __launch_bounds__(256) void ln_bwd2_kernel(const LnBwdParams p) {
     __shared__ float red[WAVES][NJ * V * 32];
     const int lane = threadIdx.x & 63, wave = threadIdx.x >> 6, l32 = lane & 31, half = lane >> 5;
@@ -174,34 +175,37 @@
         const int r = r0 + half;
         const bool ok = r < p.rows;
         const size_t src = ok ? (p.row_map ? (size_t)p.row_map[r] : (size_t)r) : 0;
+        const int ci = IM ? (ok ? p.inv[r] : -1) : 0;
+        const bool live = IM ? ci >= 0 : ok;
+        const size_t cr = IM ? (size_t)max(ci, 0) : src, cy = IM ? cr : (size_t)r;
         float dx[NJ][V];
 #pragma unroll
         for (int j = 0; j < NJ; ++j) {
             const int c = V * l32 + 32 * V * j;
-            if (p.dres_in && ok) {
-                if constexpr (V == 4) { const float4 t = *reinterpret_cast<const float4*>(p.dres_in + src * D + c); dx[j][0] = t.x; dx[j][1] = t.y; dx[j][2] = t.z; dx[j][3] = t.w; }
-                else { const float2 t = *reinterpret_cast<const float2*>(p.dres_in + src * D + c); dx[j][0] = t.x; dx[j][1] = t.y; }
+            if (p.dres_in && live) {
+                if constexpr (V == 4) { const float4 t = *reinterpret_cast<const float4*>(p.dres_in + cr * D + c); dx[j][0] = t.x; dx[j][1] = t.y; dx[j][2] = t.z; dx[j][3] = t.w; }
+                else { const float2 t = *reinterpret_cast<const float2*>(p.dres_in + cr * D + c); dx[j][0] = t.x; dx[j][1] = t.y; }
             } else {
 #pragma unroll
                 for (int e = 0; e < V; ++e) dx[j][e] = 0.f;
             }
         }
         if (p.dy) {
-            const float mu = ok ? p.mean[r] : 0.f, rs = ok ? p.rstd[r] : 0.f;
+            const float mu = live ? p.mean[r] : 0.f, rs = live ? p.rstd[r] : 0.f;
             float xh[NJ][V], g[NJ][V];
             float s1 = 0.f, s2 = 0.f;
 #pragma unroll
             for (int j = 0; j < NJ; ++j) {
                 const int c = V * l32 + 32 * V * j;
                 float xv[V], dyv[V];
-                if (ok) {
+                if (live) {
                     if constexpr (V == 4) {
                         const float4 t = *reinterpret_cast<const float4*>(p.x + src * D + c); xv[0] = t.x; xv[1] = t.y; xv[2] = t.z; xv[3] = t.w;
-                        const uint2 u = *reinterpret_cast<const uint2*>(p.dy + (size_t)r * D + c);
+                        const uint2 u = *reinterpret_cast<const uint2*>(p.dy + cy * D + c);
                         const float2 a = unpack_bf16x2(u.x), b = unpack_bf16x2(u.y); dyv[0] = a.x; dyv[1] = a.y; dyv[2] = b.x; dyv[3] = b.y;
                     } else {
                         const float2 t = *reinterpret_cast<const float2*>(p.x + src * D + c); xv[0] = t.x; xv[1] = t.y;
-                        const float2 a = unpack_bf16x2(*reinterpret_cast<const uint32_t*>(p.dy + (size_t)r * D + c)); dyv[0] = a.x; dyv[1] = a.y;
+                        const float2 a = unpack_bf16x2(*reinterpret_cast<const uint32_t*>(p.dy + cy * D + c)); dyv[0] = a.x; dyv[1] = a.y;
                     }
                 } else {
 #pragma unroll
@@ -234,7 +238,7 @@
                 if constexpr (V == 4) *reinterpret_cast<float4*>(p.dx_out + src * D + c) = make_float4(dx[j][0], dx[j][1], dx[j][2], dx[j][3]);
                 else *reinterpret_cast<float2*>(p.dx_out + src * D + c) = make_float2(dx[j][0], dx[j][1]);
             }
-            if (p.cast_out) {
+            if (p.cast_out && live) {
                 float sx[V];
 #pragma unroll
                 for (int e = 0; e < V; ++e) sx[e] = dx[j][e] * rsc;
@@ -256,8 +260,8 @@
                     const float2 rt = unpack_bf16x2(pk[e / 2]);
                     anb[j][e] += rt.x; anb[j][e + 1] += rt.y;
                 }
-                if constexpr (V == 4) *reinterpret_cast<uint2*>(p.cast_out + src * D + c) = make_uint2(pk[0], pk[1]);
-                else *reinterpret_cast<uint32_t*>(p.cast_out + src * D + c) = pk[0];
+                if constexpr (V == 4) *reinterpret_cast<uint2*>(p.cast_out + cr * D + c) = make_uint2(pk[0], pk[1]);
+                else *reinterpret_cast<uint32_t*>(p.cast_out + cr * D + c) = pk[0];
             }
         }
     }
@@ -335,6 +339,10 @@
 
 extern "C" {
 
+int ppf_layernorm_bwd_masked_supported(int D) {
+    return D > 0 && D <= 512 && (D % 128 == 0 || (D % 64 == 0 && (D / 64 == 1 || D / 64 == 3 || D / 64 == 5 || D / 64 == 7)));
+}
+
 int ppf_layernorm_fwd(const float* x, const int* row_map, const float* w, const float* b, void* y, float* mean, float* rstd,
                       int rows, int D, float eps, hipStream_t stream) {
     PPF_CHECK_ARG(rows > 0 && D > 0 && (D % 2) == 0 && D <= 128 * MAXJ, PPF_ERR_SHAPE, "ppf_layernorm_fwd: bad shape rows=%d D=%d", rows, D);
@@ -346,7 +354,7 @@
     });
 }
 
-int ppf_layernorm_bwd(const void* dy, const float* x, const int* row_map, const float* w, const float* mean, const float* rstd,
+static int ln_bwd_run(const void* dy, const float* x, const int* row_map, const int* inv, const float* w, const float* mean, const float* rstd,
                       const float* dres_in, float* dx_out, float* dw, float* db, void* cast_out, const float* rowscale,
                       int rows_per_group, const float* colscale, float* dbias_next, const void* branch, float* dcolscale,
                       int rows, int D, float* partial, size_t partial_bytes, hipStream_t stream) {
@@ -356,12 +364,16 @@
     p.dy = (const bf16_t*)dy; p.x = x; p.row_map = row_map; p.w = w; p.mean = mean; p.rstd = rstd; p.dres_in = dres_in; p.dx_out = dx_out;
     p.dw = dw; p.db = db; p.cast_out = (bf16_t*)cast_out; p.rowscale = rowscale; p.rows_per_group = rows_per_group > 0 ? rows_per_group : 1;
     p.colscale = colscale; p.dbias_next = dbias_next; p.branch = (const bf16_t*)branch; p.dcolscale = dcolscale; p.rows = rows; p.D = D;
+    p.inv = inv;
+    const bool im = inv != nullptr;
+    PPF_CHECK_ARG(!im || ppf_layernorm_bwd_masked_supported(D), PPF_ERR_SHAPE, "ppf_layernorm_bwd_masked: unsupported width D=%d", D);
     const int grid = ln_bwd_grid(rows);
     PPF_CHECK_ARG(partial == nullptr || partial_bytes >= (size_t)(grid + LN_RS) * 4 * D * sizeof(float), PPF_ERR_ARG,
                   "ppf_layernorm_bwd: partial-sum workspace needs ppf_layernorm_bwd_blocks(rows)*4*D*4 = %zu bytes", (size_t)(grid + LN_RS) * 4 * D * sizeof(float));
     p.partial = partial;
     const bool ls = colscale != nullptr || branch != nullptr || dcolscale != nullptr;
-#define PPF_LN2(V, NJ) { if (ls) hipLaunchKernelGGL((ln_bwd2_kernel<V, NJ, true>), dim3(grid), dim3(256), 0, stream, p); \
+#define PPF_LN2(V, NJ) { if (im) hipLaunchKernelGGL((ln_bwd2_kernel<V, NJ, false, true>), dim3(grid), dim3(256), 0, stream, p); \
+                         else if (ls) hipLaunchKernelGGL((ln_bwd2_kernel<V, NJ, true>), dim3(grid), dim3(256), 0, stream, p); \
                          else hipLaunchKernelGGL((ln_bwd2_kernel<V, NJ, false>), dim3(grid), dim3(256), 0, stream, p); \
                          PPF_LAUNCH_CHECK(); return 0; }
     if (D % 128 == 0 && D <= 512) { switch (D / 128) { case 1: PPF_LN2(4, 1) case 2: PPF_LN2(4, 2) case 3: PPF_LN2(4, 3) case 4: PPF_LN2(4, 4) } }
@@ -374,6 +386,22 @@
     });
 }
 
+int ppf_layernorm_bwd(const void* dy, const float* x, const int* row_map, const float* w, const float* mean, const float* rstd,
+                      const float* dres_in, float* dx_out, float* dw, float* db, void* cast_out, const float* rowscale,
+                      int rows_per_group, const float* colscale, float* dbias_next, const void* branch, float* dcolscale,
+                      int rows, int D, float* partial, size_t partial_bytes, hipStream_t stream) {
+    return ln_bwd_run(dy, x, row_map, nullptr, w, mean, rstd, dres_in, dx_out, dw, db, cast_out, rowscale, rows_per_group, colscale, dbias_next,
+                      branch, dcolscale, rows, D, partial, partial_bytes, stream);
+}
+
+int ppf_layernorm_bwd_masked(const void* dy, const float* x, const int* inv, const float* w, const float* mean, const float* rstd,
+                             const float* dres_in, float* dx_out, float* dw, float* db, void* cast_out, const float* rowscale,
+                             int rows_per_group, float* dbias_next, int rows, int D, float* partial, size_t partial_bytes, hipStream_t stream) {
+    PPF_CHECK_ARG(dy && x && inv && mean && rstd && w && dx_out, PPF_ERR_ARG, "ppf_layernorm_bwd_masked: dy, x, inv, w, mean, rstd and dx_out are required");
+    return ln_bwd_run(dy, x, nullptr, inv, w, mean, rstd, dres_in, dx_out, dw, db, cast_out, rowscale, rows_per_group, nullptr, dbias_next,
+                      nullptr, nullptr, rows, D, partial, partial_bytes, stream);
+}
+
 int ppf_layernorm_bwd_blocks(int rows) { return ln_bwd_grid(rows) + LN_RS; }
 
 int ppf_layernorm_bwd_reduce(const float* partial, int rows, int D, float* dw, float* db, float* dbias_next, float* dcolscale, hipStream_t stream) {
diff --git a/protopformer_amd/ops.py b/protopformer_amd/ops.py
--- a/protopformer_amd/ops.py
+++ b/protopformer_amd/ops.py
@@ -35,12 +35,21 @@
 
 
 def gemm(a, b, *, trans_a=False, trans_b=False, epi=EPI_BF16, out=None, bias=None, res=None, rowscale=None,
-         rows_per_group=1, colscale=None, aux_in=None, aux_out=None, colsum=None, alpha=1.0, lda=None, ldb=None, workspace=True):
+         rows_per_group=1, colscale=None, aux_in=None, aux_out=None, colsum=None, alpha=1.0, lda=None, ldb=None, workspace=True, rows=None, inv=None):
     _chk(a, torch.bfloat16), _chk(b, torch.bfloat16)
     lda = a.shape[1] if lda is None else lda
     ldb = b.shape[1] if ldb is None else ldb
     M, K = (a.shape[1], a.numel() // lda) if trans_a else (a.numel() // lda, a.shape[1])
     N, Kb = (b.shape[1], b.numel() // ldb) if trans_b else (b.numel() // ldb, b.shape[1])
+    if rows is not None:
+        _chk(rows, torch.int32)
+        if not (epi == EPI_DGELU and not trans_a and bias is None and alpha == 1.0 and rows.numel() == M):
+            raise ValueError("gemm: rows applies to EPI_DGELU with one entry per output row")
+    if inv is not None:
+        _chk(inv, torch.int32)
+        if not (epi == EPI_ATOMIC and trans_a and trans_b and inv.numel() == Kb and K <= Kb):
+            raise ValueError("gemm: inv applies to the weight-gradient form, one entry per contraction row of b")
+        K = Kb
     assert K == Kb, f"contraction mismatch {K} vs {Kb}"
     if out is None:
         odt = torch.float32 if epi in (EPI_F32, EPI_SIGMOID_F32, EPI_RESID, EPI_ATOMIC) else torch.bfloat16
@@ -55,6 +64,12 @@
     ws = None
     if epi == EPI_ATOMIC and workspace:
         ws = _workspace(a.device, _lib.lib().ppf_gemm_workspace_bytes(M, N, K), _GEMM_WS)
+    if inv is not None:
+        _lib.call("ppf_gemm_wgrad_masked", a, b, inv, out, M, N, K, lda, ldb, out.shape[-1], colsum, ws, ws.numel() if ws is not None else 0)
+        return out
+    if rows is not None:
+        _lib.call("ppf_gemm_dgelu_rows", a, b, out, M, N, K, lda, ldb, out.shape[-1], int(trans_b), aux_in, rows, ldaux)
+        return out
     _lib.call("ppf_gemm_bf16", a, b, out, M, N, K, lda, ldb, out.shape[-1], int(trans_a), int(trans_b), epi,
               bias, res, res.shape[-1] if res is not None else 0, rowscale, rows_per_group, colscale, aux_in, aux_out, ldaux,
               colsum, float(alpha), ws, ws.numel() if ws is not None else 0)
@@ -143,9 +158,11 @@
 
 
 def layernorm_bwd(dy, x, w, mean, rstd, dw, db, *, dres_in=None, dx_out=None, row_map=None, cast_out=None, rowscale=None,
-                  rows_per_group=1, colscale=None, dbias_next=None, branch=None, dcolscale=None, lane=None, defer_reduce=False):
+                  rows_per_group=1, colscale=None, dbias_next=None, branch=None, dcolscale=None, lane=None, defer_reduce=False, inv=None):
     D = x.shape[-1] if x is not None else dres_in.shape[-1]
-    if dy is not None:
+    if inv is not None:
+        rows = inv.numel()
+    elif dy is not None:
         rows = dy.numel() // D
     else:
         rows = dres_in.numel() // D
@@ -155,8 +172,16 @@
     if any(t is not None for t in sums):
         dev = (dy if dy is not None else dres_in).device
         part = torch.empty(_lib.lib().ppf_layernorm_bwd_blocks(rows) * 4 * D, dtype=torch.float32, device=dev)
-    _lib.call("ppf_layernorm_bwd", dy, x, row_map, w, mean, rstd, dres_in, dx_out, dw, db, cast_out, rowscale, rows_per_group,
-              colscale, dbias_next, branch, dcolscale, rows, D, part, part.numel() * 4 if part is not None else 0)
+    if inv is not None:
+        if row_map is not None or colscale is not None or branch is not None or dy is None or dx_out is None:
+            raise ValueError("layernorm_bwd: the inv form takes dy and dx_out and neither row_map nor LayerScale")
+        _chk(inv, torch.int32)
+        assert x.numel() // D == rows and dx_out.numel() // D == rows
+        _lib.call("ppf_layernorm_bwd_masked", dy, x, inv, w, mean, rstd, dres_in, dx_out, dw, db, cast_out, rowscale, rows_per_group,
+                  dbias_next, rows, D, part, part.numel() * 4 if part is not None else 0)
+    else:
+        _lib.call("ppf_layernorm_bwd", dy, x, row_map, w, mean, rstd, dres_in, dx_out, dw, db, cast_out, rowscale, rows_per_group,
+                  colscale, dbias_next, branch, dcolscale, rows, D, part, part.numel() * 4 if part is not None else 0)
     if part is not None:
         red = lambda: _lib.call("ppf_layernorm_bwd_reduce", part, rows, D, *sums)
         if lane is not None:
@@ -659,6 +684,16 @@
     return rows
 
 
+def inverse_rows_map(rows, nrows_full):
+    inv = torch.empty(nrows_full, dtype=torch.int32, device=rows.device)
+    _lib.call("ppf_inverse_rows_map", rows, inv, rows.numel(), nrows_full)
+    return inv
+
+
+def layernorm_bwd_masked_ok(D):
+    return bool(_lib.lib().ppf_layernorm_bwd_masked_supported(int(D)))
+
+
 def gather_rows(src, rows):
     _chk(src)
     dst = torch.empty((rows.numel(), src.shape[1]), dtype=src.dtype, device=src.device)
```

Result: no change. 17240 images/sec, median of 6 (+0.3%).
